# Fung-Lab/MatDeepLearn

Hardware: AMD Instinct MI355X
Metric: edges/sec training CGCNN on bulk_data (higher is better)
Workload: dtype bf16

## Files before the change

include/mdl_hip.h:

```cpp
#ifndef MDL_HIP_H
#define MDL_HIP_H

#include <stddef.h>
#include <stdint.h>

#ifdef __cplusplus
extern "C" {
#endif

#define MDL_VERSION 100

enum { MDL_F32 = 0, MDL_BF16 = 1 };
enum { MDL_SUM = 0, MDL_MEAN = 1, MDL_MAX = 2 };
enum {
    MDL_OK = 0,
    MDL_E_ARG = -1,
    MDL_E_UNSUPP = -2,
    MDL_E_LAUNCH = -3
};

#define MDL_DTYPE_MASK 0xff
#define MDL_DETERMINISTIC 0x100
#define MDL_K3_PER_WAVE 0x200
#define MDL_K3_EDGE_LANE 0x400
#define MDL_BN_SHIFT_ROW 0x800
#define MDL_SPLIT_BF16 0x1000
#define MDL_MLP_F32_IO 0x2000

typedef void* mdlStream_t;

int mdl_version(void);
const char* mdl_last_error_string(void);
int mdl_debug_last_k3(void);

int mdl_rbf_expand(const float* d, const float* offsets, float coeff, void* out, int64_t E, int G,
                   int64_t ld_out, int out_dtype, mdlStream_t stream);

int mdl_csr_rowptr(const int32_t* sorted_index, int64_t E, int64_t N, int32_t* rowptr, mdlStream_t stream);

int mdl_segment_reduce_fwd(const void* src, const int32_t* rowptr, const int32_t* perm, void* out,
                           int32_t* argmax, int64_t N, int64_t C, int reduce, int dtype, mdlStream_t stream);
int mdl_segment_reduce_bwd(const void* grad_out, const int32_t* rowptr, const int32_t* seg,
                           const int32_t* perm, const int32_t* argmax, void* grad_src, int64_t N,
                           int64_t E, int64_t C, int reduce, int dtype, mdlStream_t stream);
int mdl_segment_reduce_bwd_add(const void* grad_out, const int32_t* rowptr, const int32_t* seg, const int32_t* perm,
                               const void* addend, void* grad_src, int64_t N, int64_t E, int64_t C, int reduce, int dtype,
                               mdlStream_t stream);

size_t mdl_cgconv_wpack_bytes(int C, int G, int dtype);
int mdl_cgconv_pack_weights(const float* w_f, const float* b_f, const float* w_s, const float* b_s, int C,
                            int G, void* wpack, float* bpack, int dtype, mdlStream_t stream);
int mdl_cgconv_pack_weights_node(const float* w_f, const float* b_f, const float* w_s, const float* b_s, int C,
                                 int G, void* wpack, float* bpack, void* wn_t, int dtype, mdlStream_t stream);

int mdl_cgconv_pack_weights_multi(int L, const float* const* w_f, const float* const* b_f, const float* const* w_s,
                                  const float* const* b_s, int C, int G, void* const* wpack, float* const* bpack,
                                  void* const* wn_t, int dtype, mdlStream_t stream);

int mdl_cgconv_fwd(const void* x, const void* edge_attr, const int32_t* rowptr, const int32_t* src,
                   const int32_t* tgt, const int32_t* eperm, const void* wpack, const float* bpack,
                   void* out, int64_t N, int64_t E, int C, int G, int aggr, int dtype, mdlStream_t stream);

typedef struct MdlCgConv {
    uint32_t size;
    int32_t dtype;
    uint32_t flags;
    int32_t aggr;
    int64_t N, E;
    int32_t C, G;
    const void* x;
    const void* edge_attr;
    const int32_t* rowptr;
    const int32_t* src;
    const int32_t* tgt;
    const int32_t* eperm;
    const void* wpack;
    const float* bpack;
    void* out;
    float* bn_sums;
    const float* bn_shift;
    const int64_t* bn_rows;
    const void* grad_out;
    void* r_tgt;
    void* r_src;
    int32_t r_src_dtype;
    int32_t ld_dwe;
    float* dwe;
    float* db;
    void* workspace;
    size_t workspace_bytes;
    const int32_t* balance;
} MdlCgConv;
int mdl_cgconv_fwd_ex(const MdlCgConv* args, mdlStream_t stream);
int mdl_cgconv_bwd_ex(const MdlCgConv* args, mdlStream_t stream);

int mdl_cgconv_balance(const int32_t* rowptr, const int32_t* src, int64_t N, int32_t* cost, mdlStream_t stream);

size_t mdl_cgconv_workspace_bytes(int64_t N, int64_t E, int C, int G, int dtype);

typedef struct MdlCgNode {
    uint32_t size;
    int32_t dtype;
    uint32_t flags;
    int32_t zero_src;
    int64_t N;
    int32_t C;
    int32_t r_src_dtype;
    int32_t ld_dwn;
    int32_t reserved;
    const void* x;
    const void* grad_out;
    const void* r_tgt;
    void* r_src;
    const void* wn_t;
    void* dx;
    float* dwn;
} MdlCgNode;
int mdl_cgconv_bwd_node_ex(const MdlCgNode* args, mdlStream_t stream);

int mdl_cgconv_pack_node_weights(const float* w_f, const float* w_s, int C, int G, void* wn_t, int dtype, mdlStream_t stream);
int mdl_cgconv_assemble_grads(const float* dwn, const float* dwe, const float* db, int C, int G, float* dw_f, float* dw_s,
                              float* db_f, float* db_s, mdlStream_t stream);

int mdl_assemble_batch(const int64_t* ids, const int64_t* noff, const int64_t* eoff, const int64_t* node_ptr,
                       const int64_t* edge_ptr, const float* x_all, const int32_t* src_l, const int32_t* tgt_l,
                       const float* dist, const float* dist_norm, const int32_t* lrowptr, const float* y_all,
                       void* x, int64_t* batch, int32_t* rowptr, int32_t* src, int32_t* tgt, float* ew, float* dn,
                       float* y, int B, int F, int T, int target_index, int dtype, mdlStream_t stream);
int mdl_assemble_batch_padded(const int64_t* ids, const int64_t* noff, const int64_t* eoff, const int64_t* node_ptr,
                              const int64_t* edge_ptr, const float* x_all, const int32_t* src_l, const int32_t* tgt_l,
                              const float* dist, const float* dist_norm, const int32_t* lrowptr, const float* y_all,
                              void* x, int64_t* batch, int32_t* rowptr, int32_t* src, int32_t* tgt, float* ew, float* dn,
                              float* y, int B, int F, int T, int target_index, int dtype, int64_t n_cap, int64_t e_cap,
                              int32_t* pool_seg, int32_t* col_s, int32_t* eid_s, int32_t* src_s, mdlStream_t stream);

int mdl_ssp_bwd(const void* g, const void* y, void* dx, int64_t n, int dtype, mdlStream_t stream);

int mdl_linear_act_stats(const void* x, const void* w, const void* bias, const void* p1, const int32_t* idx1, const void* p2,
                         const int32_t* idx2, const void* p3, const int32_t* idx3, void* out, int64_t N, int K, int M, int act,
                         float* bn_sums, const int64_t* n_rows_dev, int dtype, mdlStream_t stream);
int mdl_linear_gather_act(const void* x, const void* w, const void* bias, const void* p1, const int32_t* idx1,
                          const void* p2, const int32_t* idx2, const void* p3, const int32_t* idx3, void* out,
                          int64_t N, int K, int M, int act, int dtype, mdlStream_t stream);

int mdl_nnconv_msg_fwd(const void* Y, const void* h, const int32_t* rowptr_s, const int32_t* eid_s, void* m, int64_t N,
                       int Co, int D3, int dtype, mdlStream_t stream);
int mdl_nnconv_msg_bwd(const void* Y, const void* h, const void* dm, const int32_t* rowptr_s, const int32_t* eid_s,
                       void* dh, void* dY, int64_t N, int Co, int D3, int dtype, mdlStream_t stream);

int mdl_pad_batch_tail(const int64_t* noff, const int64_t* eoff, int B, int64_t n_cap, int32_t* rowptr, int64_t* batch,
                       mdlStream_t stream);

int mdl_assemble_transposed(const int64_t* ids, const int64_t* noff, const int64_t* eoff, const int64_t* node_ptr,
                            const int64_t* edge_ptr, const int32_t* src_l, const int32_t* tgt_l, const int32_t* eperm_s,
                            const int32_t* lrowptr_s, int32_t* rowptr_s, int32_t* col_s, int32_t* eid_s, int32_t* src_s, int B,
                            int64_t n_cap, mdlStream_t stream);
int mdl_pad_edge_tail(const int64_t* noff, const int64_t* eoff, int B, int64_t n_cap, int64_t e_cap, int32_t* src, int32_t* tgt,
                      int32_t* col_s, int32_t* eid_s, int32_t* src_s, mdlStream_t stream);

int mdl_loss_fwd_bwd(const float* pred, const float* y, int64_t n, int kind, float* loss, float* grad, mdlStream_t stream);
int mdl_loss_fwd_bwd_rows(const float* pred, const float* y, int64_t n, int64_t n_total, int kind, float* loss, float* grad,
                          mdlStream_t stream);

#define MDL_BN_REPLICAS 16
int mdl_bn_sums_rows(void);
int mdl_bn_stats_n(const void* x, float* sums, int64_t N, int C, const int64_t* n_rows_dev, int dtype, mdlStream_t stream);
int mdl_bn_apply_n(const void* x, float* sums, const float* gamma, const float* beta, float* save, float* running_mean,
                   float* running_var, void* y, int64_t N, int C, float eps, float momentum, const int64_t* n_rows_dev,
                   int dtype, mdlStream_t stream);
int mdl_bn_bwd_stats_n(const void* dy, const void* x, const float* save, float* sums, int64_t N, int C,
                       const int64_t* n_rows_dev, int dtype, mdlStream_t stream);
int mdl_bn_bwd_apply_n(const void* dy, const void* x, const float* save, float* sums, const float* gamma, void* dx,
                       int64_t N, int C, const int64_t* n_rows_dev, int dtype, mdlStream_t stream);
int mdl_bn_bwd_apply_relu_n(const void* dy, const void* x, const float* save, float* sums, const float* gamma, void* dx,
                            int64_t N, int C, const int64_t* n_rows_dev, int dtype, mdlStream_t stream);
int mdl_linear_act(const void* x, const void* w, const void* bias, void* out, int64_t N, int K, int M, int act, int dtype,
                   mdlStream_t stream);
int mdl_linear_act_in(const void* x, const void* y, int xact, const void* w, const void* bias, void* out, int64_t N, int K,
                      int M, int act, int dtype, mdlStream_t stream);

int mdl_mlp_head_fwd(const void* x, const void* const* w, const void* const* b, void* const* h, int64_t N, int K0, int NL,
                     const int* M, int dtype, mdlStream_t stream);
int mdl_mlp_head_bwd(const void* x, const void* const* w, const void* const* h, const void* gy, void* dx, float* const* dw,
                     float* const* db, int64_t N, int K0, int NL, const int* M, int dtype, mdlStream_t stream);

int mdl_gru_gates_fwd(const void* gi, const void* gh, const float* h, float* h_out, void* out_lp, int64_t N, int C, int dtype,
                      mdlStream_t stream);
int mdl_gru_gates_bwd(const void* gi, const void* gh, const float* h, const float* g_h, const void* g_lp, void* dgi, void* dgh,
                      float* dh, int64_t N, int C, int dtype, mdlStream_t stream);

int mdl_linear_wide(const void* x, const void* w, void* out, int64_t N, int K, int64_t M, int dtype, mdlStream_t stream);

int mdl_gemm_tn(const void* a, int64_t lda, int M, const void* b, int64_t ldb, int K, float* c, int64_t N, int dtype,
                mdlStream_t stream);
int mdl_gemm_tn_colsum(const void* a, int64_t lda, int M, const void* b, int64_t ldb, int K, float* c, float* colsum,
                       int64_t N, int dtype, mdlStream_t stream);
int mdl_gemm_tn_act(const void* a, int64_t lda, int M, const void* y, int64_t ldy, int act, const void* b, int64_t ldb,
                    int K, float* c, float* colsum, int64_t N, int dtype, mdlStream_t stream);
int mdl_dense_bwd(const void* g, int64_t ldg, int M, const void* y, int64_t ldy, int act, const void* x, int64_t ldx, int K,
                  const void* w, void* dx, int64_t lddx, int xout, void* gm, float* dw, float* db, int64_t N, int dtype,
                  mdlStream_t stream);
size_t mdl_tn_scratch_bytes(void);
int mdl_dense_bwd_ex(const void* g, int64_t ldg, int M, const void* y, int64_t ldy, int act, const void* x, int64_t ldx, int K,
                     const void* w, void* dx, int64_t lddx, int xout, void* gm, float* dw, float* db, void* scratch, int64_t N,
                     int dtype, mdlStream_t stream);
int mdl_gemm_tn_ex(const void* a, int64_t lda, int M, const void* y, int64_t ldy, int act, const void* b, int64_t ldb, int K,
                   float* c, float* colsum, void* scratch, int64_t N, int dtype, mdlStream_t stream);

int mdl_gather_rows(const void* src, const int32_t* idx, void* out, int64_t E, int64_t C, int dtype,
                    mdlStream_t stream);
int mdl_gather_mul_reduce(const void* h, const void* w, const float* scale, const int32_t* rowptr,
                          const int32_t* col, const int32_t* eid, void* out, int64_t N, int64_t F, int reduce,
                          int dtype, mdlStream_t stream);
int mdl_gather_mul_reduce_dw(const void* g, const void* w, const float* scale, const int32_t* rowptr_s,
                             const int32_t* col_s, const int32_t* eid_s, void* dh, const void* h, void* dw,
                             int64_t N, int64_t F, int dtype, mdlStream_t stream);
int mdl_cfconv_supported(int F, int G, int dtype);
size_t mdl_cfconv_wpack_bytes(void);
int mdl_cfconv_pack_weights(const float* w1, const float* b1, const float* w2, const float* b2, int F, int G, void* wpack,
                            mdlStream_t stream);
int mdl_cfconv_fwd(const void* rbf, const float* cut, const void* h, const int32_t* rowptr, const int32_t* src,
                   const int32_t* tgt, const void* wpack, void* out, void* a1, void* w, int64_t N, int64_t E, int F, int G,
                   int dtype, mdlStream_t stream);
size_t mdl_cfconv_bwd_w_scratch_bytes(void);
int mdl_cfconv_bwd_w(const void* rbf, const float* cut, const void* h, const void* g, const int32_t* rowptr, const int32_t* src,
                     const int32_t* tgt, const void* wpack, float* dw1, float* db1, float* dw2, float* db2, void* scratch, int64_t N,
                     int64_t E, int F, int G, int dtype, mdlStream_t stream);
int mdl_edge_mul(const void* a, const int32_t* ia, const void* b, const int32_t* ib, const float* scale, void* out,
                 int64_t E, int64_t F, int dtype, mdlStream_t stream);
int mdl_edge_dot(const void* a, const int32_t* ia, const void* b, const int32_t* ib, const void* w, float* out, int64_t E,
                 int64_t F, int dtype, mdlStream_t stream);
int mdl_cfconv_bwd_edge_supported(int F, int G, int dtype);
int mdl_cfconv_bwd_edge(const void* rbf, const float* cut, const void* h, const void* g, const int32_t* rowptr, const int32_t* src,
                        const int32_t* tgt, const void* wpack, const float* w1, const float* b1, const float* w2, const float* b2,
                        int64_t N, int64_t E, int F, int G, int dtype, float* dcut, void* drbf, const float* d_norm,
                        const float* offsets, float coeff, float scale, float* dd, mdlStream_t stream);

int mdl_split_bf16(const float* src, void* hi, void* lo, int64_t n, mdlStream_t stream);

size_t mdl_graph_workspace_bytes(int64_t N, int64_t G, int max_neighbors);
int mdl_graph_build(const double* pos, const int64_t* node_ptr, const double* cell, const int32_t* pbc, int64_t N, int64_t G,
                    double radius, int max_neighbors, int64_t* edge_ptr, int32_t* src, int32_t* tgt, float* dist,
                    int32_t* out_deg, int64_t edge_capacity, void* workspace, size_t workspace_bytes, mdlStream_t stream);

int mdl_rbf_expand_bwd(const void* g_out, int64_t ld_g, int g_dtype, const float* d, const float* offsets, float coeff,
                       float* dd, int64_t E, int G, mdlStream_t stream);

int mdl_cgconv_bwd_edge(const void* x, const void* edge_attr, const int32_t* rowptr, const int32_t* src, const int32_t* tgt,
                        const void* wpack, const float* bpack, const void* grad_out, int64_t N, int64_t E, int C, int G,
                        int aggr, int dtype, void* de, const float* d_norm, const float* offsets, float coeff, float scale,
                        float* dd, mdlStream_t stream);

int mdl_linear_rbf_dist_grad_supported(int M, int G, int dtype);
int mdl_linear_rbf_dist_grad(const void* g, int64_t ld_g, const void* act_y, int64_t ld_y, const void* w, int dtype,
                             const float* d, const float* offsets, float coeff, float scale, float* dd, int accumulate,
                             int64_t E, int M, int G, mdlStream_t stream);

size_t mdl_edge_geometry_workspace_bytes(int64_t G);
int mdl_edge_geometry_fwd(const double* pos, const int64_t* node_ptr, const double* cell, const int32_t* pbc, int64_t N,
                          int64_t G, const int32_t* src, const int32_t* tgt, int64_t E, float* dist, float* u,
                          void* workspace, size_t workspace_bytes, mdlStream_t stream);
int mdl_edge_geometry_bwd(const float* dd, const float* u, const int32_t* rowptr_t, const int32_t* eid_t,
                          const int32_t* rowptr_s, const int32_t* eid_s, int64_t N, int64_t E, float* dpos,
                          mdlStream_t stream);

size_t mdl_edge_strain_grad_workspace_bytes(int64_t G, int64_t E, int32_t slices);
int mdl_edge_strain_grad(const float* dd, const float* dist, const float* u, const int32_t* rowptr_t, const int32_t* eid_t,
                         const int64_t* node_ptr, int64_t N, int64_t G, int64_t E, int32_t slices, float* out, void* workspace,
                         size_t workspace_bytes, mdlStream_t stream);

#ifdef __cplusplus
}
#endif
#endif
```

matdeeplearn_amd/_lib.py:

```python
import ctypes
import os

import torch

HERE = os.path.dirname(os.path.abspath(__file__))
LIB_PATH = os.path.join(HERE, "lib", "libmdl_hip.so")


def use_library(path):
    global LIB_PATH, _lib
    if _lib is not None and os.path.abspath(path) != os.path.abspath(LIB_PATH):
        raise MdlError("use_library(%s): %s is already loaded in this process" % (path, LIB_PATH))
    LIB_PATH = path

MDL_F32, MDL_BF16 = 0, 1
MDL_SUM, MDL_MEAN, MDL_MAX = 0, 1, 2
MDL_DTYPE_MASK, MDL_DETERMINISTIC, MDL_K3_PER_WAVE, MDL_K3_EDGE_LANE = 0xFF, 0x100, 0x200, 0x400
MDL_MLP_F32_IO = 0x2000
MDL_SPLIT_BF16 = 0x1000
MDL_BN_SHIFT_ROW = 0x800
MDL_BN_REPLICAS = 16
REDUCE = {"sum": MDL_SUM, "add": MDL_SUM, "mean": MDL_MEAN, "max": MDL_MAX}

_vp, _i64, _i32, _f32, _sz = ctypes.c_void_p, ctypes.c_int64, ctypes.c_int, ctypes.c_float, ctypes.c_size_t
_u32 = ctypes.c_uint32


class MdlCgConv(ctypes.Structure):
    _fields_ = [("size", _u32), ("dtype", _i32), ("flags", _u32), ("aggr", _i32), ("N", _i64), ("E", _i64), ("C", _i32), ("G", _i32),
                ("x", _vp), ("edge_attr", _vp), ("rowptr", _vp), ("src", _vp), ("tgt", _vp), ("eperm", _vp), ("wpack", _vp),
                ("bpack", _vp), ("out", _vp), ("bn_sums", _vp), ("bn_shift", _vp), ("bn_rows", _vp), ("grad_out", _vp),
                ("r_tgt", _vp), ("r_src", _vp), ("r_src_dtype", _i32), ("ld_dwe", _i32), ("dwe", _vp), ("db", _vp),
                ("workspace", _vp), ("workspace_bytes", _sz), ("balance", _vp)]


class MdlCgNode(ctypes.Structure):
    _fields_ = [("size", _u32), ("dtype", _i32), ("flags", _u32), ("zero_src", _i32), ("N", _i64), ("C", _i32), ("r_src_dtype", _i32),
                ("ld_dwn", _i32), ("reserved", _i32), ("x", _vp), ("grad_out", _vp), ("r_tgt", _vp), ("r_src", _vp), ("wn_t", _vp), ("dx", _vp), ("dwn", _vp)]


def _dp(t):
    return None if t is None else t.data_ptr()


def cg_args(**kw):
    a = MdlCgConv()
    a.size = ctypes.sizeof(MdlCgConv)
    for k, v in kw.items():
        setattr(a, k, _dp(v) if torch.is_tensor(v) else v)
    return a


def cg_node_args(**kw):
    a = MdlCgNode()
    a.size = ctypes.sizeof(MdlCgNode)
    for k, v in kw.items():
        setattr(a, k, _dp(v) if torch.is_tensor(v) else v)
    return a

PROTOTYPES = {
    "mdl_version": (_i32, []),
    "mdl_last_error_string": (ctypes.c_char_p, []),
    "mdl_debug_last_k3": (_i32, []),
    "mdl_rbf_expand": (_i32, [_vp, _vp, _f32, _vp, _i64, _i32, _i64, _i32, _vp]),
    "mdl_csr_rowptr": (_i32, [_vp, _i64, _i64, _vp, _vp]),
    "mdl_segment_reduce_fwd": (_i32, [_vp, _vp, _vp, _vp, _vp, _i64, _i64, _i32, _i32, _vp]),
    "mdl_segment_reduce_bwd": (_i32, [_vp, _vp, _vp, _vp, _vp, _vp, _i64, _i64, _i64, _i32, _i32, _vp]),
    "mdl_segment_reduce_bwd_add": (_i32, [_vp, _vp, _vp, _vp, _vp, _vp, _i64, _i64, _i64, _i32, _i32, _vp]),
    "mdl_cgconv_wpack_bytes": (_sz, [_i32, _i32, _i32]),
    "mdl_cgconv_pack_weights": (_i32, [_vp, _vp, _vp, _vp, _i32, _i32, _vp, _vp, _i32, _vp]),
    "mdl_cgconv_pack_weights_node": (_i32, [_vp, _vp, _vp, _vp, _i32, _i32, _vp, _vp, _vp, _i32, _vp]),
    "mdl_cgconv_pack_weights_multi": (_i32, [_i32, _vp, _vp, _vp, _vp, _i32, _i32, _vp, _vp, _vp, _i32, _vp]),
    "mdl_cgconv_fwd": (_i32, [_vp] * 9 + [_i64, _i64, _i32, _i32, _i32, _i32, _vp]),
    "mdl_cgconv_fwd_ex": (_i32, [ctypes.POINTER(MdlCgConv), _vp]),
    "mdl_cgconv_bwd_ex": (_i32, [ctypes.POINTER(MdlCgConv), _vp]),
    "mdl_cgconv_bwd_node_ex": (_i32, [ctypes.POINTER(MdlCgNode), _vp]),
    "mdl_cgconv_workspace_bytes": (ctypes.c_size_t, [_i64, _i64, _i32, _i32, _i32]),
    "mdl_cgconv_balance": (_i32, [_vp, _vp, _i64, _vp, _vp]),
    "mdl_cgconv_pack_node_weights": (_i32, [_vp, _vp, _i32, _i32, _vp, _i32, _vp]),
    "mdl_cgconv_assemble_grads": (_i32, [_vp, _vp, _vp, _i32, _i32, _vp, _vp, _vp, _vp, _vp]),
    "mdl_assemble_batch": (_i32, [_vp] * 20 + [_i32, _i32, _i32, _i32, _i32, _vp]),
    "mdl_assemble_batch_padded": (_i32, [_vp] * 20 + [_i32, _i32, _i32, _i32, _i32, _i64, _i64, _vp, _vp, _vp, _vp, _vp]),
    "mdl_nnconv_msg_fwd": (_i32, [_vp] * 5 + [_i64, _i32, _i32, _i32, _vp]),
    "mdl_nnconv_msg_bwd": (_i32, [_vp] * 7 + [_i64, _i32, _i32, _i32, _vp]),
    "mdl_pad_batch_tail": (_i32, [_vp, _vp, _i32, _i64, _vp, _vp, _vp]),
    "mdl_assemble_transposed": (_i32, [_vp] * 13 + [_i32, _i64, _vp]),
    "mdl_pad_edge_tail": (_i32, [_vp, _vp, _i32, _i64, _i64, _vp, _vp, _vp, _vp, _vp, _vp]),
    "mdl_loss_fwd_bwd": (_i32, [_vp, _vp, _i64, _i32, _vp, _vp, _vp]),
    "mdl_loss_fwd_bwd_rows": (_i32, [_vp, _vp, _i64, _i64, _i32, _vp, _vp, _vp]),
    "mdl_bn_sums_rows": (_i32, []),
    "mdl_bn_stats_n": (_i32, [_vp, _vp, _i64, _i32, _vp, _i32, _vp]),
    "mdl_bn_apply_n": (_i32, [_vp] * 8 + [_i64, _i32, _f32, _f32, _vp, _i32, _vp]),
    "mdl_bn_bwd_stats_n": (_i32, [_vp, _vp, _vp, _vp, _i64, _i32, _vp, _i32, _vp]),
    "mdl_bn_bwd_apply_n": (_i32, [_vp] * 6 + [_i64, _i32, _vp, _i32, _vp]),
    "mdl_bn_bwd_apply_relu_n": (_i32, [_vp] * 6 + [_i64, _i32, _vp, _i32, _vp]),
    "mdl_linear_act": (_i32, [_vp, _vp, _vp, _vp, _i64, _i32, _i32, _i32, _i32, _vp]),
    "mdl_dense_bwd": (_i32, [_vp, _i64, _i32, _vp, _i64, _i32, _vp, _i64, _i32, _vp, _vp, _i64, _i32, _vp, _vp, _vp, _i64, _i32, _vp]),
    "mdl_dense_bwd_ex": (_i32, [_vp, _i64, _i32, _vp, _i64, _i32, _vp, _i64, _i32, _vp, _vp, _i64, _i32, _vp, _vp, _vp, _vp, _i64, _i32, _vp]),
    "mdl_tn_scratch_bytes": (_sz, []),
    "mdl_linear_act_stats": (_i32, [_vp, _vp, _vp, _vp, _vp, _vp, _vp, _vp, _vp, _vp, _i64, _i32, _i32, _i32, _vp, _vp, _i32, _vp]),
    "mdl_linear_act_in": (_i32, [_vp, _vp, _i32, _vp, _vp, _vp, _i64, _i32, _i32, _i32, _i32, _vp]),
    "mdl_ssp_bwd": (_i32, [_vp, _vp, _vp, _i64, _i32, _vp]),
    "mdl_linear_gather_act": (_i32, [_vp] * 10 + [_i64, _i32, _i32, _i32, _i32, _vp]),
    "mdl_linear_wide": (_i32, [_vp, _vp, _vp, _i64, _i32, _i64, _i32, _vp]),
    "mdl_mlp_head_fwd": (_i32, [_vp, _vp, _vp, _vp, _i64, _i32, _i32, _vp, _i32, _vp]),
    "mdl_mlp_head_bwd": (_i32, [_vp, _vp, _vp, _vp, _vp, _vp, _vp, _i64, _i32, _i32, _vp, _i32, _vp]),
    "mdl_gru_gates_fwd": (_i32, [_vp, _vp, _vp, _vp, _vp, _i64, _i32, _i32, _vp]),
    "mdl_gru_gates_bwd": (_i32, [_vp, _vp, _vp, _vp, _vp, _vp, _vp, _vp, _i64, _i32, _i32, _vp]),
    "mdl_gemm_tn": (_i32, [_vp, _i64, _i32, _vp, _i64, _i32, _vp, _i64, _i32, _vp]),
    "mdl_split_bf16": (_i32, [_vp, _vp, _vp, _i64, _vp]),
    "mdl_gemm_tn_colsum": (_i32, [_vp, _i64, _i32, _vp, _i64, _i32, _vp, _vp, _i64, _i32, _vp]),
    "mdl_gemm_tn_act": (_i32, [_vp, _i64, _i32, _vp, _i64, _i32, _vp, _i64, _i32, _vp, _vp, _i64, _i32, _vp]),
    "mdl_gemm_tn_ex": (_i32, [_vp, _i64, _i32, _vp, _i64, _i32, _vp, _i64, _i32, _vp, _vp, _vp, _i64, _i32, _vp]),
    "mdl_gather_rows": (_i32, [_vp, _vp, _vp, _i64, _i64, _i32, _vp]),
    "mdl_gather_mul_reduce": (_i32, [_vp] * 7 + [_i64, _i64, _i32, _i32, _vp]),
    "mdl_gather_mul_reduce_dw": (_i32, [_vp] * 9 + [_i64, _i64, _i32, _vp]),
    "mdl_edge_mul": (_i32, [_vp] * 6 + [_i64, _i64, _i32, _vp]),
    "mdl_cfconv_supported": (_i32, [_i32, _i32, _i32]),
    "mdl_cfconv_wpack_bytes": (_sz, []),
    "mdl_cfconv_pack_weights": (_i32, [_vp] * 4 + [_i32, _i32, _vp, _vp]),
    "mdl_cfconv_fwd": (_i32, [_vp] * 10 + [_i64, _i64, _i32, _i32, _i32, _vp]),
    "mdl_cfconv_bwd_w_scratch_bytes": (_sz, []),
    "mdl_cfconv_bwd_w": (_i32, [_vp] * 13 + [_i64, _i64, _i32, _i32, _i32, _vp]),
    "mdl_cfconv_bwd_edge_supported": (_i32, [_i32, _i32, _i32]),
    "mdl_cfconv_bwd_edge": (_i32, [_vp] * 12 + [_i64, _i64, _i32, _i32, _i32, _vp, _vp, _vp, _vp, _f32, _f32, _vp, _vp]),
    "mdl_edge_dot": (_i32, [_vp] * 6 + [_i64, _i64, _i32, _vp]),
    "mdl_graph_workspace_bytes": (_sz, [_i64, _i64, _i32]),
    "mdl_graph_build": (_i32, [_vp] * 4 + [_i64, _i64, ctypes.c_double, _i32] + [_vp] * 5 + [_i64, _vp, _sz, _vp]),
    "mdl_rbf_expand_bwd": (_i32, [_vp, _i64, _i32, _vp, _vp, _f32, _vp, _i64, _i32, _vp]),
    "mdl_cgconv_bwd_edge": (_i32, [_vp] * 8 + [_i64, _i64, _i32, _i32, _i32, _i32, _vp, _vp, _vp, _f32, _f32, _vp, _vp]),
    "mdl_linear_rbf_dist_grad_supported": (_i32, [_i32, _i32, _i32]),
    "mdl_linear_rbf_dist_grad": (_i32, [_vp, _i64, _vp, _i64, _vp, _i32, _vp, _vp, _f32, _f32, _vp, _i32, _i64, _i32, _i32, _vp]),
    "mdl_edge_geometry_workspace_bytes": (_sz, [_i64]),
    "mdl_edge_geometry_fwd": (_i32, [_vp] * 4 + [_i64, _i64, _vp, _vp, _i64, _vp, _vp, _vp, _sz, _vp]),
    "mdl_edge_geometry_bwd": (_i32, [_vp] * 6 + [_i64, _i64, _vp, _vp]),
    "mdl_edge_strain_grad_workspace_bytes": (_sz, [_i64, _i64, _i32]),
    "mdl_edge_strain_grad": (_i32, [_vp] * 6 + [_i64, _i64, _i64, _i32, _vp, _vp, _sz, _vp]),
}

_lib = None


class MdlError(RuntimeError):
    pass


def lib():
    global _lib
    if _lib is None:
        if not os.path.exists(LIB_PATH):
            raise MdlError(
                "libmdl_hip.so not found at %s — build it with `python -m matdeeplearn_amd._build` "
                "(hipcc --offload-arch=gfx950).  matdeeplearn_amd has no CPU/eager fallback." % LIB_PATH)
        handle = ctypes.CDLL(LIB_PATH)
        for name, (res, args) in PROTOTYPES.items():
            fn = getattr(handle, name)
            fn.restype, fn.argtypes = res, args
        _lib = handle
    return _lib


def check(rc, what):
    if rc != 0:
        raise MdlError("%s failed (%d): %s" % (what, rc, lib().mdl_last_error_string().decode()))


def dtype_code(t):
    if t.dtype == torch.float32:
        return MDL_F32
    if t.dtype == torch.bfloat16:
        return MDL_BF16
    raise MdlError("unsupported dtype %s (float32 or bfloat16)" % t.dtype)


def require_hip(*tensors):
    cur = None
    for t in tensors:
        if t is None:
            continue
        if not t.is_cuda:
            raise MdlError("matdeeplearn_amd ops need tensors on a HIP device (got %s); there is no CPU path — "
                           "the CPU restatement lives in oracle/ and is test infrastructure only" % t.device)
        if cur is None:
            cur = torch.cuda.current_device()
        if t.device.index != cur:
            raise MdlError("tensor on %s but the current HIP device is cuda:%d — call torch.cuda.set_device(%d) in "
                           "this process before using matdeeplearn_amd" % (t.device, cur, t.device.index))


def ptr(t):
    return None if t is None else ctypes.c_void_p(t.data_ptr())


def stream():
    return ctypes.c_void_p(torch._C._cuda_getCurrentRawStream(torch.cuda.current_device()))
```

matdeeplearn_amd/csrc/bn.hip:

```cpp
#include "mdl_common.h"

namespace mdl {

constexpr int BN_R = MDL_BN_REPLICAS;

__device__ __forceinline__ void bn_totals(const float* __restrict__ sums, float* tot, int C, float* publish) {
    for (int c = threadIdx.x; c < 2 * C; c += blockDim.x) {
        float v[BN_R];
#pragma unroll
        for (int r = 0; r < BN_R; ++r) v[r] = sums[(size_t)r * 2 * C + c];
        float t = 0.0f;
#pragma unroll
        for (int r = 0; r < BN_R; ++r) t += v[r];
        tot[c] = t;
        if (publish && blockIdx.x == 0) publish[c] = t;
    }
    __syncthreads();
}

template <typename T, int MODE, int W>
__global__ __launch_bounds__(256) void bn_reduce_kernel(const T* __restrict__ a, const T* __restrict__ b,
                                                        const float* __restrict__ save, float* __restrict__ sums,
                                                        int64_t Ncap, int C, const int64_t* __restrict__ n_dev) {
    typedef VecW<T, W> V;
    const int64_t N = n_dev ? max((int64_t)1, min(*n_dev, Ncap)) : Ncap;
    __shared__ float red[2][256 * 8 / 8 * 8];
    const int CG = C / W;
    const int rows_per_block = (int)blockDim.x / CG;
    const int cg = threadIdx.x % CG, rl = threadIdx.x / CG;
    const bool active = rl < rows_per_block;
    float s0[W], s1[W], p0[W], p1[W];
#pragma unroll
    for (int j = 0; j < W; ++j) { s0[j] = 0.0f; s1[j] = 0.0f; }
    if (MODE == 0) {
        V::ld(a + cg * W, p0);
    } else {
#pragma unroll
        for (int j = 0; j < W; ++j) { p0[j] = save[cg * W + j]; p1[j] = save[C + cg * W + j]; }
    }
    if (active) {
        constexpr int U = 4;
        const int64_t stride = (int64_t)gridDim.x * rows_per_block;
        for (int64_t n0 = (int64_t)blockIdx.x * rows_per_block + rl; n0 < N; n0 += U * stride) {
            float va[U][W], vb[U][W];
#pragma unroll
            for (int u = 0; u < U; ++u) {
                const int64_t n = min(n0 + u * stride, N - 1);
                V::ld(a + n * C + cg * W, va[u]);
                if (MODE != 0) V::ld(b + n * C + cg * W, vb[u]);
            }
#pragma unroll
            for (int u = 0; u < U; ++u) {
                const float m = (n0 + u * stride < N) ? 1.0f : 0.0f;
                if (MODE == 0) {
#pragma unroll
                    for (int j = 0; j < W; ++j) { const float d = (va[u][j] - p0[j]) * m; s0[j] += d; s1[j] += d * d; }
                } else {
#pragma unroll
                    for (int j = 0; j < W; ++j) { const float v = va[u][j] * m; s0[j] += v; s1[j] += v * ((vb[u][j] - p0[j]) * p1[j]); }
                }
            }
        }
    }
#pragma unroll
    for (int j = 0; j < W; ++j) { red[0][threadIdx.x * W + j] = s0[j]; red[1][threadIdx.x * W + j] = s1[j]; }
    __syncthreads();
    if ((int)threadIdx.x < C) {
        const int c = threadIdx.x, g = c / W, j = c % W;
        float t0 = 0.0f, t1 = 0.0f;
        for (int r = 0; r < rows_per_block; ++r) { t0 += red[0][(r * CG + g) * W + j]; t1 += red[1][(r * CG + g) * W + j]; }
        float* dst = sums + (size_t)(blockIdx.x % BN_R) * 2 * C;
        unsafeAtomicAdd(dst + c, t0);
        unsafeAtomicAdd(dst + C + c, t1);
    }
}

template <typename T, int W>
__global__ __launch_bounds__(256) void bn_apply_kernel(const T* __restrict__ x, float* __restrict__ sums,
                                                       const float* __restrict__ gamma, const float* __restrict__ beta,
                                                       float* __restrict__ save, float* __restrict__ run_mean,
                                                       float* __restrict__ run_var, T* __restrict__ y, int64_t Ncap, int C,
                                                       float eps, float momentum, const int64_t* __restrict__ n_dev,
                                                       int shift_row) {
    typedef VecW<T, W> V;
    constexpr int U = 4;
    const int64_t N = n_dev ? max((int64_t)1, min(*n_dev, Ncap)) : Ncap;
    __shared__ float tot[512];
    const int CG = C / W;
    const int cg = threadIdx.x % CG;
    const int64_t total = N * CG;
    const int64_t stride = (int64_t)gridDim.x * blockDim.x;
    int64_t q0 = (int64_t)blockIdx.x * blockDim.x + threadIdx.x;
    float v[U][W];
#pragma unroll
    for (int u = 0; u < U; ++u) V::ld(x + (min(q0 + u * stride, total - 1) / CG) * C + cg * W, v[u]);
    float mean[W], scale[W], shiftv[W], sh[W];
    V::ld(x + cg * W, sh);
    if (shift_row) {
        const float* srow = sums + (size_t)(2 * BN_R + 2) * C;
#pragma unroll
        for (int j = 0; j < W; ++j) sh[j] = srow[cg * W + j];
    }
    bn_totals(sums, tot, C, sums + (size_t)BN_R * 2 * C);
    const float invn = 1.0f / (float)N;
#pragma unroll
    for (int j = 0; j < W; ++j) {
        const int c = cg * W + j;
        const float m1 = tot[c] * invn;
        const float var = fmaxf(tot[C + c] * invn - m1 * m1, 0.0f);
        const float istd = rsqrtf(var + eps);
        mean[j] = sh[j] + m1;
        const float g = gamma ? gamma[c] : 1.0f;
        scale[j] = istd * g;
        shiftv[j] = (beta ? beta[c] : 0.0f) - mean[j] * scale[j];
        if (blockIdx.x == 0 && (int)threadIdx.x < CG) {
            save[c] = mean[j];
            save[C + c] = istd;
            if (run_mean) {
                const float unb = N > 1 ? var * ((float)N / (float)(N - 1)) : var;
                run_mean[c] = (1.0f - momentum) * run_mean[c] + momentum * mean[j];
                run_var[c] = (1.0f - momentum) * run_var[c] + momentum * unb;
            }
        }
    }
    while (true) {
#pragma unroll
        for (int u = 0; u < U; ++u) {
            const int64_t q = q0 + u * stride;
#pragma unroll
            for (int j = 0; j < W; ++j) v[u][j] = v[u][j] * scale[j] + shiftv[j];
            if (q < total) V::st(y + (q / CG) * C + cg * W, v[u]);
        }
        q0 += U * stride;
        if (q0 >= total) break;
#pragma unroll
        for (int u = 0; u < U; ++u) V::ld(x + (min(q0 + u * stride, total - 1) / CG) * C + cg * W, v[u]);
    }
    if (N < Ncap) {
        float z[W];
#pragma unroll
        for (int j = 0; j < W; ++j) z[j] = 0.0f;
        for (int64_t q = total + (int64_t)blockIdx.x * blockDim.x + threadIdx.x; q < Ncap * CG; q += stride)
            V::st(y + (q / CG) * C + cg * W, z);
    }
}

template <typename T, int W, bool MASK = false>
__global__ __launch_bounds__(256) void bn_bwd_apply_kernel(const T* __restrict__ dy, const T* __restrict__ x,
                                                           const float* __restrict__ save, float* __restrict__ sums,
                                                           const float* __restrict__ gamma, T* __restrict__ dx, int64_t Ncap,
                                                           int C, const int64_t* __restrict__ n_dev) {
    typedef VecW<T, W> V;
    constexpr int U = 2;
    const int64_t N = n_dev ? max((int64_t)1, min(*n_dev, Ncap)) : Ncap;
    __shared__ float tot[512];
    const int CG = C / W;
    const int cg = threadIdx.x % CG;
    const int64_t total = N * CG;
    const int64_t stride = (int64_t)gridDim.x * blockDim.x;
    int64_t q0 = (int64_t)blockIdx.x * blockDim.x + threadIdx.x;
    float vd[U][W], vx[U][W];
#pragma unroll
    for (int u = 0; u < U; ++u) {
        const int64_t n = min(q0 + u * stride, total - 1) / CG;
        V::ld(dy + n * C + cg * W, vd[u]);
        V::ld(x + n * C + cg * W, vx[u]);
    }
    bn_totals(sums, tot, C, sums + (size_t)BN_R * 2 * C);
    const float invn = 1.0f / (float)N;
    float mean[W], istd[W], k0[W], k1[W], gs[W];
#pragma unroll
    for (int j = 0; j < W; ++j) {
        const int c = cg * W + j;
        mean[j] = save[c];
        istd[j] = save[C + c];
        gs[j] = (gamma ? gamma[c] : 1.0f) * istd[j];
        k0[j] = tot[c] * invn;
        k1[j] = tot[C + c] * invn;
    }
    while (true) {
#pragma unroll
        for (int u = 0; u < U; ++u) {
            const int64_t q = q0 + u * stride;
#pragma unroll
            for (int j = 0; j < W; ++j) {
                const float d = gs[j] * (vd[u][j] - k0[j] - (vx[u][j] - mean[j]) * istd[j] * k1[j]);
                vd[u][j] = (!MASK || vx[u][j] > 0.0f) ? d : 0.0f;
            }
            if (q < total) V::st(dx + (q / CG) * C + cg * W, vd[u]);
        }
        q0 += U * stride;
        if (q0 >= total) break;
#pragma unroll
        for (int u = 0; u < U; ++u) {
            const int64_t n = min(q0 + u * stride, total - 1) / CG;
            V::ld(dy + n * C + cg * W, vd[u]);
            V::ld(x + n * C + cg * W, vx[u]);
        }
    }
    if (N < Ncap) {
        float z[W];
#pragma unroll
        for (int j = 0; j < W; ++j) z[j] = 0.0f;
        for (int64_t q = total + (int64_t)blockIdx.x * blockDim.x + threadIdx.x; q < Ncap * CG; q += stride)
            V::st(dx + (q / CG) * C + cg * W, z);
    }
}


static int bn_width(int C, int dtype) { return (dtype == MDL_BF16 && C % 8 == 0) ? 8 : 4; }
static int bn_threads(int C, int W) { const int cg = C / W; return 256 / cg * cg; }

static int bn_check(const char* name, int64_t N, int C, int dtype, const void* p) {
    MDL_REQUIRE(dtype == MDL_F32 || dtype == MDL_BF16, MDL_E_UNSUPP, "%s: unsupported dtype %d", name, dtype);
    MDL_REQUIRE(N >= 1 && C >= 4 && C % 4 == 0 && C <= 256, MDL_E_UNSUPP,
                "%s: need N>=1 and C a multiple of 4, C<=256 (got N=%lld C=%d)", name, (long long)N, C);
    MDL_REQUIRE(p && reinterpret_cast<uintptr_t>(p) % (bn_width(C, dtype) * (dtype == MDL_BF16 ? 2 : 4)) == 0, MDL_E_ARG,
                "%s: null or misaligned tensor", name);
    return MDL_OK;
}

static unsigned bn_grid(int64_t N, int C, int W, bool det) {
    if (det) return 1;
    const int rows = 256 / (C / W);
    int64_t g = cdiv(N, (int64_t)rows * 8);
    if (g > 1024) g = 1024;
    return (unsigned)(g < 1 ? 1 : g);
}

}

extern "C" int mdl_bn_sums_rows(void) { return 2 * (MDL_BN_REPLICAS + 1); }

extern "C" int mdl_bn_stats_n(const void* x, float* sums, int64_t N, int C, const int64_t* n_dev, int dtype, mdlStream_t stream) {
    using namespace mdl;
    const bool det = (dtype & MDL_DETERMINISTIC) != 0;
    dtype &= MDL_DTYPE_MASK;
    int rc = bn_check("mdl_bn_stats", N, C, dtype, x);
    if (rc) return rc;
    hipStream_t st = (hipStream_t)stream;
    const int W = bn_width(C, dtype);
    if (dtype == MDL_BF16 && W == 8) hipLaunchKernelGGL((bn_reduce_kernel<bf16_t, 0, 8>), dim3(bn_grid(N, C, W, det)), dim3(bn_threads(C, 8)), 0, st, (const bf16_t*)x, (const bf16_t*)nullptr, (const float*)nullptr, sums, N, C, n_dev);
    else if (dtype == MDL_BF16) hipLaunchKernelGGL((bn_reduce_kernel<bf16_t, 0, 4>), dim3(bn_grid(N, C, W, det)), dim3(bn_threads(C, 4)), 0, st, (const bf16_t*)x, (const bf16_t*)nullptr, (const float*)nullptr, sums, N, C, n_dev);
    else hipLaunchKernelGGL((bn_reduce_kernel<float, 0, 4>), dim3(bn_grid(N, C, W, det)), dim3(bn_threads(C, 4)), 0, st, (const float*)x, (const float*)nullptr, (const float*)nullptr, sums, N, C, n_dev);
    return check_launch("mdl_bn_stats");
}

extern "C" int mdl_bn_apply_n(const void* x, float* sums, const float* gamma, const float* beta, float* save,
                              float* running_mean, float* running_var, void* y, int64_t N, int C, float eps, float momentum,
                              const int64_t* n_dev, int dtype, mdlStream_t stream) {
    using namespace mdl;
    const int shift_row = (dtype & MDL_BN_SHIFT_ROW) ? 1 : 0;
    dtype &= MDL_DTYPE_MASK;
    int rc = bn_check("mdl_bn_apply", N, C, dtype, x);
    if (rc) return rc;
    hipStream_t st = (hipStream_t)stream;
    int64_t g = cdiv(N * (C / bn_width(C, dtype)), 256 * 4);
    if (g > 768) g = 768;
    if (g < 1) g = 1;
    const int W = bn_width(C, dtype);
    if (dtype == MDL_BF16 && W == 8) hipLaunchKernelGGL((bn_apply_kernel<bf16_t, 8>), dim3((unsigned)g), dim3(bn_threads(C, 8)), 0, st, (const bf16_t*)x, sums, gamma, beta, save, running_mean, running_var, (bf16_t*)y, N, C, eps, momentum, n_dev, shift_row);
    else if (dtype == MDL_BF16) hipLaunchKernelGGL((bn_apply_kernel<bf16_t, 4>), dim3((unsigned)g), dim3(bn_threads(C, 4)), 0, st, (const bf16_t*)x, sums, gamma, beta, save, running_mean, running_var, (bf16_t*)y, N, C, eps, momentum, n_dev, shift_row);
    else hipLaunchKernelGGL((bn_apply_kernel<float, 4>), dim3((unsigned)g), dim3(bn_threads(C, 4)), 0, st, (const float*)x, sums, gamma, beta, save, running_mean, running_var, (float*)y, N, C, eps, momentum, n_dev, shift_row);
    return check_launch("mdl_bn_apply");
}

extern "C" int mdl_bn_bwd_stats_n(const void* dy, const void* x, const float* save, float* sums, int64_t N, int C,
                                  const int64_t* n_dev, int dtype, mdlStream_t stream) {
    using namespace mdl;
    const bool det = (dtype & MDL_DETERMINISTIC) != 0;
    dtype &= MDL_DTYPE_MASK;
    int rc = bn_check("mdl_bn_bwd_stats", N, C, dtype, x);
    if (rc) return rc;
    hipStream_t st = (hipStream_t)stream;
    const int W = bn_width(C, dtype);
    if (dtype == MDL_BF16 && W == 8) hipLaunchKernelGGL((bn_reduce_kernel<bf16_t, 1, 8>), dim3(bn_grid(N, C, W, det)), dim3(bn_threads(C, 8)), 0, st, (const bf16_t*)dy, (const bf16_t*)x, save, sums, N, C, n_dev);
    else if (dtype == MDL_BF16) hipLaunchKernelGGL((bn_reduce_kernel<bf16_t, 1, 4>), dim3(bn_grid(N, C, W, det)), dim3(bn_threads(C, 4)), 0, st, (const bf16_t*)dy, (const bf16_t*)x, save, sums, N, C, n_dev);
    else hipLaunchKernelGGL((bn_reduce_kernel<float, 1, 4>), dim3(bn_grid(N, C, W, det)), dim3(bn_threads(C, 4)), 0, st, (const float*)dy, (const float*)x, save, sums, N, C, n_dev);
    return check_launch("mdl_bn_bwd_stats");
}

static int bn_bwd_apply_launch(const char* name, bool mask, const void* dy, const void* x, const float* save, float* sums, const float* gamma,
                               void* dx, int64_t N, int C, const int64_t* n_dev, int dtype, mdlStream_t stream) {
    using namespace mdl;
    dtype &= MDL_DTYPE_MASK;
    int rc = bn_check(name, N, C, dtype, x);
    if (rc) return rc;
    hipStream_t st = (hipStream_t)stream;
    int64_t g = cdiv(N * (C / bn_width(C, dtype)), 256 * 4);
    if (g > 768) g = 768;
    if (g < 1) g = 1;
    const int W = bn_width(C, dtype);
    if (mask) {
        MDL_REQUIRE(dtype == MDL_BF16, MDL_E_UNSUPP, "%s: bf16 only", name);
        if (W == 8) hipLaunchKernelGGL((bn_bwd_apply_kernel<bf16_t, 8, true>), dim3((unsigned)g), dim3(bn_threads(C, 8)), 0, st, (const bf16_t*)dy, (const bf16_t*)x, save, sums, gamma, (bf16_t*)dx, N, C, n_dev);
        else hipLaunchKernelGGL((bn_bwd_apply_kernel<bf16_t, 4, true>), dim3((unsigned)g), dim3(bn_threads(C, 4)), 0, st, (const bf16_t*)dy, (const bf16_t*)x, save, sums, gamma, (bf16_t*)dx, N, C, n_dev);
        return check_launch(name);
    }
    if (dtype == MDL_BF16 && W == 8) hipLaunchKernelGGL((bn_bwd_apply_kernel<bf16_t, 8>), dim3((unsigned)g), dim3(bn_threads(C, 8)), 0, st, (const bf16_t*)dy, (const bf16_t*)x, save, sums, gamma, (bf16_t*)dx, N, C, n_dev);
    else if (dtype == MDL_BF16) hipLaunchKernelGGL((bn_bwd_apply_kernel<bf16_t, 4>), dim3((unsigned)g), dim3(bn_threads(C, 4)), 0, st, (const bf16_t*)dy, (const bf16_t*)x, save, sums, gamma, (bf16_t*)dx, N, C, n_dev);
    else hipLaunchKernelGGL((bn_bwd_apply_kernel<float, 4>), dim3((unsigned)g), dim3(bn_threads(C, 4)), 0, st, (const float*)dy, (const float*)x, save, sums, gamma, (float*)dx, N, C, n_dev);
    return check_launch(name);
}

extern "C" int mdl_bn_bwd_apply_n(const void* dy, const void* x, const float* save, float* sums, const float* gamma,
                                  void* dx, int64_t N, int C, const int64_t* n_dev, int dtype, mdlStream_t stream) {
    return bn_bwd_apply_launch("mdl_bn_bwd_apply", false, dy, x, save, sums, gamma, dx, N, C, n_dev, dtype, stream);
}
extern "C" int mdl_bn_bwd_apply_relu_n(const void* dy, const void* x, const float* save, float* sums, const float* gamma,
                                       void* dx, int64_t N, int C, const int64_t* n_dev, int dtype, mdlStream_t stream) {
    return bn_bwd_apply_launch("mdl_bn_bwd_apply_relu", true, dy, x, save, sums, gamma, dx, N, C, n_dev, dtype, stream);
}
```

matdeeplearn_amd/csrc/cgconv_node.hip:

```cpp
#include "mdl_common.h"

namespace mdl {

constexpr int K3C_NW = 8;

typedef __attribute__((ext_vector_type(4))) unsigned u32x4_t;

__device__ __forceinline__ bf16x8 pack8(const float* v) {
    u32x4_t r = {pk_bf16(v[0], v[1]), pk_bf16(v[2], v[3]), pk_bf16(v[4], v[5]), pk_bf16(v[6], v[7])};
    return __builtin_bit_cast(bf16x8, r);
}

template <int CP, bool RS16 = false, int NW = 4>
__global__ __launch_bounds__(64 * NW, 2) void cgconv_node_stream_kernel(const bf16_t* __restrict__ x, const bf16_t* __restrict__ gout,
                                                                    const bf16_t* __restrict__ r_tgt,
                                                                    const float* __restrict__ r_src,
                                                                    const bf16_t* __restrict__ wn_t, bf16_t* __restrict__ dx,
                                                                    float* __restrict__ dwn, int64_t N, int zero_src, int ld_out) {
    typedef __attribute__((ext_vector_type(4))) short s16x4;
    typedef __attribute__((address_space(3))) s16x4* lds4_t;
    constexpr int TN = 64;
    constexpr int K4 = 4 * CP;
    constexpr int LD = K4 + 8;
    constexpr int LX = CP + 8;
    constexpr int NT = CP / 32;
    constexpr int TCH = 2 * CP / 8;
    constexpr int SCH = 2 * CP / 4;
    constexpr int NTH = 64 * NW;
    constexpr int NTL = TN * TCH / NTH;
    constexpr int NSL = RS16 ? NTL : TN * SCH / NTH;
    constexpr int XCH = CP / 8;
    constexpr int NXL = TN * XCH / NTH;
    constexpr int MJ = (K4 / 32) * NT / NW;
    static_assert(NTL >= 1 && NSL >= 1 && NXL >= 1 && MJ >= 1, "too many waves for this width");
    extern __shared__ __attribute__((aligned(16))) char smem[];
    bf16_t* wl = reinterpret_cast<bf16_t*>(smem);
    bf16_t* rl = wl + CP * LD;
    bf16_t* xl = rl + TN * LD;
    const int tid = threadIdx.x, lane = tid & 63, i = lane & 31, h = lane >> 5, wv = __builtin_amdgcn_readfirstlane(tid >> 6);
    for (int q = tid; q < CP * (K4 / 8); q += NTH) {
        const int row = q / (K4 / 8), c8 = q - row * (K4 / 8);
        *reinterpret_cast<bf16x8*>(wl + row * LD + c8 * 8) = *reinterpret_cast<const bf16x8*>(wn_t + row * K4 + c8 * 8);
    }
    f32x16 dw[MJ];
#pragma unroll
    for (int j = 0; j < MJ; ++j)
#pragma unroll
        for (int r = 0; r < 16; ++r) dw[j][r] = 0.0f;

    const int64_t n_tiles = (N + TN - 1) / TN;
    u32x4_t treg[NTL];
    f32x4 sreg[NSL];
    u32x4_t xreg[NXL];
    static_assert(NTH % TCH == 0 && NTH % SCH == 0 && NTH % XCH == 0, "chunk mapping");
    constexpr int TROWS = NTH / TCH, SROWS = NTH / SCH, XROWS = NTH / XCH;
    const int trow0 = tid / TCH, tcc = tid % TCH, srow0 = tid / SCH, scc = tid % SCH, xrow0 = tid / XCH, xcc = tid % XCH;
    const int to = (trow0 * (2 * CP) + 8 * tcc) * 2, so = (srow0 * (2 * CP) + 4 * scc) * 4, xo = (xrow0 * CP + 8 * xcc) * 2;
    auto rsrc = [](const void* base, int64_t bytes) {
        return __builtin_amdgcn_make_buffer_rsrc(const_cast<void*>(base), 0, (int)(bytes < 0x7fffffffLL ? bytes : 0x7fffffffLL), 0x00020000);
    };
    auto opaque = [](int v) { asm volatile("" : "+s"(v)); return v; };
    auto load_tile = [&](int64_t tile) {
        const int64_t nb = tile * TN, rem = N - nb;
        const __amdgpu_buffer_rsrc_t tr = rsrc(r_tgt + nb * (2 * CP), rem * (2 * CP * 2));
        const __amdgpu_buffer_rsrc_t sr = RS16 ? rsrc(reinterpret_cast<const bf16_t*>(r_src) + nb * (2 * CP), rem * (2 * CP * 2))
                                               : rsrc(r_src + nb * (2 * CP), rem * (2 * CP * 4));
        const __amdgpu_buffer_rsrc_t xr = rsrc(x + nb * CP, rem * (CP * 2));
#pragma unroll
        for (int l = 0; l < NTL; ++l) treg[l] = __builtin_amdgcn_raw_buffer_load_b128(tr, to + opaque(l * (TROWS * 2 * CP * 2)), 0, 0);
#pragma unroll
        for (int l = 0; l < NSL; ++l)
            sreg[l] = __builtin_bit_cast(f32x4, __builtin_amdgcn_raw_buffer_load_b128(
                sr, RS16 ? to + opaque(l * (TROWS * 2 * CP * 2)) : so + opaque(l * (SROWS * 2 * CP * 4)), 0, 0));
#pragma unroll
        for (int l = 0; l < NXL; ++l) xreg[l] = __builtin_amdgcn_raw_buffer_load_b128(xr, xo + opaque(l * (XROWS * CP * 2)), 0, 0);
    };
    int64_t tile = blockIdx.x;
    if (tile < n_tiles) load_tile(tile);
    for (; tile < n_tiles; tile += gridDim.x) {
        const int64_t nb = tile * TN;
        __syncthreads();
#pragma unroll
        for (int l = 0; l < NTL; ++l) *reinterpret_cast<u32x4_t*>(rl + (trow0 + l * TROWS) * LD + 8 * tcc) = treg[l];
#pragma unroll
        for (int l = 0; l < NSL; ++l) {
            if constexpr (RS16) {
                *reinterpret_cast<u32x4_t*>(rl + (trow0 + l * TROWS) * LD + 2 * CP + 8 * tcc) = __builtin_bit_cast(u32x4_t, sreg[l]);
            } else {
                typedef __attribute__((ext_vector_type(2))) unsigned u32x2_t;
                const u32x2_t v = {pk_bf16(sreg[l][0], sreg[l][1]), pk_bf16(sreg[l][2], sreg[l][3])};
                *reinterpret_cast<u32x2_t*>(rl + (srow0 + l * SROWS) * LD + 2 * CP + 4 * scc) = v;
            }
        }
        if (zero_src) {
            const int64_t rem = N - nb;
            const __amdgpu_buffer_rsrc_t sz = RS16 ? rsrc(reinterpret_cast<const bf16_t*>(r_src) + nb * (2 * CP), rem * (2 * CP * 2))
                                                   : rsrc(r_src + nb * (2 * CP), rem * (2 * CP * 4));
#pragma unroll
            for (int l = 0; l < NSL; ++l)
                __builtin_amdgcn_raw_buffer_store_b128(u32x4_t{0u, 0u, 0u, 0u}, sz,
                                                       RS16 ? to + opaque(l * (TROWS * 2 * CP * 2)) : so + opaque(l * (SROWS * 2 * CP * 4)), 0, 0);
        }
#pragma unroll
        for (int l = 0; l < NXL; ++l) {
            *reinterpret_cast<u32x4_t*>(xl + (xrow0 + l * XROWS) * LX + 8 * xcc) = xreg[l];
        }
        __syncthreads();
        const bool dxw = wv < 2 * NT;
        const int mt0 = wv / NT, nt0 = wv - mt0 * NT;
        const int64_t remg = N - nb - mt0 * 32;
        const int go = (4 * h * CP + nt0 * 32 + i) * 2;
        const bool more = tile + gridDim.x < n_tiles;
        if (!dxw) {
            if (more) load_tile(tile + gridDim.x);
        } else {
            short gv[16];
            const __amdgpu_buffer_rsrc_t gr = rsrc(gout + (nb + mt0 * 32) * CP, (remg > 0 ? remg : 0) * (CP * 2));
#pragma unroll
            for (int r = 0; r < 16; ++r) gv[r] = __builtin_amdgcn_raw_buffer_load_b16(gr, go + ((r & 3) + 8 * (r >> 2)) * CP * 2, 0, 0);
            if (more) load_tile(tile + gridDim.x);
            f32x16 acc;
#pragma unroll
            for (int r = 0; r < 16; ++r) acc[r] = 0.0f;
#pragma unroll
            for (int kk = 0; kk < K4 / 16; ++kk) {
                const bf16x8 a = *reinterpret_cast<const bf16x8*>(rl + (mt0 * 32 + i) * LD + 16 * kk + 8 * h);
                const bf16x8 b = *reinterpret_cast<const bf16x8*>(wl + (nt0 * 32 + i) * LD + 16 * kk + 8 * h);
                acc = __builtin_amdgcn_mfma_f32_32x32x16_bf16(a, b, acc, 0, 0, 0);
            }
            const __amdgpu_buffer_rsrc_t dr = rsrc(dx + (nb + mt0 * 32) * CP, (remg > 0 ? remg : 0) * (CP * 2));
#pragma unroll
            for (int r = 0; r < 16; ++r)
                __builtin_amdgcn_raw_buffer_store_b16((short)f2bf(bf2f((bf16_t)gv[r]) + acc[r]), dr, go + ((r & 3) + 8 * (r >> 2)) * CP * 2, 0, 0);
        }
#pragma unroll
        for (int j = 0; j < MJ; ++j) {
            const int blk = wv * MJ + j, mt = blk / NT, nt = blk - mt * NT;
            const int t = i & 15;
#pragma unroll
            for (int ks = 0; ks < TN / 16; ++ks) {
                const bf16_t* pa = rl + (16 * ks + 8 * h + (t >> 2)) * LD + mt * 32 + (i & 16) + 4 * (t & 3);
                const bf16_t* pb = xl + (16 * ks + 8 * h + (t >> 2)) * LX + nt * 32 + (i & 16) + 4 * (t & 3);
                const s16x4 a0 = __builtin_amdgcn_ds_read_tr16_b64_v4i16((lds4_t)pa), a1 = __builtin_amdgcn_ds_read_tr16_b64_v4i16((lds4_t)(pa + 4 * LD));
                const s16x4 b0 = __builtin_amdgcn_ds_read_tr16_b64_v4i16((lds4_t)pb), b1 = __builtin_amdgcn_ds_read_tr16_b64_v4i16((lds4_t)(pb + 4 * LX));
                const bf16x8 af = {a0[0], a0[1], a0[2], a0[3], a1[0], a1[1], a1[2], a1[3]};
                const bf16x8 bfr = {b0[0], b0[1], b0[2], b0[3], b1[0], b1[1], b1[2], b1[3]};
                dw[j] = __builtin_amdgcn_mfma_f32_32x32x16_bf16(af, bfr, dw[j], 0, 0, 0);
            }
        }
    }
#pragma unroll
    for (int j = 0; j < MJ; ++j) {
        const int blk = wv * MJ + j, mt = blk / NT, nt = blk - mt * NT;
#pragma unroll
        for (int r = 0; r < 16; ++r) {
            const int R = mt * 32 + d_row(r, h), K = nt * 32 + i;
            const int64_t at = ld_out > 0 ? (int64_t)(((R / CP) & 1) * CP + R % CP) * ld_out + ((R / CP) >> 1) * CP + K : (int64_t)R * CP + K;
            unsafeAtomicAdd(dwn + at, dw[j][r]);
        }
    }
}

template <int CP, int NW>
__global__ __launch_bounds__(64 * NW, 1) void cgconv_node_x3_kernel(const float* __restrict__ x, const float* __restrict__ gout,
                                                                    const float* __restrict__ r_tgt, float* __restrict__ r_src,
                                                                    const float* __restrict__ wn_t, float* __restrict__ dx,
                                                                    float* __restrict__ dwn, int64_t N, int zero_src, int ld_out) {
    typedef __attribute__((ext_vector_type(4))) short s16x4;
    typedef __attribute__((address_space(3))) s16x4* lds4_t;
    typedef __attribute__((ext_vector_type(2))) unsigned u32x2_t;
    constexpr int TN = 64, K4 = 4 * CP, LD = K4 + 8, LX = CP + 8, NT = CP / 32, NTH = 64 * NW;
    constexpr int RCH = 2 * CP / 4;
    constexpr int XCH = CP / 4;
    constexpr int NRL = TN * RCH / NTH;
    constexpr int NXL = TN * XCH / NTH;
    constexpr int MJ = (K4 / 32) * NT / NW;
    static_assert(NRL >= 1 && NXL >= 1 && MJ >= 1 && NTH % RCH == 0 && NTH % XCH == 0 && 2 * NT <= NW, "shape / wave count");
    extern __shared__ __attribute__((aligned(16))) char smem[];
    bf16_t* wl_h = reinterpret_cast<bf16_t*>(smem);
    bf16_t* wl_l = wl_h + CP * LD;
    bf16_t* rl_h = wl_l + CP * LD;
    bf16_t* rl_l = rl_h + TN * LD;
    bf16_t* xl_h = rl_l + TN * LD;
    bf16_t* xl_l = xl_h + TN * LX;
    const int tid = threadIdx.x, lane = tid & 63, i = lane & 31, h = lane >> 5, wv = __builtin_amdgcn_readfirstlane(tid >> 6);
    auto split4 = [](const f32x4& v, u32x2_t& hi, u32x2_t& lo) {
        const unsigned ha = pk_bf16(v[0], v[1]), hb = pk_bf16(v[2], v[3]);
        hi = u32x2_t{ha, hb};
        lo = u32x2_t{pk_bf16(v[0] - __builtin_bit_cast(float, ha << 16), v[1] - __builtin_bit_cast(float, ha & 0xffff0000u)),
                     pk_bf16(v[2] - __builtin_bit_cast(float, hb << 16), v[3] - __builtin_bit_cast(float, hb & 0xffff0000u))};
    };
    for (int q = tid; q < CP * (K4 / 4); q += NTH) {
        const int row = q / (K4 / 4), c4 = q - row * (K4 / 4);
        u32x2_t hi, lo;
        split4(*reinterpret_cast<const f32x4*>(wn_t + row * K4 + c4 * 4), hi, lo);
        *reinterpret_cast<u32x2_t*>(wl_h + row * LD + c4 * 4) = hi;
        *reinterpret_cast<u32x2_t*>(wl_l + row * LD + c4 * 4) = lo;
    }
    f32x16 dw[MJ];
#pragma unroll
    for (int j = 0; j < MJ; ++j)
#pragma unroll
        for (int r = 0; r < 16; ++r) dw[j][r] = 0.0f;

    const int64_t n_tiles = (N + TN - 1) / TN;
    f32x4 treg[NRL], sreg[NRL], xreg[NXL];
    constexpr int RROWS = NTH / RCH, XROWS = NTH / XCH;
    const int rrow0 = tid / RCH, rcc = tid % RCH, xrow0 = tid / XCH, xcc = tid % XCH;
    const int ro = (rrow0 * (2 * CP) + 4 * rcc) * 4, xo = (xrow0 * CP + 4 * xcc) * 4;
    auto rsrc = [](const void* base, int64_t bytes) {
        return __builtin_amdgcn_make_buffer_rsrc(const_cast<void*>(base), 0, (int)(bytes < 0 ? 0 : (bytes < 0x7fffffffLL ? bytes : 0x7fffffffLL)), 0x00020000);
    };
    auto opaque = [](int v) { asm volatile("" : "+s"(v)); return v; };
    auto load_tile = [&](int64_t tile) {
        const int64_t nb = tile * TN, rem = N - nb;
        const __amdgpu_buffer_rsrc_t tr = rsrc(r_tgt + nb * (2 * CP), rem * (2 * CP * 4));
        const __amdgpu_buffer_rsrc_t sr = rsrc(r_src + nb * (2 * CP), rem * (2 * CP * 4));
        const __amdgpu_buffer_rsrc_t xr = rsrc(x + nb * CP, rem * (CP * 4));
#pragma unroll
        for (int l = 0; l < NRL; ++l) treg[l] = __builtin_bit_cast(f32x4, __builtin_amdgcn_raw_buffer_load_b128(tr, ro + opaque(l * (RROWS * 2 * CP * 4)), 0, 0));
#pragma unroll
        for (int l = 0; l < NRL; ++l) sreg[l] = __builtin_bit_cast(f32x4, __builtin_amdgcn_raw_buffer_load_b128(sr, ro + opaque(l * (RROWS * 2 * CP * 4)), 0, 0));
#pragma unroll
        for (int l = 0; l < NXL; ++l) xreg[l] = __builtin_bit_cast(f32x4, __builtin_amdgcn_raw_buffer_load_b128(xr, xo + opaque(l * (XROWS * CP * 4)), 0, 0));
    };
    int64_t tile = blockIdx.x;
    if (tile < n_tiles) load_tile(tile);
    for (; tile < n_tiles; tile += gridDim.x) {
        const int64_t nb = tile * TN;
        __syncthreads();
#pragma unroll
        for (int l = 0; l < NRL; ++l) {
            u32x2_t hi, lo;
            split4(treg[l], hi, lo);
            *reinterpret_cast<u32x2_t*>(rl_h + (rrow0 + l * RROWS) * LD + 4 * rcc) = hi;
            *reinterpret_cast<u32x2_t*>(rl_l + (rrow0 + l * RROWS) * LD + 4 * rcc) = lo;
            split4(sreg[l], hi, lo);
            *reinterpret_cast<u32x2_t*>(rl_h + (rrow0 + l * RROWS) * LD + 2 * CP + 4 * rcc) = hi;
            *reinterpret_cast<u32x2_t*>(rl_l + (rrow0 + l * RROWS) * LD + 2 * CP + 4 * rcc) = lo;
        }
        if (zero_src) {
            const __amdgpu_buffer_rsrc_t sz = rsrc(r_src + nb * (2 * CP), (N - nb) * (2 * CP * 4));
#pragma unroll
            for (int l = 0; l < NRL; ++l)
                __builtin_amdgcn_raw_buffer_store_b128(u32x4_t{0u, 0u, 0u, 0u}, sz, ro + opaque(l * (RROWS * 2 * CP * 4)), 0, 0);
        }
#pragma unroll
        for (int l = 0; l < NXL; ++l) {
            u32x2_t hi, lo;
            split4(xreg[l], hi, lo);
            *reinterpret_cast<u32x2_t*>(xl_h + (xrow0 + l * XROWS) * LX + 4 * xcc) = hi;
            *reinterpret_cast<u32x2_t*>(xl_l + (xrow0 + l * XROWS) * LX + 4 * xcc) = lo;
        }
        __syncthreads();
        const bool dxw = wv < 2 * NT;
        const int mt0 = wv / NT, nt0 = wv - mt0 * NT;
        const int64_t remg = N - nb - mt0 * 32;
        const int go = (4 * h * CP + nt0 * 32 + i) * 4;
        const bool more = tile + gridDim.x < n_tiles;
        if (!dxw) {
            if (more) load_tile(tile + gridDim.x);
        } else {
            float gv[16];
            const __amdgpu_buffer_rsrc_t gr = rsrc(gout + (nb + mt0 * 32) * CP, (remg > 0 ? remg : 0) * (CP * 4));
#pragma unroll
            for (int r = 0; r < 16; ++r)
                gv[r] = __builtin_bit_cast(float, __builtin_amdgcn_raw_buffer_load_b32(gr, go + ((r & 3) + 8 * (r >> 2)) * CP * 4, 0, 0));
            if (more) load_tile(tile + gridDim.x);
            f32x16 acc;
#pragma unroll
            for (int r = 0; r < 16; ++r) acc[r] = 0.0f;
#pragma unroll
            for (int kk = 0; kk < K4 / 16; ++kk) {
                const int ao = (mt0 * 32 + i) * LD + 16 * kk + 8 * h, bo = (nt0 * 32 + i) * LD + 16 * kk + 8 * h;
                const bf16x8 ah = *reinterpret_cast<const bf16x8*>(rl_h + ao), al = *reinterpret_cast<const bf16x8*>(rl_l + ao);
                const bf16x8 bh = *reinterpret_cast<const bf16x8*>(wl_h + bo), bl = *reinterpret_cast<const bf16x8*>(wl_l + bo);
                acc = __builtin_amdgcn_mfma_f32_32x32x16_bf16(al, bh, acc, 0, 0, 0);
                acc = __builtin_amdgcn_mfma_f32_32x32x16_bf16(ah, bl, acc, 0, 0, 0);
                acc = __builtin_amdgcn_mfma_f32_32x32x16_bf16(ah, bh, acc, 0, 0, 0);
            }
            const __amdgpu_buffer_rsrc_t dr = rsrc(dx + (nb + mt0 * 32) * CP, (remg > 0 ? remg : 0) * (CP * 4));
#pragma unroll
            for (int r = 0; r < 16; ++r)
                __builtin_amdgcn_raw_buffer_store_b32(__builtin_bit_cast(unsigned, gv[r] + acc[r]), dr, go + ((r & 3) + 8 * (r >> 2)) * CP * 4, 0, 0);
        }
#pragma unroll
        for (int j = 0; j < MJ; ++j) {
            const int blk = wv * MJ + j, mt = blk / NT, nt = blk - mt * NT;
            const int t = i & 15;
#pragma unroll
            for (int ks = 0; ks < TN / 16; ++ks) {
                const int pa = (16 * ks + 8 * h + (t >> 2)) * LD + mt * 32 + (i & 16) + 4 * (t & 3);
                const int pb = (16 * ks + 8 * h + (t >> 2)) * LX + nt * 32 + (i & 16) + 4 * (t & 3);
                auto frag = [&](const bf16_t* base, int off, int ld) {
                    const s16x4 v0 = __builtin_amdgcn_ds_read_tr16_b64_v4i16((lds4_t)(base + off));
                    const s16x4 v1 = __builtin_amdgcn_ds_read_tr16_b64_v4i16((lds4_t)(base + off + 4 * ld));
                    return bf16x8{v0[0], v0[1], v0[2], v0[3], v1[0], v1[1], v1[2], v1[3]};
                };
                const bf16x8 ah = frag(rl_h, pa, LD), al = frag(rl_l, pa, LD), bh = frag(xl_h, pb, LX), bl = frag(xl_l, pb, LX);
                dw[j] = __builtin_amdgcn_mfma_f32_32x32x16_bf16(al, bh, dw[j], 0, 0, 0);
                dw[j] = __builtin_amdgcn_mfma_f32_32x32x16_bf16(ah, bl, dw[j], 0, 0, 0);
                dw[j] = __builtin_amdgcn_mfma_f32_32x32x16_bf16(ah, bh, dw[j], 0, 0, 0);
            }
        }
    }
#pragma unroll
    for (int j = 0; j < MJ; ++j) {
        const int blk = wv * MJ + j, mt = blk / NT, nt = blk - mt * NT;
#pragma unroll
        for (int r = 0; r < 16; ++r) {
            const int R = mt * 32 + d_row(r, h), K = nt * 32 + i;
            const int64_t at = ld_out > 0 ? (int64_t)(((R / CP) & 1) * CP + R % CP) * ld_out + ((R / CP) >> 1) * CP + K : (int64_t)R * CP + K;
            unsafeAtomicAdd(dwn + at, dw[j][r]);
        }
    }
}

}

namespace mdl {
template <typename TO>
__global__ __launch_bounds__(256) void cgconv_pack_node_kernel(const float* __restrict__ wf, const float* __restrict__ ws, int C,
                                                               int Cp, int ldw, TO* __restrict__ wn_t) {
    const int total = C * 4 * Cp;
    for (int q = blockIdx.x * blockDim.x + threadIdx.x; q < total; q += gridDim.x * blockDim.x) {
        const int k = q / (4 * Cp), r = q - k * (4 * Cp);
        const int blk = r / Cp, c = r - blk * Cp;
        float v = 0.0f;
        if (c < C) v = ((blk & 1) ? ws : wf)[c * ldw + (blk >> 1) * C + k];
        if constexpr (std::is_same<TO, float>::value) wn_t[q] = v; else wn_t[q] = f2bf(v);
    }
}
__global__ __launch_bounds__(256) void cgconv_grads_kernel(const float* __restrict__ dwn, const float* __restrict__ dwe,
                                                           const float* __restrict__ db, int C, int Cp, int G, int GP,
                                                           float* __restrict__ dwf, float* __restrict__ dws,
                                                           float* __restrict__ dbf, float* __restrict__ dbs) {
    const int ldw = 2 * C + G, total = 2 * C * ldw;
    for (int q = blockIdx.x * blockDim.x + threadIdx.x; q < total; q += gridDim.x * blockDim.x) {
        const int part = q / (C * ldw), rem = q - part * (C * ldw);
        const int c = rem / ldw, k = rem - c * ldw;
        float v;
        if (k < C) v = dwn[(part * Cp + c) * C + k];
        else if (k < 2 * C) v = dwn[((2 + part) * Cp + c) * C + (k - C)];
        else v = dwe[(part * Cp + c) * GP + (k - 2 * C)];
        (part ? dws : dwf)[rem] = v;
    }
    for (int q = blockIdx.x * blockDim.x + threadIdx.x; q < 2 * C; q += gridDim.x * blockDim.x) {
        const int part = q / C, c = q - part * C;
        float* dst = part ? dbs : dbf;
        if (dst) dst[c] = db[part * Cp + c];
    }
}
}

extern "C" int mdl_cgconv_pack_node_weights(const float* w_f, const float* w_s, int C, int G, void* wn_t, int dtype,
                                            mdlStream_t stream) {
    using namespace mdl;
    MDL_REQUIRE(dtype == MDL_BF16 || dtype == MDL_F32, MDL_E_UNSUPP, "mdl_cgconv_pack_node_weights: dtype must be MDL_BF16 or MDL_F32");
    MDL_REQUIRE(w_f && w_s && wn_t && C >= 1 && G >= 0, MDL_E_ARG, "mdl_cgconv_pack_node_weights: bad arguments");
    const int Cp = (C + 31) / 32 * 32;
    if (dtype == MDL_F32)
        hipLaunchKernelGGL(cgconv_pack_node_kernel<float>, dim3((unsigned)cdiv((int64_t)C * 4 * Cp, 256)), dim3(256), 0, (hipStream_t)stream,
                           w_f, w_s, C, Cp, 2 * C + G, (float*)wn_t);
    else
    hipLaunchKernelGGL(cgconv_pack_node_kernel<bf16_t>, dim3((unsigned)cdiv((int64_t)C * 4 * Cp, 256)), dim3(256), 0, (hipStream_t)stream, w_f,
                       w_s, C, Cp, 2 * C + G, (bf16_t*)wn_t);
    return check_launch("mdl_cgconv_pack_node_weights");
}

extern "C" int mdl_cgconv_assemble_grads(const float* dwn, const float* dwe, const float* db, int C, int G, float* dw_f,
                                         float* dw_s, float* db_f, float* db_s, mdlStream_t stream) {
    using namespace mdl;
    MDL_REQUIRE(dwn && dwe && db && dw_f && dw_s && C >= 1 && G >= 0, MDL_E_ARG, "mdl_cgconv_assemble_grads: bad arguments");
    const int Cp = (C + 31) / 32 * 32, GP = (G + 63) / 64 * 64;
    hipLaunchKernelGGL(cgconv_grads_kernel, dim3((unsigned)cdiv((int64_t)2 * C * (2 * C + G), 256)), dim3(256), 0, (hipStream_t)stream,
                       dwn, dwe, db, C, Cp, G, GP, dw_f, dw_s, db_f, db_s);
    return check_launch("mdl_cgconv_assemble_grads");
}

static int bwd_node_launch(const void* x, const void* grad_out, const void* r_tgt, float* r_src, const void* wn_t, void* dx,
                           float* dwn, int64_t N, int C, int dtype, int zero_src, bool rs16, int ld_out, mdlStream_t stream);

extern "C" int mdl_cgconv_bwd_node_ex(const MdlCgNode* a, mdlStream_t stream) {
    MDL_REQUIRE(a && a->size == sizeof(MdlCgNode), MDL_E_ARG, "mdl_cgconv_bwd_node_ex: argument struct of another layout (size %u, expected %u)",
                a ? a->size : 0u, (unsigned)sizeof(MdlCgNode));
    MDL_REQUIRE((a->flags & ~(uint32_t)(MDL_DETERMINISTIC | MDL_SPLIT_BF16)) == 0, MDL_E_ARG, "mdl_cgconv_bwd_node_ex: unknown flag bits %#x", a->flags);
    MDL_REQUIRE(a->r_src_dtype == MDL_F32 || a->r_src_dtype == MDL_BF16, MDL_E_ARG, "mdl_cgconv_bwd_node_ex: r_src_dtype must be MDL_F32 or MDL_BF16");
    if (a->flags & MDL_SPLIT_BF16) {
        using namespace mdl;
        MDL_REQUIRE(a->dtype == MDL_F32 && a->r_src_dtype == MDL_F32 && a->C == 64 && !(a->flags & MDL_DETERMINISTIC), MDL_E_UNSUPP,
                    "mdl_cgconv_bwd_node_ex: MDL_SPLIT_BF16 needs MDL_F32 storage, fp32 by-source sums, C = 64 (C=%d dtype=%d)", a->C, a->dtype);
        MDL_REQUIRE(a->N >= 0 && (a->N == 0 || (a->x && a->grad_out && a->r_tgt && a->r_src && a->wn_t && a->dx && a->dwn)), MDL_E_ARG,
                    "mdl_cgconv_bwd_node_ex: bad arguments");
        MDL_REQUIRE(reinterpret_cast<uintptr_t>(a->wn_t) % 16 == 0 && reinterpret_cast<uintptr_t>(a->r_tgt) % 16 == 0 &&
                        reinterpret_cast<uintptr_t>(a->r_src) % 16 == 0 && reinterpret_cast<uintptr_t>(a->x) % 16 == 0 &&
                        reinterpret_cast<uintptr_t>(a->grad_out) % 4 == 0 && reinterpret_cast<uintptr_t>(a->dx) % 4 == 0, MDL_E_ARG,
                    "mdl_cgconv_bwd_node_ex: 16-byte alignment required");
        MDL_REQUIRE(a->ld_dwn == 0 || a->ld_dwn >= 2 * a->C, MDL_E_ARG, "mdl_cgconv_bwd_node_ex: ld_dwn (%d) below 2 C", a->ld_dwn);
        if (a->N == 0) return MDL_OK;
        constexpr int NWX = 8;
        const int lds = (2 * 64 * (256 + 8) + 2 * 64 * (256 + 8) + 2 * 64 * (64 + 8)) * 2;
        int64_t sgrid = cdiv(a->N, 64);
        if (sgrid > 256) sgrid = 256;
        auto kf = cgconv_node_x3_kernel<64, NWX>;
        hipError_t e = set_max_dynamic_lds(reinterpret_cast<const void*>(kf), lds);
        if (e != hipSuccess) { set_error("mdl_cgconv_bwd_node_ex: LDS attribute (%d B): %s", lds, hipGetErrorString(e)); return MDL_E_LAUNCH; }
        hipLaunchKernelGGL(kf, dim3((unsigned)sgrid), dim3(64 * NWX), lds, (hipStream_t)stream, (const float*)a->x, (const float*)a->grad_out,
                           (const float*)a->r_tgt, static_cast<float*>(a->r_src), (const float*)a->wn_t, (float*)a->dx, a->dwn, a->N, a->zero_src, a->ld_dwn);
        return check_launch("mdl_cgconv_bwd_node_ex");
    }
    return bwd_node_launch(a->x, a->grad_out, a->r_tgt, static_cast<float*>(a->r_src), a->wn_t, a->dx, a->dwn, a->N, a->C,
                           a->dtype | (int)a->flags, a->zero_src, a->r_src_dtype == MDL_BF16, a->ld_dwn, stream);
}

static int bwd_node_launch(const void* x, const void* grad_out, const void* r_tgt, float* r_src, const void* wn_t, void* dx,
                           float* dwn, int64_t N, int C, int dtype, int zero_src, bool rs16, int ld_out, mdlStream_t stream) {
    using namespace mdl;
    const bool det = (dtype & MDL_DETERMINISTIC) != 0;
    dtype &= MDL_DTYPE_MASK;
    MDL_REQUIRE(dtype == MDL_BF16, MDL_E_UNSUPP, "mdl_cgconv_bwd_node: bf16 only (fp32 parity mode uses library GEMMs)");
    MDL_REQUIRE(C == 32 || C == 64, MDL_E_UNSUPP, "mdl_cgconv_bwd_node: C must be 32 or 64 (got %d)", C);
    MDL_REQUIRE(N >= 0 && (N == 0 || (x && grad_out && r_tgt && r_src && wn_t && dx && dwn)), MDL_E_ARG,
                "mdl_cgconv_bwd_node: bad arguments");
    MDL_REQUIRE(reinterpret_cast<uintptr_t>(wn_t) % 16 == 0 && reinterpret_cast<uintptr_t>(r_tgt) % 16 == 0 &&
                    reinterpret_cast<uintptr_t>(r_src) % 16 == 0, MDL_E_ARG, "mdl_cgconv_bwd_node: 16-byte alignment required");
    MDL_REQUIRE(ld_out == 0 || ld_out >= 2 * C, MDL_E_ARG, "mdl_cgconv_bwd_node_ex: ld_dwn (%d) below 2 C", ld_out);
    if (N == 0) return MDL_OK;
    hipStream_t st = (hipStream_t)stream;
    int64_t sgrid = cdiv(N, 64);
    if (det) sgrid = 1;
    if (sgrid > 256) sgrid = 256;
    if (C == 64) {
        const int lds = (64 * (256 + 8) + 64 * (256 + 8) + 64 * (64 + 8)) * 2;
        auto kf = rs16 ? cgconv_node_stream_kernel<64, true, K3C_NW> : cgconv_node_stream_kernel<64, false, K3C_NW>;
        set_max_dynamic_lds(reinterpret_cast<const void*>(kf), lds);
        hipLaunchKernelGGL(kf, dim3((unsigned)sgrid), dim3(64 * K3C_NW), lds, st, (const bf16_t*)x, (const bf16_t*)grad_out,
                           (const bf16_t*)r_tgt, r_src, (const bf16_t*)wn_t, (bf16_t*)dx, dwn, N, zero_src, ld_out);
    } else {
        const int lds = (32 * (128 + 8) + 64 * (128 + 8) + 64 * (32 + 8)) * 2;
        auto kf = rs16 ? cgconv_node_stream_kernel<32, true> : cgconv_node_stream_kernel<32, false>;
        hipLaunchKernelGGL(kf, dim3((unsigned)sgrid), dim3(256), lds, st, (const bf16_t*)x, (const bf16_t*)grad_out,
                           (const bf16_t*)r_tgt, r_src, (const bf16_t*)wn_t, (bf16_t*)dx, dwn, N, zero_src, ld_out);
    }
    return check_launch("mdl_cgconv_bwd_node");
}
```

matdeeplearn_amd/models/_base.py:

```python
import torch
import torch.nn.functional as F
from torch import nn

from .. import ops
from ..nn import BatchNorm1d, Set2Set, lowp_copies as _lowp


def dense(lin, h, split=False):
    if h.dtype == lin.weight.dtype:
        if split and ops.linear_split_ok(h, lin.weight):
            return ops._LinearSplitTN.apply(h, lin.weight, lin.bias)
        return lin(h)
    return ops.linear(h, lin.weight, lin.bias, _lowp(lin))


def dense_act(lin, h, act, split=False):
    if h.dtype == lin.weight.dtype:
        return getattr(F, act)(dense(lin, h, split))
    return ops.linear_act(h, lin.weight, lin.bias, act, _lowp(lin))


class GraphModel(nn.Module):

    def _begin(self, data, dim1, pre_fc_count, gc_count, pool, pool_order, batch_norm, batch_track_stats, act,
               dropout_rate, compute_dtype, lists=("conv_list", "bn_list")):
        assert gc_count > 0, "Need at least 1 GC layer"
        self.batch_track_stats = batch_track_stats != "False"
        self.batch_norm, self.pool, self.act = batch_norm, pool, act
        self.pool_order, self.dropout_rate = pool_order, dropout_rate
        self.compute_dtype = {"fp32": torch.float32, "bf16": torch.bfloat16, "bf16x3": torch.float32}[compute_dtype]
        self.split_products = compute_dtype == "bf16x3"
        self.gc_dim = data.num_features if pre_fc_count == 0 else dim1
        y0 = data[0].y
        self.output_dim = 1 if y0.ndim == 0 else len(y0[0])
        self.pre_lin_list = nn.ModuleList(
            [nn.Linear(data.num_features if i == 0 else dim1, dim1) for i in range(pre_fc_count)])
        for name in lists:
            setattr(self, name, nn.ModuleList())

    def _add_bn(self, dim):
        if self.batch_norm == "True":
            self.bn_list.append(BatchNorm1d(dim, track_running_stats=self.batch_track_stats))

    def _finish(self, dim2, post_fc_count, post_in, early_mult=1, set2set_names=("set2set",)):
        s2s_early = self.pool == "set2set" and self.pool_order == "early"
        if self.pool_order == "early":
            first_in = post_in * ((2 * early_mult - 1) if (s2s_early and early_mult > 1) else (2 if s2s_early else early_mult))
        else:
            first_in = post_in
        self.post_lin_list = nn.ModuleList(
            [nn.Linear(first_in if i == 0 else dim2, dim2) for i in range(post_fc_count)])
        self.lin_out = nn.Linear(dim2 if post_fc_count > 0 else first_in, self.output_dim)
        if s2s_early:
            for name in set2set_names:
                setattr(self, name, Set2Set(post_in, processing_steps=3))
        elif self.pool == "set2set" and self.pool_order == "late":
            setattr(self, set2set_names[0], Set2Set(self.output_dim, processing_steps=3, num_layers=1))
            self.lin_out_2 = nn.Linear(self.output_dim * 2, self.output_dim)
        if self.split_products:
            from ..nn import use_split_linears
            use_split_linears(self)

    def _inputs(self, data):
        cd = self.compute_dtype
        n = data.x.shape[0]
        csr = getattr(data, "csr", None)
        if csr is None:
            csr = ops.csr_for(data.edge_index, n)
        return data.x.to(cd), data.edge_attr.to(cd), csr

    def _cast_dense(self, dtype):
        lins = getattr(self, "_dense_layers", None)
        if lins is None:
            lins = [m for m in self.modules() if isinstance(m, nn.Linear)]
            object.__setattr__(self, "_dense_layers", lins)
        params = [p for lin in lins for p in (lin.weight, lin.bias) if p is not None]
        if not params or not params[0].is_cuda or params[0].dtype == dtype:
            return
        cache = getattr(self, "_lowp_cache", None)
        if cache is None or len(cache) != len(params) or cache[0].dtype != dtype or cache[0].device != params[0].device:
            cache = [torch.empty_like(p, dtype=dtype) for p in params]
            self._lowp_cache = cache
        with torch.no_grad():
            torch._foreach_copy_(cache, [p.detach() for p in params])
        k = 0
        for lin in lins:
            w = cache[k]; k += 1
            b = None
            if lin.bias is not None:
                b = cache[k]; k += 1
            lin._mdl_lowp = (w, b, lin.weight._version, None if lin.bias is None else lin.bias._version)

    def _open_grad_arena(self, device):
        n = getattr(self, "_arena_floats", None)
        if n is None:
            R = ops.bn_sums_rows()
            n = sum(p.numel() + 128 for m in self.modules() if isinstance(m, nn.Linear) for p in (m.weight, m.bias) if p is not None)
            n += sum(R * m.num_features + 128 for m in self.modules() if isinstance(m, (BatchNorm1d, nn.BatchNorm1d)))
            object.__setattr__(self, "_arena_floats", n)
        ops.new_grad_arena(device, n)

    def _pre(self, out):
        if torch.is_grad_enabled() and out.is_cuda:
            self._open_grad_arena(out.device)
        if out.dtype == torch.bfloat16 and torch.is_grad_enabled():
            self._cast_dense(out.dtype)
        for lin in self.pre_lin_list:
            out = dense_act(lin, out, self.act, split=self.split_products)
        return out

    def _bn(self, i, out):
        return self.bn_list[i](out) if self.batch_norm == "True" else out

    def _drop(self, out):
        return F.dropout(out, p=self.dropout_rate, training=self.training)

    def _post(self, out, final=False):
        lins = list(self.post_lin_list) + [self.lin_out]
        if out.dtype != self.lin_out.weight.dtype and ops.mlp_head_ok(out, lins, self.act):
            return ops.mlp_head(out, lins, [_lowp(lin) for lin in lins], f32_out=final)
        for lin in self.post_lin_list:
            out = dense_act(lin, out, self.act, split=self.split_products)
        return dense(self.lin_out, out)

    def _pool(self, out, data):
        num_graphs = getattr(data, "num_graphs", None)
        if self.pool == "set2set":
            return self.set2set(out, data.batch, num_graphs)
        return ops.POOLS[self.pool](out, data.batch, num_graphs, seg_index=getattr(data, "pool_index", None))

    def _head(self, out, data):
        if self.pool_order == "early":
            out = self._post(self._pool(out, data).to(out.dtype), final=True)
        else:
            out = self._post(out)
            if self.pool == "set2set":
                out = dense(self.lin_out_2, self._pool(out, data).to(out.dtype))
            else:
                out = self._pool(out, data)
        out = out.float()
        return out.view(-1) if out.shape[1] == 1 else out
```

matdeeplearn_amd/models/cgcnn.py:

```python
import torch
from torch import nn

from .. import ops
from ..nn import CGConv
from ._base import GraphModel


class CGCNN(GraphModel):
    needs_by_source = False

    def __init__(self, data, dim1=64, dim2=64, pre_fc_count=1, gc_count=3, post_fc_count=1,
                 pool="global_mean_pool", pool_order="early", batch_norm="True", batch_track_stats="True",
                 act="relu", dropout_rate=0.0, compute_dtype="fp32", **kwargs):
        super().__init__()
        self._begin(data, dim1, pre_fc_count, gc_count, pool, pool_order, batch_norm, batch_track_stats, act,
                    dropout_rate, compute_dtype)
        for _ in range(gc_count):
            self.conv_list.append(CGConv(self.gc_dim, data.num_edge_features, aggr="mean", batch_norm=False))
            self._add_bn(self.gc_dim)
        self._finish(dim2, post_fc_count, self.gc_dim)

    def forward(self, data):
        x, edge_attr, csr = self._inputs(data)
        out = self._pre(x)
        bn_on = self.batch_norm == "True"
        packs = ops.cgconv_prepack(list(self.conv_list), out.dtype, out.device, want_node=torch.is_grad_enabled()) if out.is_cuda else None
        dist = getattr(data, "dist", None)
        for i, conv in enumerate(self.conv_list):
            prev = self.bn_list[i - 1].bias if (bn_on and i > 0) else None
            out = self._drop(conv(out, None, edge_attr, csr=csr, bn=self.bn_list[i] if bn_on else None, bn_shift=prev,
                                  packed=None if packs is None else packs[i], split=self.split_products, dist=dist))
        return self._head(out, data)
```

matdeeplearn_amd/nn.py:

```python
from torch import nn

from . import ops


class CGConv(nn.Module):

    def __init__(self, channels, dim=0, aggr="add", batch_norm=False, bias=True, **kwargs):
        super().__init__()
        if isinstance(channels, (tuple, list)):
            if channels[0] != channels[1]:
                raise ops.MdlError("CGConv: bipartite channel pairs are not on the reference path")
            channels = channels[0]
        if batch_norm:
            raise ops.MdlError("CGConv(batch_norm=True) is not used by the reference (cgcnn.py:81)")
        self.channels, self.dim, self.aggr = channels, dim, aggr
        self.lin_f = nn.Linear(2 * channels + dim, channels, bias=bias)
        self.lin_s = nn.Linear(2 * channels + dim, channels, bias=bias)
        self.reset_parameters()

    def reset_parameters(self):
        self.lin_f.reset_parameters()
        self.lin_s.reset_parameters()

    def forward(self, x, edge_index, edge_attr=None, csr=None, bn=None, bn_shift=None, packed=None, split=False, dist=None):
# ... 195 lines not shown
        n = x.shape[0]
        if edge_weight is None:
            edge_weight = torch.ones(csr.E, device=x.device)
        ew = edge_weight.float()
        deg = ops.scatter(ew.unsqueeze(1), csr.col, 0, n, "sum").squeeze(1)
        dis = deg.pow(-0.5)
        dis = torch.where(torch.isinf(dis), torch.zeros_like(dis), dis)
        norm = ops.gather(dis.unsqueeze(1), csr.row).squeeze(1) * ew * ops.gather(dis.unsqueeze(1), csr.col).squeeze(1)
        out = ops.gather_mul_reduce(_lin(self.lin, x), csr, w=None, scale=norm, reduce="sum")
        return out + self.bias.to(out.dtype) if self.bias is not None else out


class NNConv(nn.Module):
    def __init__(self, in_channels, out_channels, nn_module, aggr="add", root_weight=True, bias=True, chunk=32768):
        super().__init__()
        self.in_channels, self.out_channels, self.aggr, self.chunk = in_channels, out_channels, aggr, chunk
        self.nn = nn_module
        self.lin = nn.Linear(in_channels, out_channels, bias=False) if root_weight else None
        self.bias = nn.Parameter(torch.zeros(out_channels)) if bias else None
        self.reset_parameters()

    def reset_parameters(self):
        for m in self.nn.modules():
            if m is not self.nn and hasattr(m, "reset_parameters"):
                m.reset_parameters()
        if self.lin is not None:
            self.lin.reset_parameters()
        if self.bias is not None:
            self.bias.data.zero_()

    def _messages(self, xj, edge_attr):
        w = self.nn(edge_attr).view(-1, self.in_channels, self.out_channels)
        return torch.bmm(xj.unsqueeze(1), w).squeeze(1)

    def _last_linear(self):
        last = self.nn[-1] if isinstance(self.nn, nn.Sequential) and len(self.nn) > 0 else None
        if isinstance(last, nn.Linear) and last.out_features == self.in_channels * self.out_channels:
            return last
        return None

    def forward(self, x, edge_index, edge_attr, csr=None, dist=None):
        from torch.utils.checkpoint import checkpoint
        if csr is None:
            csr = ops.csr_for(edge_index, x.shape[0])
        last = self._last_linear()
        ci, co = self.in_channels, self.out_channels
        if last is not None and (co * (last.in_features + 1) + last.in_features + co) * 4 <= 160 * 1024:
            hdn = _seq(list(self.nn)[:-1], edge_attr, dist=dist)
            d3 = last.in_features
            w2 = last.weight.view(ci, co * d3).to(x.dtype)
            Y = ops.matmul_wide(x, w2)
            m = ops.nnconv_msg(Y, hdn.to(x.dtype), csr, co)
            linear_aggr = self.aggr in ("mean", "add", "sum")
            if last.bias is not None and not linear_aggr:
                m = m + ops.gather(x @ last.bias.view(ci, co).to(x.dtype), csr.row)
            out = ops.scatter(m, csr.col, 0, x.shape[0], self.aggr)
            if last.bias is not None and linear_aggr:
                out = out + ops.gather_mul_reduce(x @ last.bias.view(ci, co).to(x.dtype), csr, reduce=self.aggr)
            if self.lin is not None:
                out = out + _lin(self.lin, x)
            if self.bias is not None:
                out = out + self.bias.to(out.dtype)
            return out
        if dist is not None and torch.is_grad_enabled() and dist[0].requires_grad:
            edge_attr = ops.expansion_of(dist, edge_attr.dtype)
        xj = ops.gather(x, csr.row)
        parts = []
        for s in range(0, csr.E, self.chunk):
            a, b = xj[s:s + self.chunk], edge_attr[s:s + self.chunk]
            parts.append(checkpoint(self._messages, a, b, use_reentrant=False) if torch.is_grad_enabled()
                         else self._messages(a, b))
        m = torch.cat(parts) if parts else xj.new_zeros((0, self.out_channels))
        out = ops.scatter(m, csr.col, 0, x.shape[0], self.aggr)
        if self.lin is not None:
            out = out + self.lin(x)
        if self.bias is not None:
            out = out + self.bias.to(out.dtype)
        return out


class MetaLayer(nn.Module):
    def __init__(self, edge_model=None, node_model=None, global_model=None):
        super().__init__()
        self.edge_model, self.node_model, self.global_model = edge_model, node_model, global_model

    def forward(self, x, edge_index, edge_attr=None, u=None, batch=None):
        row, col = edge_index[0], edge_index[1]
        if self.edge_model is not None:
            edge_attr = self.edge_model(ops.gather(x, row), ops.gather(x, col), edge_attr, u,
                                        batch if batch is None else batch.index_select(0, row))
        if self.node_model is not None:
            x = self.node_model(x, edge_index, edge_attr, u, batch)
        if self.global_model is not None:
            u = self.global_model(x, edge_index, edge_attr, u, batch)
        return x, edge_attr, u


class Set2Set(nn.Module):
    def __init__(self, in_channels, processing_steps, num_layers=1):
        super().__init__()
        self.in_channels, self.out_channels = in_channels, 2 * in_channels
        self.processing_steps, self.num_layers = processing_steps, num_layers
        self.lstm = nn.LSTM(self.out_channels, in_channels, num_layers)
        self.lstm.reset_parameters()

    def forward(self, x, batch, size=None):
        b = int(batch.max()) + 1 if size is None else size
        xf = x.float()
        h = (xf.new_zeros((self.num_layers, b, self.in_channels)), xf.new_zeros((self.num_layers, b, self.in_channels)))
        q_star = xf.new_zeros(b, self.out_channels)
        for _ in range(self.processing_steps):
            q, h = self.lstm(q_star.unsqueeze(0), h)
            q = q.view(b, self.in_channels)
            e = (xf * ops.gather(q, batch)).sum(dim=-1, keepdim=True)
            emax = ops.gather(ops.scatter(e, batch, 0, b, "max", assume_sorted=True).detach(), batch)
            a = torch.exp(e - emax)
            a = a / (ops.gather(ops.scatter(a, batch, 0, b, "sum", assume_sorted=True), batch) + 1e-16)
            r = ops.scatter(a * xf, batch, 0, b, "sum", assume_sorted=True)
            q_star = torch.cat([q, r], dim=-1)
        return q_star


class BatchNorm1d(nn.BatchNorm1d):

    def _sync_counter(self):
        pending = getattr(self, "_nbt_pending", 0)
        if pending and self.num_batches_tracked is not None:
            self.num_batches_tracked.add_(pending)
        self._nbt_pending = 0

    def forward(self, x):
        use_batch_stats = self.training or not self.track_running_stats
        if use_batch_stats and x.dim() == 2 and ops.bn_supported(x) and self.momentum is not None:
            rm = rv = None
            if self.training and self.track_running_stats:
                rm, rv = self.running_mean, self.running_var
                self._nbt_pending = getattr(self, "_nbt_pending", 0) + 1
            return ops.batch_norm_train(x, self.weight, self.bias, rm, rv, self.eps, self.momentum)
        self._sync_counter()
        return super().forward(x)

    def after_cgconv(self, conv, x, edge_index, edge_attr, csr, shift=None, packed=None):
        use_batch_stats = self.training or not self.track_running_stats
        if not (use_batch_stats and self.momentum is not None and self.num_features == x.shape[1] and ops.bn_supported(x)
                and ops.cgconv_bn_stats_ok(x, edge_attr, csr)):
            return None
        rm = rv = None
        if self.training and self.track_running_stats:
            rm, rv = self.running_mean, self.running_var
            self._nbt_pending = getattr(self, "_nbt_pending", 0) + 1
        return ops.cgconv_bn(x, edge_index, edge_attr, conv.lin_f.weight, conv.lin_f.bias, conv.lin_s.weight, conv.lin_s.bias,
                             conv.aggr, csr, self.weight, self.bias, rm, rv, self.eps, self.momentum, shift, packed)

    def after_linear_relu(self, h, weight, bias, lowp=None, gathered=None):
        use_batch_stats = self.training or not self.track_running_stats
        if not (use_batch_stats and self.momentum is not None and ops.linear_relu_bn_ok(h, weight, bias is not None, gathered)):
            return None
        rm = rv = None
        if self.training and self.track_running_stats:
            rm, rv = self.running_mean, self.running_var
            self._nbt_pending = getattr(self, "_nbt_pending", 0) + 1
        return ops.linear_relu_bn(h, weight, bias, lowp, self.weight, self.bias, rm, rv, self.eps, self.momentum, gathered)

    def _save_to_state_dict(self, destination, prefix, keep_vars):
        self._sync_counter()
        super()._save_to_state_dict(destination, prefix, keep_vars)

    def _load_from_state_dict(self, *args, **kwargs):
        self._nbt_pending = 0
        super()._load_from_state_dict(*args, **kwargs)
```

matdeeplearn_amd/ops.py:

```python
import collections
import os

import torch

from . import _lib
from ._lib import MdlError, check, dtype_code, lib, ptr, require_hip, stream

_ACT_CODE = {"relu": 1, "ssp": 2}
_LN2 = 0.6931471805599453


def _f32c(t):
    return None if t is None else t.detach().float().contiguous()


def _stream_key(device):
    return (device.index, torch.cuda.current_stream(device).cuda_stream)


class EdgeCSR:

    __slots__ = ("rowptr", "src", "tgt", "eperm", "N", "E", "_row", "_col", "_t", "_attr", "_tb", "_bal", "partial", "__weakref__")

    def __init__(self, rowptr, src, tgt, eperm, N, E, row=None, col=None):
# ... 362 lines not shown
    if ev is None or key not in ev:
        return fn()
    a, b = torch.cuda.Event(enable_timing=True), torch.cuda.Event(enable_timing=True)
    a.record()
    rc = fn()
    b.record()
    ev[key].append((a, b))
    return rc


class ZeroArena:

    def __init__(self, device, nbytes=4 << 20):
        self.buf = torch.empty(nbytes // 4, dtype=torch.float32, device=device)
        self.off = 0

    def reset(self):
        self.buf.zero_()
        self.off = 0

    def take(self, shape):
        n = 1
        for d in shape:
            n *= int(d)
        n_al = (n + 63) & ~63
        if self.off + n_al > self.buf.numel():
            return None
        t = self.buf[self.off:self.off + n].view(*shape)
        self.off += n_al
        return t


_ARENA = None

_GRAD_ARENA = None


def new_grad_arena(device, nfloats):
    global _GRAD_ARENA
    _GRAD_ARENA = [torch.zeros(int(nfloats), dtype=torch.float32, device=device), 0]


def _zeros_grad(n, device):
    a = _GRAD_ARENA
    n_al = (int(n) + 63) & ~63
    if a is not None and a[0].device == device and a[1] + n_al <= a[0].numel():
        t = a[0][a[1]:a[1] + int(n)]
        a[1] += n_al
        return t
    return torch.zeros(int(n), dtype=torch.float32, device=device)


class zero_arena:
    def __init__(self, device, nbytes=4 << 20):
        self.key = (torch.device(device), nbytes)

    _cache = {}

    def __enter__(self):
        global _ARENA
        a = zero_arena._cache.get(self.key)
        if a is None:
            a = zero_arena._cache[self.key] = ZeroArena(*self.key)
        a.reset()
        self.prev, _ARENA = _ARENA, a
        return a

    def __exit__(self, *exc):
        global _ARENA
        _ARENA = self.prev
        return False


def _zeros_step(shape, device):
    a = _ARENA
    if a is not None and a.buf.device == device:
        t = a.take(shape)
        if t is not None:
            return t
    return torch.zeros(shape, dtype=torch.float32, device=device)


_WS = {}


def _workspace(device, nbytes):
    key = _stream_key(device)
    t = _WS.get(key)
    if t is None or t.numel() < nbytes:
        t = _WS[key] = torch.empty(max(int(nbytes), 256), dtype=torch.uint8, device=device)
    return t


_TN_SCRATCH = True
_TNS = {}


_TN_SCRATCH_MIN_ROWS = 4096
_DENSE_MIN_ROWS = 64


def _tn_scratch(device, rows=None):
    if not _TN_SCRATCH or (rows is not None and rows < _TN_SCRATCH_MIN_ROWS):
        return None
    key = _stream_key(device)
    t = _TNS.get(key)
    if t is None:
        t = _TNS[key] = torch.empty(lib().mdl_tn_scratch_bytes(), dtype=torch.uint8, device=device)
    return t


def _gemm_tn(a, lda, M, y, ldy, act, b, ldb, K, c, colsum, N, flags, device):
    return lib().mdl_gemm_tn_ex(ptr(a), lda, M, ptr(y), ldy, act, ptr(b), ldb, K, ptr(c), ptr(colsum), ptr(_tn_scratch(device, N)), N, flags,
                                stream())


_DET = False


def set_deterministic(on=True):
    global _DET
    prev, _DET = _DET, bool(on)
    return prev


class deterministic:
    def __init__(self, on=True):
        self.on = on

    def __enter__(self):
        self.prev = set_deterministic(self.on)
        return self

    def __exit__(self, *exc):
        set_deterministic(self.prev)
        return False


OPTIONS = {
    "deterministic": ("_DET", "bit-reproducible launch shapes of every atomically accumulating kernel (slow; HIP-vs-HIP tests)"),
    "gmr_dw": ("_GMR_DW", "CFConv backward: dh and dw from one walk over the by-source CSR"),
    "balance": ("_BALANCE", "cost-balanced node ranges for the edge-per-lane CGConv backward (E >= 4e5)"),
    "pad128": ("_PAD128", "C in (96, 128): static 128-channel CGConv kernels on zero-padded rows"),
    "rsrc16": ("_RSRC16", "by-source sums of the CGConv backward in bf16 (packed atomics)"),
    "cg_bn_stats": ("_CG_BN_STATS", "BatchNorm statistics in the CGConv forward's epilogue (measured time-neutral: off)"),
    "direct_grads": ("_DIRECT_GRADS", "K3 / K3c add into the final dW layout (measured slower at small batches: off)"),
    "cfconv_fused": ("_CFCONV_FUSED", "K4: the fused CFConv forward"),
    "cfconv_recompute": ("_CFCONV_RECOMPUTE", "K4b: CFConv backward with the filter recomputed (no per-edge activations)"),
    "tn_colsum": ("_TN_COLSUM", "bias gradients out of the TN GEMM"),
    "dense_bwd": ("_DENSE_BWD", "dX + dW + db of a tall dense layer in one pass"),
    "dense_bwd_wide": ("_DENSE_BWD_WIDE", "... also when both widths exceed 128"),
    "mlp_head": ("_MLP_HEAD", "post-FC head as one launch per direction"),
    "linear_wide": ("_LINEAR_WIDE", "NNConv's Y = x W2r on the streaming kernel"),
    "tn_scratch": ("_TN_SCRATCH", "weight-gradient blocks of the TN products as plain stores + a reduce launch (off: atomics from every workgroup)"),
}


def configure(**kw):
    prev = {}
    g = globals()
    for k, v in kw.items():
        if k not in OPTIONS:
            raise MdlError("ops.configure: unknown option %r (known: %s)" % (k, ", ".join(sorted(OPTIONS))))
        attr = OPTIONS[k][0]
        prev[k] = g[attr]
        g[attr] = bool(v)
    return prev


def options():
    return {k: globals()[a] for k, (a, _) in OPTIONS.items()}


def _dflag():
    return _lib.MDL_DETERMINISTIC if _DET else 0


K3_VARIANT = None


def _k3flag():
    return {None: 0, "per_wave": _lib.MDL_K3_PER_WAVE, "edge_lane": _lib.MDL_K3_EDGE_LANE}[K3_VARIANT]


def last_k3():
    return int(lib().mdl_debug_last_k3())


_GMR_DW = True
_BALANCE = True
_PAD128 = True
_RSRC16 = True


_RSRC = {}


_RSRC_CAP = {}


def _take_rsrc(nfloats, device):
    if torch.cuda.is_current_stream_capturing():
        owned = _RSRC_CAP.setdefault(device.index, [])
        for ent in owned:
            if ent[0].numel() >= nfloats and not ent[1]:
                return ent
        cand = [k for k, v in _RSRC.items() if k[0] == device.index and not v[1] and v[0].numel() >= nfloats]
        if not cand:
            return None
        ent = _RSRC.pop(max(cand, key=lambda k: _RSRC[k][0].numel()))
        owned.append(ent)
        return ent
    key = _stream_key(device)
    ent = _RSRC.get(key)
    if ent is None or ent[0].numel() < nfloats or ent[1]:
        ent = _RSRC[key] = [torch.zeros(int(nfloats), dtype=torch.float32, device=device), False]
    return ent


class _CGConvFn(torch.autograd.Function):
    @staticmethod
    def forward(ctx, x, edge_attr, w_f, b_f, w_s, b_s, csr, aggr, bn=None, packed=None, split=False, d_norm=None, rbf=None):
        require_hip(x, edge_attr, w_f, w_s)
        if edge_attr.dtype != x.dtype:
            raise MdlError("cgconv: x (%s) and edge_attr (%s) must share a dtype" % (x.dtype, edge_attr.dtype))
        x, edge_attr = x.contiguous(), edge_attr.contiguous()
        N, C = x.shape
        E, G = edge_attr.shape
        if csr.N != N or csr.E != E:
            raise MdlError("cgconv: CSR (%d nodes, %d edges) does not match x/edge_attr (%d, %d)" % (csr.N, csr.E, N, E))
        dt = dtype_code(x)
        L = lib()
        sp = _lib.MDL_SPLIT_BF16 if (split and dt == _lib.MDL_F32 and G == 50 and E > 0 and not _DET
                                     and ((C == 64 and x.data_ptr() % 16 == 0) or (_PAD128 and 96 < C <= 128))) else 0
        ctx.split = sp
        wf32, ws32, bf32, bs32 = _f32c(w_f), _f32c(w_s), _f32c(b_f), _f32c(b_s)
        nbytes = L.mdl_cgconv_wpack_bytes(C, G, dt | sp)
        if nbytes == 0:
            raise MdlError("cgconv: unsupported C=%d G=%d" % (C, G))
        Ck = C
        if _PAD128 and (dt == _lib.MDL_BF16 or sp) and G == 50 and 96 < C < 128 and (csr.eperm is None or sp) and E > 0:
            Ck = 128
            x = torch.nn.functional.pad(x, (0, Ck - C))
        use_packed = packed is not None and packed[3] == (C, G, dt)
        wn_t = None
        if use_packed:
            wpack, bpack, wn_t = packed[:3]
        elif dt == _lib.MDL_BF16 and (C in (32, 64) or Ck == 128) and any(ctx.needs_input_grad):
            wpack = torch.empty(nbytes, dtype=torch.uint8, device=x.device)
            bpack = torch.empty(2 * _rup(C, 32), dtype=torch.float32, device=x.device)
            wn_t = torch.empty((C, 4 * _rup(C, 32)), dtype=torch.bfloat16, device=x.device)
            check(L.mdl_cgconv_pack_weights_node(ptr(wf32), ptr(bf32), ptr(ws32), ptr(bs32), C, G, ptr(wpack), ptr(bpack),
                                                 ptr(wn_t), dt, stream()), "mdl_cgconv_pack_weights_node")
        else:
            wpack, bpack = _plain_pack(wf32, bf32, ws32, bs32, C, G, dt | sp, x.device, nbytes)
        ctx.wn_t = wn_t
        out = torch.empty_like(x)
        edge_attr = csr.sorted_attr(edge_attr)
        bn_sums, bn_shift = bn if bn is not None else (None, None)
        args = _lib.cg_args(dtype=dt, flags=sp, aggr=aggr, N=N, E=E, C=Ck, G=G, x=x, edge_attr=edge_attr, rowptr=csr.rowptr, src=csr.src,
                            tgt=csr.tgt, wpack=wpack, bpack=bpack, out=out, bn_sums=bn_sums, bn_shift=bn_shift,
                            bn_rows=_true_rows_for(N) if bn_sums is not None else None)
        check(_launch_timed("fwd", lambda: L.mdl_cgconv_fwd_ex(args, stream())), "mdl_cgconv_fwd_ex")
        dist_saved = () if d_norm is None else (d_norm.detach().contiguous(), rbf[0].contiguous())
        ctx.save_for_backward(x, edge_attr, wf32, ws32, wpack, bpack, *dist_saved)
        ctx.rbf_coeff = None if d_norm is None else float(rbf[1])
        ctx.bias32 = (bf32, bs32)
        ctx.csr, ctx.aggr, ctx.has_bias = csr, aggr, (b_f is not None, b_s is not None)
        ctx.wdtypes = (w_f.dtype, w_s.dtype)
        ctx.C = C
        return out if Ck == C else out[:, :C].contiguous()

    @staticmethod
    @torch.autograd.function.once_differentiable
    def backward(ctx, g):
        need_de = ctx.needs_input_grad[1]
        need_dd = len(ctx.needs_input_grad) > 11 and ctx.needs_input_grad[11] and ctx.rbf_coeff is not None
        de, dd = _cgconv_edge_grads(ctx, g, need_de, need_dd) if (need_de or need_dd) else (None, None)
        grads = _CGConvFn._backward_main(ctx, g)
        return grads[:1] + (de,) + grads[2:] + (dd, None)

    @staticmethod
    def _backward_main(ctx, g):
        x, edge_attr, wf32, ws32, wpack, bpack = ctx.saved_tensors[:6]
        csr = ctx.csr
        N, Ck = x.shape
        C = ctx.C
        E, G = edge_attr.shape
        Cp, GP = _rup(C, 32), _rup(G, 64)
        g = g.contiguous()
        dt = dtype_code(x)
        xk, gk = x, g
        if Ck != C:
            gk = torch.nn.functional.pad(g, (0, Ck - C))
            x = x[:, :C]
        r_tgt = torch.empty((N, 2 * Cp), dtype=x.dtype, device=x.device)
        sp = ctx.split
        node_x3 = bool(sp) and dt == _lib.MDL_F32 and C == 64
        node_hip = (dt == _lib.MDL_BF16 and C == Cp and C in (32, 64)) or node_x3
        rs16 = (_RSRC16 and dt == _lib.MDL_BF16 and (node_hip or Ck == 128) and G == 50 and E > 0
                and x.data_ptr() % 16 == 0 and edge_attr.data_ptr() % 4 == 0)
        nrs = N * 2 * Cp // 2 if rs16 else N * 2 * Cp
        keep = _take_rsrc(nrs, x.device) if node_hip else None
        if keep is not None:
            r_src, keep[1] = keep[0][:nrs], True
            r_src = r_src.view(torch.bfloat16).view(N, 2 * Cp) if rs16 else r_src.view(N, 2 * Cp)
        else:
            r_src = torch.zeros((N, 2 * Cp), dtype=torch.bfloat16 if rs16 else torch.float32, device=x.device)
        ldw = 2 * C + G
        direct = node_hip and _DIRECT_GRADS
        if direct:
            gbuf = _zeros_grad(2 * C * ldw + 2 * C, x.device)
            dW = gbuf[:2 * C * ldw].view(2 * C, ldw)
            db = gbuf[2 * C * ldw:]
            dwe, dwn, ld_dwe = dW[:, 2 * C:], dW, ldw
        else:
            small = _zeros_step((2 * Cp * GP + 2 * Cp + 4 * Cp * C,), x.device)
            dwe = small[:2 * Cp * GP].view(2 * Cp, GP)
            db = small[2 * Cp * GP:2 * Cp * GP + 2 * Cp]
            dwn = small[2 * Cp * GP + 2 * Cp:].view(4 * Cp, C)
            ld_dwe = 0
        ws = _workspace(x.device, lib().mdl_cgconv_workspace_bytes(N, E, C, G, dt))
        fl = _dflag()
        bal = csr.balance() if (rs16 and _BALANCE and E >= 400000 and not fl) else None
        eargs = _lib.cg_args(dtype=dt, flags=fl | (_k3flag() if rs16 else 0) | sp, aggr=ctx.aggr, N=N, E=E, C=Ck, G=G, x=xk, edge_attr=edge_attr,
                             rowptr=csr.rowptr, src=csr.src, tgt=csr.tgt, wpack=wpack, bpack=bpack, grad_out=gk, r_tgt=r_tgt, r_src=r_src,
                             r_src_dtype=_lib.MDL_BF16 if rs16 else _lib.MDL_F32, dwe=dwe, ld_dwe=ld_dwe, db=db, workspace=ws,
                             workspace_bytes=ws.numel(), balance=bal)
        check(_launch_timed("bwd", lambda: lib().mdl_cgconv_bwd_ex(eargs, stream())), "mdl_cgconv_bwd_ex")
        if node_hip:
            wn_t = _node_weights(ctx, C, Cp, torch.float32 if node_x3 else torch.bfloat16, x.device, wf32, ws32)
            dx = torch.empty_like(x)
            nargs = _lib.cg_node_args(dtype=dt, flags=fl | (sp if node_x3 else 0), zero_src=1 if keep is not None else 0, N=N, C=C,
                                      r_src_dtype=_lib.MDL_BF16 if rs16 else _lib.MDL_F32, ld_dwn=ldw if direct else 0, x=x, grad_out=g,
                                      r_tgt=r_tgt, r_src=r_src, wn_t=wn_t, dx=dx, dwn=dwn)
            check(_launch_timed("bwd_node", lambda: lib().mdl_cgconv_bwd_node_ex(nargs, stream())), "mdl_cgconv_bwd_node_ex")
            if keep is not None:
                keep[1] = False
            if direct:
                dW_f, dW_s = dW[:C], dW[C:]
                db_f = db[:C].to(ctx.wdtypes[0]) if ctx.has_bias[0] else None
                db_s = db[C:].to(ctx.wdtypes[1]) if ctx.has_bias[1] else None
            else:
                dW_f, db_f, dW_s, db_s = _assemble_grads(ctx, dwn, dwe, db, C, G, x.device, timed=True)
        elif dt == _lib.MDL_BF16 and Cp == 128 and C % 2 == 0 and N > 0:
            rs_b = r_src.to(torch.bfloat16)
            wn_t = _node_weights(ctx, C, Cp, torch.bfloat16, x.device, wf32, ws32)
            dx = torch.addmm(g, r_tgt, wn_t[:, :2 * Cp].t())
            dx.addmm_(rs_b, wn_t[:, 2 * Cp:].t())
            xc = x.contiguous()
            for blk, r in enumerate((r_tgt[:, :Cp], r_tgt[:, Cp:], rs_b[:, :Cp], rs_b[:, Cp:])):
                check(_gemm_tn(r, r.stride(0), Cp, None, 0, 0, xc, xc.stride(0), C, dwn[blk * Cp:(blk + 1) * Cp], None, N, dt | fl,
                               x.device), "mdl_gemm_tn")
            dW_f, db_f, dW_s, db_s = _assemble_grads(ctx, dwn, dwe, db, C, G, x.device, timed=False)
        else:
            Wn = torch.cat([wf32[:, :C], ws32[:, :C], wf32[:, C:2 * C], ws32[:, C:2 * C]], dim=0)
            rt = r_tgt.view(N, 2, Cp)[:, :, :C]
            rs = r_src.view(N, 2, Cp)[:, :, :C]
            cd = torch.float32 if dt == _lib.MDL_F32 else torch.bfloat16
            R = torch.cat([rt[:, 0], rt[:, 1], rs[:, 0], rs[:, 1]], dim=1).to(cd)
            dx = torch.addmm(g, R, Wn.to(cd))
            dWn = torch.mm(R.t(), x).float()
            dW_f = torch.cat([dWn[0:C], dWn[2 * C:3 * C], dwe[:C, :G]], dim=1)
            dW_s = torch.cat([dWn[C:2 * C], dWn[3 * C:4 * C], dwe[Cp:Cp + C, :G]], dim=1)
            db_f = db[:C].clone() if ctx.has_bias[0] else None
            db_s = db[Cp:Cp + C].clone() if ctx.has_bias[1] else None
        return dx, None, dW_f.to(ctx.wdtypes[0]), db_f, dW_s.to(ctx.wdtypes[1]), db_s, None, None, None, None, None


def _node_weights(ctx, C, Cp, dtype, device, wf32, ws32):
    wn_t, ctx.wn_t = ctx.wn_t, None
    if wn_t is None:
        wn_t = torch.empty((C, 4 * Cp), dtype=dtype, device=device)
        check(lib().mdl_cgconv_pack_node_weights(ptr(wf32), ptr(ws32), C, wf32.shape[1] - 2 * C, ptr(wn_t), dtype_code(wn_t), stream()),
              "mdl_cgconv_pack_node_weights")
    return wn_t


def _assemble_grads(ctx, dwn, dwe, db, C, G, device, timed):
    dW_f = torch.empty((C, 2 * C + G), dtype=torch.float32, device=device)
    dW_s = torch.empty_like(dW_f)
    db_f = torch.empty(C, dtype=torch.float32, device=device) if ctx.has_bias[0] else None
    db_s = torch.empty(C, dtype=torch.float32, device=device) if ctx.has_bias[1] else None
    launch = lambda: lib().mdl_cgconv_assemble_grads(ptr(dwn), ptr(dwe), ptr(db), C, G, ptr(dW_f), ptr(dW_s), ptr(db_f), ptr(db_s), stream())
    check(_launch_timed("bwd_grads", launch) if timed else launch(), "mdl_cgconv_assemble_grads")
    return dW_f, db_f, dW_s, db_s


def cgconv_prepack(convs, x_dtype, device, want_node=True):
    import ctypes
    if len(convs) < 2 or len(convs) > 16 or device.type != "cuda":
        return None
    C, G = convs[0].channels, convs[0].dim
    dt = _lib.MDL_BF16 if x_dtype == torch.bfloat16 else _lib.MDL_F32
    if any(c.channels != C or c.dim != G or c.lin_f.weight.dtype != torch.float32 or not c.lin_f.weight.is_contiguous()
           or not c.lin_s.weight.is_contiguous() or (c.lin_f.bias is None) != (convs[0].lin_f.bias is None) for c in convs):
        return None
    if not (dt == _lib.MDL_BF16 and (C in (32, 64) or (_PAD128 and G == 50 and 96 < C < 128))):
        return None
    L = lib()
    nbytes = L.mdl_cgconv_wpack_bytes(C, G, dt)
    if nbytes == 0:
        return None
    n = len(convs)
    wbuf = torch.empty((n, nbytes), dtype=torch.uint8, device=device)
    bbuf = torch.empty((n, 2 * _rup(C, 32)), dtype=torch.float32, device=device)
    nbuf = torch.empty((n, C, 4 * _rup(C, 32)), dtype=torch.bfloat16, device=device) if want_node else None
    tab = lambda ts: (ctypes.c_void_p * n)(*[None if t is None else t.data_ptr() for t in ts])
    has_b = convs[0].lin_f.bias is not None
    check(L.mdl_cgconv_pack_weights_multi(
        n, tab([c.lin_f.weight.detach() for c in convs]), tab([c.lin_f.bias.detach() for c in convs]) if has_b else None,
        tab([c.lin_s.weight.detach() for c in convs]), tab([c.lin_s.bias.detach() for c in convs]) if has_b else None, C, G,
        tab(list(wbuf)), tab(list(bbuf)), tab(list(nbuf)) if want_node else None, dt, stream()), "mdl_cgconv_pack_weights_multi")
    return [(wbuf[k], bbuf[k], nbuf[k] if want_node else None, (C, G, dt)) for k in range(n)]


def cgconv(x, edge_index, edge_attr, w_f, b_f, w_s, b_s, aggr="mean", csr=None, bn_stats=None, packed=None, split=False, dist=None):
    if aggr not in ("mean", "add", "sum"):
        raise MdlError("cgconv: aggr must be mean or add")
    if csr is None:
        csr = csr_for(edge_index, x.shape[0])
    if dist is None:
        return _CGConvFn.apply(x, edge_attr, w_f, b_f, w_s, b_s, csr, _lib.REDUCE[aggr], bn_stats, packed, split)
    d_norm, offsets, coeff = _check_dist("cgconv", dist, edge_attr, "edge_attr")
    return _CGConvFn.apply(x, edge_attr, w_f, b_f, w_s, b_s, csr, _lib.REDUCE[aggr], bn_stats, packed, split, d_norm,
                           (offsets.float(), float(coeff)))


def _check_dist(name, dist, edge_attr, what):
    d_norm, offsets, coeff = dist
    require_hip(d_norm, offsets)
    if d_norm.dtype != torch.float32 or d_norm.numel() != edge_attr.shape[0] or offsets.numel() != edge_attr.shape[1]:
        raise MdlError("%s: dist = (d_norm [E] float32, offsets [G], coeff) must match %s %s" % (name, what, tuple(edge_attr.shape)))
    return d_norm, offsets, coeff


def _dist_grad_inputs(name, x, edge_index, d_norm, csr, start, stop, resolution, width, edge_attr, out):
    if csr is None:
        csr = csr_for(edge_index, x.shape[0])
    if d_norm.dtype != torch.float32 or d_norm.numel() != csr.E or csr.N != x.shape[0]:
        raise MdlError("%s: d_norm must be [E] float32 over the CSR's %d edges" % (name, csr.E))
    if out is not None and csr.eperm is not None:
        raise MdlError("%s: out= needs an edge list in CSR (target-sorted) order" % name)
    offsets = rbf_offsets(start, stop, resolution, x.device)
    d_sorted = _sort_edges(d_norm, csr).contiguous()
    if edge_attr is None:
        ea = rbf_expand(d_sorted.detach(), start, stop, resolution, width, out_dtype=x.dtype, offsets=offsets)
    else:
        ea = csr.sorted_attr(edge_attr.detach().contiguous())
    return csr, offsets, d_sorted, ea


def _bwd_edge_launch(x, ea_sorted, csr, wpack, bpack, g, aggr, C, G, de=None, d_sorted=None, offsets=None, coeff=0.0, scale=1.0, dd=None):
    check(_launch_timed("bwd_edge", lambda: lib().mdl_cgconv_bwd_edge(
        ptr(x), ptr(ea_sorted), ptr(csr.rowptr), ptr(csr.src), ptr(csr.tgt), ptr(wpack), ptr(bpack), ptr(g), x.shape[0], ea_sorted.shape[0],
        C, G, aggr, dtype_code(x), ptr(de), ptr(d_sorted), ptr(offsets), float(coeff), float(scale), ptr(dd), stream())),
        "mdl_cgconv_bwd_edge")


def _plain_pack(wf32, bf32, ws32, bs32, C, G, dt, device, nbytes=None):
    wpack = torch.empty(lib().mdl_cgconv_wpack_bytes(C, G, dt) if nbytes is None else nbytes, dtype=torch.uint8, device=device)
    bpack = torch.empty(2 * _rup(C, 32), dtype=torch.float32, device=device)
    check(lib().mdl_cgconv_pack_weights(ptr(wf32), ptr(bf32), ptr(ws32), ptr(bs32), C, G, ptr(wpack), ptr(bpack), dt, stream()),
          "mdl_cgconv_pack_weights")
    return wpack, bpack


def _unsort_edges(t, csr):
    if csr.eperm is None:
        return t
    out = torch.empty_like(t)
    out[csr.eperm.long()] = t
    return out


def _cgconv_edge_grads(ctx, g, need_de, need_dd):
    saved = ctx.saved_tensors
    x, edge_attr, wf32, ws32, wpack, bpack = saved[:6]
    csr = ctx.csr
    C = ctx.C
    E, G = edge_attr.shape
    dt = dtype_code(x)
    if x.shape[1] != C:
        x = x[:, :C].contiguous()
    g = g.contiguous()
    if ctx.split:
        wpack, bpack = _plain_pack(wf32, ctx.bias32[0], ws32, ctx.bias32[1], C, G, dt, x.device)
    de = dd = None
    if need_de:
        de = (torch.zeros if csr.partial else torch.empty)((E, G), dtype=edge_attr.dtype, device=x.device)
        _bwd_edge_launch(x, edge_attr, csr, wpack, bpack, g, ctx.aggr, C, G, de=de)
        de = _unsort_edges(de, csr)
    if need_dd:
        d_norm, offsets = saved[6], saved[7]
        d_sorted = _sort_edges(d_norm, csr)
        dd = torch.zeros(E, dtype=torch.float32, device=x.device)
        _bwd_edge_launch(x, edge_attr, csr, wpack, bpack, g, ctx.aggr, C, G, d_sorted=d_sorted, offsets=offsets, coeff=ctx.rbf_coeff, dd=dd)
        dd = _unsort_edges(dd, csr)
    return de, dd


def cgconv_dist_grad(x, edge_index, d_norm, w_f, b_f, w_s, b_s, grad_out, aggr="mean", csr=None, start=0.0, stop=1.0, resolution=50,
                     width=0.2, scale=1.0, edge_attr=None, out=None):
    if aggr not in ("mean", "add", "sum"):
        raise MdlError("cgconv_dist_grad: aggr must be mean or add")
    require_hip(x, d_norm, w_f, w_s, grad_out)
    with torch.no_grad():
        C, G, dt = x.shape[1], int(resolution), dtype_code(x)
        if lib().mdl_cgconv_wpack_bytes(C, G, dt) == 0:
            raise MdlError("cgconv_dist_grad: unsupported C=%d G=%d" % (C, G))
        csr, offsets, d_sorted, ea = _dist_grad_inputs("cgconv_dist_grad", x, edge_index, d_norm, csr, start, stop, G, width, edge_attr, out)
        wpack, bpack = _plain_pack(_f32c(w_f), _f32c(b_f), _f32c(w_s), _f32c(b_s), C, G, dt, x.device)
        dd = out if out is not None else torch.zeros(csr.E, dtype=torch.float32, device=x.device)
        _bwd_edge_launch(x.detach().contiguous(), ea, csr, wpack, bpack, grad_out.detach().to(x.dtype).contiguous(), _lib.REDUCE[aggr], C, G,
                         d_sorted=d_sorted, offsets=offsets, coeff=rbf_coeff(start, stop, width), scale=scale, dd=dd)
        return dd if out is not None else _unsort_edges(dd, csr)


_CG_BN_STATS = False
_DIRECT_GRADS = False


def cgconv_bn_stats_ok(x, edge_attr, csr):
    return (_CG_BN_STATS and not _DET and x.is_cuda and x.dtype == torch.bfloat16 and edge_attr.dtype == torch.bfloat16 and x.dim() == 2
            and x.shape[1] in (32, 64) and edge_attr.shape[1] == 50 and csr.eperm is None and csr.E > 0 and x.shape[0] >= 2
            and x.is_contiguous() and x.data_ptr() % 16 == 0 and edge_attr.data_ptr() % 4 == 0)


def cgconv_bn(x, edge_index, edge_attr, w_f, b_f, w_s, b_s, aggr, csr, bn_weight, bn_bias, running_mean, running_var, eps, momentum,
              shift=None, packed=None):
    C = x.shape[1]
    R = lib().mdl_bn_sums_rows()
    buf = _zeros_step((R + 3, C), x.device)
    y = cgconv(x, edge_index, edge_attr, w_f, b_f, w_s, b_s, aggr, csr=csr, bn_stats=(buf, _f32c(shift)), packed=packed)
    return _BatchNormTrain.apply(y, bn_weight, bn_bias, running_mean, running_var, eps, momentum, buf)


class _Gather(torch.autograd.Function):
    @staticmethod
    def forward(ctx, src, index):
        require_hip(src, index)
        src = src.contiguous()
        idx = index.to(torch.int32).contiguous()
        C = src.numel() // max(src.shape[0], 1)
        out = torch.empty((idx.numel(),) + tuple(src.shape[1:]), dtype=src.dtype, device=src.device)
        check(lib().mdl_gather_rows(ptr(src), ptr(idx), ptr(out), idx.numel(), C, dtype_code(src), stream()),
              "mdl_gather_rows")
        ctx.index, ctx.n = index, src.shape[0]
        return out

    @staticmethod
    def backward(ctx, g):
        return scatter(g, ctx.index, 0, ctx.n, "sum"), None


def gather(src, index):
    return _Gather.apply(src, index)


class _GatherMulReduce(torch.autograd.Function):
    @staticmethod
    def forward(ctx, h, w, scale, csr, reduce, pre=None):
        require_hip(h)
        h = h.contiguous()
        N, F = csr.N, h.shape[1]
        if w is not None:
            w = w.contiguous()
            if w.dtype != h.dtype:
                raise MdlError("gather_mul_reduce: h and w must share a dtype")
        if scale is not None:
            scale = scale.float().contiguous()
        if pre is not None:
            out = pre.view_as(pre)
        else:
            out = torch.empty((N, F), dtype=h.dtype, device=h.device)
            check(_launch_timed("gmr_fwd", lambda: lib().mdl_gather_mul_reduce(
                ptr(h), ptr(w), ptr(scale), ptr(csr.rowptr), ptr(csr.src), ptr(csr.eperm), ptr(out), N, F, reduce, dtype_code(h),
                stream())), "mdl_gather_mul_reduce")
        ctx.csr, ctx.reduce = csr, reduce
        ctx.save_for_backward(h, w, scale)
        return out

    @staticmethod
    def backward(ctx, g):
        h, w, scale = ctx.saved_tensors
        csr = ctx.csr
        g = g.contiguous()
        if ctx.reduce == _lib.MDL_MEAN:
            deg = (csr.rowptr[1:] - csr.rowptr[:-1]).clamp(min=1).to(g.dtype)
            g = g / deg.unsqueeze(1)
        dh = dw = None
        if scale is not None and ctx.needs_input_grad[2]:
            dscale = torch.empty(csr.E, dtype=torch.float32, device=h.device)
            check(lib().mdl_edge_dot(ptr(g), ptr(csr.col), ptr(h), ptr(csr.row), ptr(w), ptr(dscale), csr.E, h.shape[1],
                                     dtype_code(h), stream()), "mdl_edge_dot")
            dh, dw = _gmr_dh_dw(ctx, g, h, w, scale, csr)
            return dh, dw, dscale, None, None, None
        if (w is not None and ctx.needs_input_grad[0] and ctx.needs_input_grad[1] and _GMR_DW and h.dtype == torch.bfloat16
                and h.shape[1] % 2 == 0 and h.shape[1] <= 512 and scale is not None):
            rowptr_s, col_s, eid_s, _ = csr.transposed()
            dh = torch.empty_like(h)
            dw = (torch.zeros_like if _true_rows_for(w.shape[0]) is not None else torch.empty_like)(w)
            check(lib().mdl_gather_mul_reduce_dw(ptr(g), ptr(w), ptr(scale), ptr(rowptr_s), ptr(col_s), ptr(eid_s), ptr(dh), ptr(h),
                                                 ptr(dw), csr.N, h.shape[1], dtype_code(h), stream()), "mdl_gather_mul_reduce_dw")
            return dh, dw, None, None, None, None
        dh, dw = _gmr_dh_dw(ctx, g, h, w, scale, csr)
        return dh, dw, None, None, None, None


def _gmr_dh_dw(ctx, g, h, w, scale, csr):
    dh = dw = None
    if ctx.needs_input_grad[0]:
        rowptr_s, col_s, eid_s, _ = csr.transposed()
        dh = torch.empty_like(h)
        check(lib().mdl_gather_mul_reduce(ptr(g), ptr(w), ptr(scale), ptr(rowptr_s), ptr(col_s), ptr(eid_s),
                                          ptr(dh), csr.N, h.shape[1], _lib.MDL_SUM, dtype_code(h), stream()),
              "mdl_gather_mul_reduce(T)")
    if w is not None and ctx.needs_input_grad[1]:
        dw = torch.empty_like(w)
        check(lib().mdl_edge_mul(ptr(h), ptr(csr.row), ptr(g), ptr(csr.col), ptr(scale), ptr(dw), csr.E,
                                 h.shape[1], dtype_code(h), stream()), "mdl_edge_mul")
    return dh, dw


def gather_mul_reduce(h, csr, w=None, scale=None, reduce="sum", pre=None):
    return _GatherMulReduce.apply(h, w, scale, csr, _lib.REDUCE[reduce], pre)


_CFCONV_FUSED = True
_CFCONV_RECOMPUTE = True
_CFCONV_RECOMPUTE_MIN_F = 96


def cfconv_fused_ok(rbf, h, csr, lin_a, lin_b):
    if not (_CFCONV_FUSED and rbf.is_cuda and rbf.dtype == torch.bfloat16 and h.dtype == torch.bfloat16 and rbf.dim() == 2
            and h.dim() == 2 and rbf.is_contiguous() and csr.eperm is None and rbf.shape[0] == csr.E):
        return False
    F, G = h.shape[1], rbf.shape[1]
    if tuple(lin_a.weight.shape) != (F, G) or tuple(lin_b.weight.shape) != (F, F):
        return False
    for t in (lin_a.weight, lin_b.weight, lin_a.bias, lin_b.bias):
        if t is not None and (t.dtype != torch.float32 or not t.is_contiguous() or not t.is_cuda):
            return False
    if not lib().mdl_cfconv_supported(F, G, dtype_code(h)):
        return False
    if torch.is_grad_enabled() and (lin_a.weight.requires_grad or lin_b.weight.requires_grad or h.requires_grad):
        return (linear_act_fused_ok(rbf, lin_a.weight, "ssp") and _hip_shape_ok(F, F) and rbf.shape[0] >= _DENSE_MIN_ROWS
                and lin_a.weight.requires_grad and lin_b.weight.requires_grad)
    return True


def cfconv_fused(rbf, cut, h, csr, lin_a, lin_b, want_acts):
    require_hip(rbf, h)
    F, G = h.shape[1], rbf.shape[1]
    E, N = csr.E, csr.N
    dev = h.device
    wpack = _cfconv_pack(lin_a.weight, lin_a.bias, lin_b.weight, lin_b.bias, F, G, dev)
    out = torch.empty((N, F), dtype=h.dtype, device=dev)
    a1 = torch.empty((E, F), dtype=h.dtype, device=dev) if want_acts else None
    w = torch.empty((E, F), dtype=h.dtype, device=dev) if want_acts else None
    h = h.contiguous()
    _cfconv_fwd_launch("cfconv_fwd", rbf, cut.float().contiguous(), h, csr.rowptr, csr.src, csr.tgt, wpack, N, E, out, a1, w)
    return out, a1, w


def _cfconv_pack(w1, b1, w2, b2, F, G, device):
    wpack = torch.empty(lib().mdl_cfconv_wpack_bytes(), dtype=torch.uint8, device=device)
    check(lib().mdl_cfconv_pack_weights(ptr(w1), ptr(b1), ptr(w2), ptr(b2), F, G, ptr(wpack), stream()), "mdl_cfconv_pack_weights")
    return wpack


def _cfconv_fwd_launch(key, rbf, cut, x, rowptr, src, tgt, wpack, N, E, out, a1=None, w=None):
    F, G = x.shape[1], rbf.shape[1]
    check(_launch_timed(key, lambda: lib().mdl_cfconv_fwd(
        ptr(rbf), ptr(cut), ptr(x), ptr(rowptr), ptr(src), ptr(tgt), ptr(wpack), ptr(out), ptr(a1), ptr(w), N, E, F, G,
        dtype_code(out), stream())), "mdl_cfconv_fwd" if key == "cfconv_fwd" else "mdl_cfconv_fwd(T)")


def _cfconv_param_grads(rbf, cut, h, g, csr, wpack, has_b):
    F, G = h.shape[1], rbf.shape[1]
    buf = torch.zeros(F * G + F * F + 2 * F, dtype=torch.float32, device=h.device)
    dw1, dw2 = buf[:F * G].view(F, G), buf[F * G:F * G + F * F].view(F, F)
    db1 = buf[F * G + F * F:F * G + F * F + F] if has_b[0] else None
    db2 = buf[F * G + F * F + F:] if has_b[1] else None
    scratch = torch.empty(lib().mdl_cfconv_bwd_w_scratch_bytes(), dtype=torch.uint8, device=h.device)
    check(_launch_timed("cfconv_bwd_w", lambda: lib().mdl_cfconv_bwd_w(
        ptr(rbf), ptr(cut), ptr(h), ptr(g), ptr(csr.rowptr), ptr(csr.src), ptr(csr.tgt), ptr(wpack), ptr(dw1), ptr(db1),
        ptr(dw2), ptr(db2), ptr(scratch), csr.N, csr.E, F, G, dtype_code(h) | _dflag(), stream())), "mdl_cfconv_bwd_w")
# ... 723 lines not shown
    return torch.nn.functional.linear(x, weight.to(x.dtype), None if bias is None else bias.to(x.dtype))


class _GRUGates(torch.autograd.Function):

    @staticmethod
    def forward(ctx, gi, gh, h):
        N, C3 = gi.shape
        C = C3 // 3
        gi, gh, h = gi.contiguous(), gh.contiguous(), h.contiguous()
        h_new = torch.empty((N, C), dtype=torch.float32, device=gi.device)
        lp = gi.dtype != torch.float32
        out = torch.empty((N, C), dtype=gi.dtype, device=gi.device) if lp else None
        check(lib().mdl_gru_gates_fwd(ptr(gi), ptr(gh), ptr(h), ptr(h_new), ptr(out), N, C, dtype_code(gi), stream()), "mdl_gru_gates_fwd")
        ctx.save_for_backward(gi, gh, h)
        ctx.lp = lp
        if lp:
            return h_new, out
        dummy = h_new.new_empty(0)
        ctx.mark_non_differentiable(dummy)
        return h_new, dummy

    @staticmethod
    def backward(ctx, g_h, g_out):
        gi, gh, h = ctx.saved_tensors
        N, C3 = gi.shape
        C = C3 // 3
        if not ctx.lp:
            g_out = None
        g_h = None if g_h is None else g_h.contiguous().float()
        g_out = None if g_out is None else g_out.contiguous().to(gi.dtype)
        if g_h is None and g_out is None:
            return None, None, None
        dgi, dgh = torch.empty_like(gi), torch.empty_like(gh)
        dh = torch.empty_like(h)
        check(lib().mdl_gru_gates_bwd(ptr(gi), ptr(gh), ptr(h), ptr(g_h), ptr(g_out), ptr(dgi), ptr(dgh), ptr(dh), N, C,
                                      dtype_code(gi), stream()), "mdl_gru_gates_bwd")
        return dgi, dgh, dh


def gru_gates_ok(gi, gh, h):
    return (gi.is_cuda and gi.dim() == 2 and gi.shape == gh.shape and gi.dtype == gh.dtype and gi.dtype in (torch.float32, torch.bfloat16)
            and gi.shape[1] % 3 == 0 and h.dtype == torch.float32 and h.shape == (gi.shape[0], gi.shape[1] // 3) and gi.shape[0] > 0)


def gru_gates(gi, gh, h):
    h_new, out = _GRUGates.apply(gi, gh, h)
    return (h_new, out) if gi.dtype != torch.float32 else (h_new, h_new)


_UNIT = {}


def unit_grad(device):
    device = torch.device(device)
    key = (device.type, device.index if device.index is not None else torch.cuda.current_device())
    t = _UNIT.get(key)
    if t is None:
        t = _UNIT[key] = torch.ones((), dtype=torch.float32, device=device)
    return t


def backward(loss):
    if loss.is_cuda and loss.dtype == torch.float32 and loss.dim() == 0:
        loss.backward(gradient=unit_grad(loss.device))
    else:
        loss.backward()


def _is_unit(g):
    t = _UNIT.get((g.device.type, g.device.index))
    return t is not None and g.data_ptr() == t.data_ptr() and g.dim() == 0


class _FusedLoss(torch.autograd.Function):
    @staticmethod
    def forward(ctx, pred, target, kind, rows, buf):
        p = pred.contiguous()
        y = target.contiguous()
        out = torch.empty(1 + p.numel(), dtype=torch.float32, device=p.device) if buf is None else buf[:1 + p.numel()]
        if rows is None:
            check(lib().mdl_loss_fwd_bwd(ptr(p), ptr(y), p.numel(), kind, ptr(out), ptr(out[1:]), stream()), "mdl_loss_fwd_bwd")
        else:
            check(lib().mdl_loss_fwd_bwd_rows(ptr(p), ptr(y), int(rows), p.numel(), kind, ptr(out), ptr(out[1:]), stream()),
                  "mdl_loss_fwd_bwd_rows")
        ctx.save_for_backward(out)
        ctx.shape = tuple(pred.shape)
        return out[0]

    @staticmethod
    def backward(ctx, g):
        (out,) = ctx.saved_tensors
        grad = out[1:] if _is_unit(g) else out[1:] * g
        return grad.view(ctx.shape), None, None, None, None


def loss(name, pred, target, rows=None, buf=None):
    if buf is not None and not (buf.is_cuda and buf.dtype == torch.float32 and buf.is_contiguous() and buf.dim() == 1
                                and buf.numel() >= 1 + pred.numel() and buf.device == pred.device):
        buf = None
    kind = {"l1_loss": 0, "mse_loss": 1}.get(name)
    if rows is not None:
        rows = int(rows)
        if (kind is not None and pred.is_cuda and pred.dtype == torch.float32 and target.dtype == torch.float32 and pred.dim() == 1
                and target.dim() == 1 and target.numel() == rows and 1 <= rows <= pred.numel() and not target.requires_grad):
            return _FusedLoss.apply(pred, target, kind, rows, buf)
        pred = pred[:rows]
    if (kind is not None and pred.is_cuda and pred.dtype == torch.float32 and target.dtype == torch.float32
            and pred.shape == target.shape and pred.numel() >= 1 and not target.requires_grad):
        return _FusedLoss.apply(pred, target, kind, None, buf)
    return getattr(torch.nn.functional, name)(pred, target)


def bn_supported(x):
    if not (x.is_cuda and x.dim() == 2 and x.is_contiguous() and x.dtype in (torch.float32, torch.bfloat16)):
        return False
    c = x.shape[1]
    w = 8 if (x.dtype == torch.bfloat16 and c % 8 == 0) else 4
    return x.shape[0] >= 2 and c % 4 == 0 and 4 <= c <= 256 and x.data_ptr() % (w * x.element_size()) == 0


_TRUE_ROWS = None


def _true_rows_for(nrows):
    tr = _TRUE_ROWS
    if tr is None:
        return None
    if isinstance(tr, dict):
        return tr.get(int(nrows))
    return tr


class true_rows:

    def __init__(self, n_dev):
        self.n_dev = n_dev

    def __enter__(self):
        global _TRUE_ROWS
        self.prev, _TRUE_ROWS = _TRUE_ROWS, self.n_dev
        return self

    def __exit__(self, *exc):
        global _TRUE_ROWS
        _TRUE_ROWS = self.prev
        return False


def bn_sums_rows():
    return int(lib().mdl_bn_sums_rows())


class _BatchNormTrain(torch.autograd.Function):
    @staticmethod
    def forward(ctx, x, weight, bias, running_mean, running_var, eps, momentum, pre=None):
        N, C = x.shape
        dt = dtype_code(x)
        R = lib().mdl_bn_sums_rows()
        buf = _zeros_step((R + 2, C), x.device) if pre is None else pre
        sums, save = buf[:R], buf[-2:]
        gw, gb = _f32c(weight), _f32c(bias)
        y = torch.empty_like(x)
        nd = _true_rows_for(N)
        if pre is None:
            check(lib().mdl_bn_stats_n(ptr(x), ptr(sums), N, C, ptr(nd), dt | _dflag(), stream()), "mdl_bn_stats")
        check(lib().mdl_bn_apply_n(ptr(x), ptr(sums), ptr(gw), ptr(gb), ptr(save), ptr(running_mean), ptr(running_var),
                                   ptr(y), N, C, float(eps), float(momentum), ptr(nd),
                                   dt | (_lib.MDL_BN_SHIFT_ROW if pre is not None else 0), stream()), "mdl_bn_apply")
        ctx.n_dev = nd
        ctx.save_for_backward(x, save, gw)
        ctx.has = (weight is not None, bias is not None)
        ctx.wdt = None if weight is None else weight.dtype
        return y

    @staticmethod
    def backward(ctx, dy):
        x, save, gw = ctx.saved_tensors
        N, C = x.shape
        dy = dy.contiguous()
        dt = dtype_code(x)
        R = lib().mdl_bn_sums_rows()
        sums = _zeros_grad(R * C, x.device).view(R, C)
        dx = torch.empty_like(x)
        nd = ctx.n_dev
        check(lib().mdl_bn_bwd_stats_n(ptr(dy), ptr(x), ptr(save), ptr(sums), N, C, ptr(nd), dt | _dflag(), stream()), "mdl_bn_bwd_stats")
        check(lib().mdl_bn_bwd_apply_n(ptr(dy), ptr(x), ptr(save), ptr(sums), ptr(gw), ptr(dx), N, C, ptr(nd), dt, stream()),
              "mdl_bn_bwd_apply")
        dgamma = sums[R - 1].to(ctx.wdt) if ctx.has[0] else None
        dbeta = sums[R - 2].to(ctx.wdt) if ctx.has[1] else None
        return dx, dgamma, dbeta, None, None, None, None, None


class _LinearReluBN(torch.autograd.Function):

    @staticmethod
    def forward(ctx, x, weight, bias, w_lp, b_lp, bn_w, bn_b, rm, rv, eps, momentum, idx, *tables):
        w = weight.to(x.dtype) if w_lp is None else w_lp
        b = None if bias is None else (bias.to(x.dtype) if b_lp is None else b_lp)
        N, K = x.shape
        M = weight.shape[0]
        dt = dtype_code(x)
        y = torch.empty((N, M), dtype=x.dtype, device=x.device)
        tabs = [None if t is None else t.contiguous() for t in tables]
        tb = tabs + [None] * (3 - len(tabs))
        ids = list(idx) + [None] * (3 - len(idx))
        R = lib().mdl_bn_sums_rows()
        buf = _zeros_step((R + 3, M), x.device)
        sums, save = buf[:R], buf[R + 1:]
        nd = _true_rows_for(N)
        in_epilogue = not _DET and len(tabs) in (0, 2) and K <= 160
        if in_epilogue:
            launch = lambda: lib().mdl_linear_act_stats(
                ptr(x), ptr(w), ptr(b), ptr(tb[0]), ptr(ids[0]), ptr(tb[1]), ptr(ids[1]), ptr(tb[2]), ptr(ids[2]), ptr(y),
                N, K, M, 1, ptr(sums), ptr(nd), dt, stream())
            check(_launch_timed("edge_linear", launch) if tabs else launch(), "mdl_linear_act_stats")
        elif tabs:
            check(_launch_timed("edge_linear", lambda: lib().mdl_linear_gather_act(
                ptr(x), ptr(w), ptr(b), ptr(tb[0]), ptr(ids[0]), ptr(tb[1]), ptr(ids[1]), ptr(tb[2]), ptr(ids[2]), ptr(y),
                N, K, M, 1, dt, stream())), "mdl_linear_gather_act")
        else:
            check(lib().mdl_linear_act(ptr(x), ptr(w), ptr(b), ptr(y), N, K, M, 1, dt, stream()), "mdl_linear_act")
        gw, gb = _f32c(bn_w), _f32c(bn_b)
        z = torch.empty_like(y)
        if not in_epilogue:
            check(lib().mdl_bn_stats_n(ptr(y), ptr(sums), N, M, ptr(nd), dt | _dflag(), stream()), "mdl_bn_stats")
        check(lib().mdl_bn_apply_n(ptr(y), ptr(sums), ptr(gw), ptr(gb), ptr(save), ptr(rm), ptr(rv), ptr(z), N, M, float(eps),
                                   float(momentum), ptr(nd), dt | (_lib.MDL_BN_SHIFT_ROW if in_epilogue else 0), stream()),
              "mdl_bn_apply")
        ctx.save_for_backward(x, w, y, save, gw)
        ctx.n_dev, ctx.idx, ctx.rows, ctx.ntab = nd, list(idx), [None if t is None else t.shape[0] for t in tabs], len(tabs)
        ctx.wdtype, ctx.has_bias, ctx.shape = weight.dtype, bias is not None, tuple(weight.shape)
        ctx.bn_has = (bn_w is not None, bn_b is not None)
        ctx.bn_wdt = None if bn_w is None else bn_w.dtype
        return z

    @staticmethod
    def backward(ctx, gz):
        x, w, y, save, gw = ctx.saved_tensors
        M, K = ctx.shape
        N = x.shape[0]
        gz = gz.contiguous()
        dt = dtype_code(x)
        R = lib().mdl_bn_sums_rows()
        sums = _zeros_grad(R * M, x.device).view(R, M)
        gp = torch.empty_like(y)
        check(lib().mdl_bn_bwd_stats_n(ptr(gz), ptr(y), ptr(save), ptr(sums), N, M, ptr(ctx.n_dev), dt | _dflag(), stream()),
              "mdl_bn_bwd_stats")
        check(lib().mdl_bn_bwd_apply_relu_n(ptr(gz), ptr(y), ptr(save), ptr(sums), ptr(gw), ptr(gp), N, M, ptr(ctx.n_dev), dt,
                                            stream()), "mdl_bn_bwd_apply_relu")
        dgamma = sums[R - 1].to(ctx.bn_wdt) if ctx.bn_has[0] else None
        dbeta = sums[R - 2].to(ctx.bn_wdt) if ctx.bn_has[1] else None
        buf = _zeros_grad(M * K + M, x.device)
        dw, dbv = buf[:M * K].view(M, K), buf[M * K:]
        dx = torch.empty((N, K), dtype=x.dtype, device=x.device)
        check(lib().mdl_dense_bwd_ex(ptr(gp), M, M, None, 0, 0, ptr(x), x.stride(0), K, ptr(w), ptr(dx), K, 0, None, ptr(dw),
                                     ptr(dbv) if ctx.has_bias else None, ptr(_tn_scratch(x.device, N)), N, dt | _dflag(), stream()),
              "mdl_dense_bwd")
        dts = []
        for t in range(ctx.ntab):
            need = ctx.needs_input_grad[12 + t] and ctx.rows[t] is not None
            dts.append(scatter(gp, ctx.idx[t], 0, ctx.rows[t], "sum") if need else None)
        return (dx if ctx.needs_input_grad[0] else None, dw.to(ctx.wdtype), dbv.to(ctx.wdtype) if ctx.has_bias else None,
                None, None, dgamma, dbeta, None, None, None, None, None) + tuple(dts)


def linear_relu_bn_ok(x, weight, has_bias, gathered=None):
    M, K = weight.shape
    kb = K + (1 if has_bias else 0)
    return (_DENSE_BWD and x.dtype == torch.bfloat16 and x.is_cuda and x.dim() == 2 and x.is_contiguous() and x.shape[0] >= _DENSE_MIN_ROWS
            and x.requires_grad and torch.is_grad_enabled() and weight.requires_grad
            and 34 <= M <= (128 if gathered else 160) and 34 <= K and kb <= 160 and M % 2 == 0 and K % 2 == 0
            and not (M > 128 and kb > 128) and M % 4 == 0 and x.data_ptr() % 16 == 0 and (gathered is None or len(gathered) <= 3))


def linear_relu_bn(x, weight, bias, lowp, bn_weight, bn_bias, running_mean, running_var, eps, momentum, gathered=None):
    w_lp, b_lp = (lowp if lowp is not None and lowp[0].dtype == x.dtype else (None, None))
    gathered = gathered or []
    idx = [ix if ix.dtype == torch.int32 else ix.to(torch.int32) for _, ix in gathered]
    return _LinearReluBN.apply(x, weight, bias, w_lp, b_lp, bn_weight, bn_bias, running_mean, running_var, eps, momentum, idx,
                               *[t.to(x.dtype) for t, _ in gathered])


def batch_norm_train(x, weight, bias, running_mean, running_var, eps=1e-5, momentum=0.1):
    return _BatchNormTrain.apply(x, weight, bias, running_mean, running_var, eps, momentum)


GRAPH_MAX_NEIGHBORS = 64


def _graph_args(pos, node_ptr, cell, pbc):
    require_hip(pos, node_ptr, cell, pbc)
    if pos.dtype != torch.float64 or pos.dim() != 2 or pos.shape[1] != 3:
        raise MdlError("build_graphs: pos must be [N, 3] float64 (got %s %s)" % (tuple(pos.shape), pos.dtype))
    if node_ptr.dtype != torch.int64 or node_ptr.dim() != 1 or node_ptr.numel() < 2:
        raise MdlError("build_graphs: node_ptr must be [G + 1] int64 with G >= 1")
    G = node_ptr.numel() - 1
    if cell.dtype != torch.float64 or tuple(cell.shape) != (G, 3, 3):
        raise MdlError("build_graphs: cell must be [G, 3, 3] float64 (got %s %s)" % (tuple(cell.shape), cell.dtype))
    if pbc.dim() == 2 and tuple(pbc.shape) == (G, 3):
        pbc = (pbc.to(torch.int32) * torch.tensor([1, 2, 4], dtype=torch.int32, device=pbc.device)).sum(1, dtype=torch.int32)
    if pbc.dtype != torch.int32 or tuple(pbc.shape) != (G,):
        raise MdlError("build_graphs: pbc must be a [G] int32 bitmask or [G, 3] booleans")
    return pos.contiguous(), node_ptr.contiguous(), cell.contiguous(), pbc.contiguous(), G


def _build_graphs_launch(pos, node_ptr, cell, pbc, G, radius, max_neighbors):
    N, k, dev = pos.shape[0], int(max_neighbors), pos.device
    nbytes = lib().mdl_graph_workspace_bytes(N, G, k)
    ws = torch.empty(max(nbytes, 1), dtype=torch.uint8, device=dev)
    cap = N * (k + 1) if 1 <= k <= GRAPH_MAX_NEIGHBORS else 1
    edge_ptr = torch.empty(G + 1, dtype=torch.int64, device=dev)
    src = torch.empty(cap, dtype=torch.int32, device=dev)
    tgt = torch.empty(cap, dtype=torch.int32, device=dev)
    dist = torch.empty(cap, dtype=torch.float32, device=dev)
    out_deg = torch.empty(N, dtype=torch.int32, device=dev)
    check(lib().mdl_graph_build(ptr(pos), ptr(node_ptr), ptr(cell), ptr(pbc), N, G, float(radius), k, ptr(edge_ptr), ptr(src),
                                ptr(tgt), ptr(dist), ptr(out_deg), cap, ptr(ws), nbytes, stream()), "mdl_graph_build")
    return edge_ptr, src, tgt, dist, out_deg


def build_graphs(pos, node_ptr, cell, pbc, radius=8.0, max_neighbors=12):
    pos, node_ptr, cell, pbc, G = _graph_args(pos, node_ptr, cell, pbc)
    N = pos.shape[0]
    if N < 1:
        raise MdlError("build_graphs: no atoms")
    bad = (node_ptr[0] != 0) | (node_ptr[-1] != N) | (node_ptr[1:] < node_ptr[:-1]).any()
    if bool(bad):
        raise MdlError("build_graphs: node_ptr must start at 0, be non-decreasing and end at N = %d" % N)
    edge_ptr, src, tgt, dist, out_deg = _build_graphs_launch(pos, node_ptr, cell, pbc, G, radius, max_neighbors)
    E = int(edge_ptr[-1])
    return edge_ptr, src[:E], tgt[:E], dist[:E], out_deg


class _EdgeVectors(torch.autograd.Function):
    @staticmethod
    def forward(ctx, pos, node_ptr, cell, pbc, src, tgt, csr):
        N, G, E = pos.shape[0], node_ptr.numel() - 1, src.numel()
        dist = torch.empty(E, dtype=torch.float32, device=pos.device)
        u = torch.empty((E, 3), dtype=torch.float32, device=pos.device)
        nbytes = lib().mdl_edge_geometry_workspace_bytes(G)
        ws = torch.empty(max(nbytes, 8), dtype=torch.uint8, device=pos.device)
        check(lib().mdl_edge_geometry_fwd(ptr(pos), ptr(node_ptr), ptr(cell), ptr(pbc), N, G, ptr(src), ptr(tgt), E, ptr(dist), ptr(u),
                                          ptr(ws), nbytes, stream()), "mdl_edge_geometry_fwd")
        ctx.save_for_backward(u, src, tgt)
        ctx.csr, ctx.N, ctx.pos_dtype = csr, N, pos.dtype
        ctx.mark_non_differentiable(u)
        return dist, u

    @staticmethod
    @torch.autograd.function.once_differentiable
    def backward(ctx, g_dist, _g_u):
        u, src, tgt = ctx.saved_tensors
        csr = ctx.csr
        if csr is None:
            csr = build_csr(torch.stack([src, tgt]), ctx.N)
        rowptr_s, _, eid_s, _ = csr.transposed()
        dpos = torch.empty((ctx.N, 3), dtype=torch.float32, device=u.device)
        check(lib().mdl_edge_geometry_bwd(ptr(g_dist.float().contiguous()), ptr(u), ptr(csr.rowptr), ptr(csr.eperm), ptr(rowptr_s), ptr(eid_s),
                                          ctx.N, u.shape[0], ptr(dpos), stream()), "mdl_edge_geometry_bwd")
        return dpos.to(ctx.pos_dtype), None, None, None, None, None, None


def edge_vectors(pos, node_ptr, cell, pbc, src, tgt, edge_ptr=None, csr=None, return_unit=False):
    pos, node_ptr, cell, pbc, G = _graph_args(pos, node_ptr, cell, pbc)
    require_hip(src, tgt)
    if src.dtype != torch.int32 or tgt.dtype != torch.int32 or src.shape != tgt.shape or src.dim() != 1:
        raise MdlError("edge_vectors: src / tgt must be [E] int32")
    if pos.shape[0] < 1:
        raise MdlError("edge_vectors: no atoms")
    if edge_ptr is not None:
        shift = torch.repeat_interleave(node_ptr[:-1], edge_ptr[1:] - edge_ptr[:-1], output_size=src.numel()).to(torch.int32)
        src, tgt = src + shift, tgt + shift
    if csr is not None and (csr.N != pos.shape[0] or csr.E != src.numel()):
        raise MdlError("edge_vectors: csr does not match the edge list")
    dist, u = _EdgeVectors.apply(pos, node_ptr, cell, pbc, src.contiguous(), tgt.contiguous(), csr)
    return (dist, u) if return_unit else dist


def edge_strain_grad(g_dist, dist, u, node_ptr, csr=None, src=None, tgt=None, _slices=None):
    require_hip(g_dist, dist, u, node_ptr)
    E = dist.numel()
    if dist.dtype != torch.float32 or dist.dim() != 1 or u.dtype != torch.float32 or tuple(u.shape) != (E, 3):
        raise MdlError("edge_strain_grad: dist must be [E] float32 and u [E, 3] float32 (got %s %s, %s %s)"
                       % (tuple(dist.shape), dist.dtype, tuple(u.shape), u.dtype))
    if not g_dist.is_floating_point() or tuple(g_dist.shape) != (E,):
        raise MdlError("edge_strain_grad: g_dist must be [E] floating point with E = %d (got %s %s)" % (E, tuple(g_dist.shape), g_dist.dtype))
    if node_ptr.dtype != torch.int64 or node_ptr.dim() != 1 or node_ptr.numel() < 2:
        raise MdlError("edge_strain_grad: node_ptr must be [G + 1] int64 with G >= 1")
    if any(t.device != dist.device for t in (g_dist, u, node_ptr)):
        raise MdlError("edge_strain_grad: g_dist, dist, u and node_ptr must be on one device")
    if csr is None:
        if src is None or tgt is None:
            raise MdlError("edge_strain_grad: needs the EdgeCSR of the edge list, or src / tgt to build it")
        require_hip(src, tgt)
        if src.dtype != torch.int32 or tgt.dtype != torch.int32 or tuple(src.shape) != (E,) or tuple(tgt.shape) != (E,):
            raise MdlError("edge_strain_grad: src / tgt must be [E] int32")
        csr = build_csr(torch.stack([src, tgt]), int(node_ptr[-1]))
    if csr.E != E or csr.rowptr.device != dist.device:
        raise MdlError("edge_strain_grad: csr does not match the edge list")
    S = 0 if _slices is None else int(_slices)
    if _slices is not None and not 1 <= S <= 65536:
        raise MdlError("edge_strain_grad: _slices must be in [1, 65536] (got %d)" % S)
    G = node_ptr.numel() - 1
    out = torch.empty((G, 3, 3), dtype=torch.float32, device=dist.device)
    nbytes = lib().mdl_edge_strain_grad_workspace_bytes(G, E, S)
    ws = torch.empty(max(nbytes, 8), dtype=torch.uint8, device=dist.device)
    check(lib().mdl_edge_strain_grad(ptr(g_dist.detach().float().contiguous()), ptr(dist.detach().contiguous()), ptr(u.contiguous()),
                                     ptr(csr.rowptr), ptr(csr.eperm), ptr(node_ptr.contiguous()), csr.N, G, E, S, ptr(out), ptr(ws),
                                     nbytes, stream()), "mdl_edge_strain_grad")
    return out
```

Measured before the change: 802.8 million.

## Fuse BN backward stats into cgconv node backward and fuse BN with mean-pool readout

The cgconv node-backward kernel gains a BN variant. It re-applies the preceding batch norm to the saved pre-BN activations, then accumulates the per-channel BN backward sums (sum of dy and dy*xhat) from the dx it just produced and pushes them into replica buffers with atomics. The BN backward then skips its own stats pass when the record matches its incoming gradient. A separate fused batchnorm plus mean-pool readout path with its own forward and backward kernels is also added, which avoids materialising the normalised node tensor before pooling. The cost is extra LDS, registers and atomics in the node kernel, plus version-based bookkeeping to check that the precomputed sums are still valid.

Measured after the change: 811.2 million (median of 6 runs). +1.0%, better.

```diff
diff --git a/include/mdl_hip.h b/include/mdl_hip.h
--- a/include/mdl_hip.h
+++ b/include/mdl_hip.h
@@ -115,6 +115,12 @@
     const void* wn_t;
     void* dx;
     float* dwn;
+    const void* bn_y;
+    const float* bn_save;
+    const float* bn_gamma;
+    const float* bn_beta;
+    float* bn_sums;
+    const int64_t* bn_nrows;
 } MdlCgNode;
 int mdl_cgconv_bwd_node_ex(const MdlCgNode* args, mdlStream_t stream);
 
@@ -174,6 +180,12 @@
                        int64_t N, int C, const int64_t* n_rows_dev, int dtype, mdlStream_t stream);
 int mdl_bn_bwd_apply_relu_n(const void* dy, const void* x, const float* save, float* sums, const float* gamma, void* dx,
                             int64_t N, int C, const int64_t* n_rows_dev, int dtype, mdlStream_t stream);
+int mdl_bn_meanpool_fwd(const void* y, float* sums, const float* gamma, const float* beta, float* save, float* running_mean,
+                        float* running_var, const int32_t* rowptr, void* pooled, float* mean_xhat, int64_t N, int C, int64_t G,
+                        float eps, float momentum, const int64_t* n_rows_dev, int dtype, mdlStream_t stream);
+int mdl_bn_meanpool_bwd(const void* grad_pooled, const void* y, const float* save, float* sums, const float* gamma,
+                        const int32_t* rowptr, const int32_t* seg, const float* mean_xhat, void* dx, int64_t N, int C, int64_t G,
+                        const int64_t* n_rows_dev, int dtype, mdlStream_t stream);
 int mdl_linear_act(const void* x, const void* w, const void* bias, void* out, int64_t N, int K, int M, int act, int dtype,
                    mdlStream_t stream);
 int mdl_linear_act_in(const void* x, const void* y, int xact, const void* w, const void* bias, void* out, int64_t N, int K,
diff --git a/matdeeplearn_amd/_lib.py b/matdeeplearn_amd/_lib.py
--- a/matdeeplearn_amd/_lib.py
+++ b/matdeeplearn_amd/_lib.py
@@ -36,7 +36,8 @@
 
 class MdlCgNode(ctypes.Structure):
     _fields_ = [("size", _u32), ("dtype", _i32), ("flags", _u32), ("zero_src", _i32), ("N", _i64), ("C", _i32), ("r_src_dtype", _i32),
-                ("ld_dwn", _i32), ("reserved", _i32), ("x", _vp), ("grad_out", _vp), ("r_tgt", _vp), ("r_src", _vp), ("wn_t", _vp), ("dx", _vp), ("dwn", _vp)]
+                ("ld_dwn", _i32), ("reserved", _i32), ("x", _vp), ("grad_out", _vp), ("r_tgt", _vp), ("r_src", _vp), ("wn_t", _vp), ("dx", _vp), ("dwn", _vp),
+                ("bn_y", _vp), ("bn_save", _vp), ("bn_gamma", _vp), ("bn_beta", _vp), ("bn_sums", _vp), ("bn_nrows", _vp)]
 
 
 def _dp(t):
@@ -94,6 +95,8 @@
     "mdl_bn_bwd_stats_n": (_i32, [_vp, _vp, _vp, _vp, _i64, _i32, _vp, _i32, _vp]),
     "mdl_bn_bwd_apply_n": (_i32, [_vp] * 6 + [_i64, _i32, _vp, _i32, _vp]),
     "mdl_bn_bwd_apply_relu_n": (_i32, [_vp] * 6 + [_i64, _i32, _vp, _i32, _vp]),
+    "mdl_bn_meanpool_fwd": (_i32, [_vp] * 10 + [_i64, _i32, _i64, _f32, _f32, _vp, _i32, _vp]),
+    "mdl_bn_meanpool_bwd": (_i32, [_vp] * 9 + [_i64, _i32, _i64, _vp, _i32, _vp]),
     "mdl_linear_act": (_i32, [_vp, _vp, _vp, _vp, _i64, _i32, _i32, _i32, _i32, _vp]),
     "mdl_dense_bwd": (_i32, [_vp, _i64, _i32, _vp, _i64, _i32, _vp, _i64, _i32, _vp, _vp, _i64, _i32, _vp, _vp, _vp, _i64, _i32, _vp]),
     "mdl_dense_bwd_ex": (_i32, [_vp, _i64, _i32, _vp, _i64, _i32, _vp, _i64, _i32, _vp, _vp, _i64, _i32, _vp, _vp, _vp, _vp, _i64, _i32, _vp]),
diff --git a/matdeeplearn_amd/csrc/bn.hip b/matdeeplearn_amd/csrc/bn.hip
--- a/matdeeplearn_amd/csrc/bn.hip
+++ b/matdeeplearn_amd/csrc/bn.hip
@@ -1,22 +1,7 @@
 #include "mdl_common.h"
+#include "bn_apply.h"
 
 namespace mdl {
-
-constexpr int BN_R = MDL_BN_REPLICAS;
-
-__device__ __forceinline__ void bn_totals(const float* __restrict__ sums, float* tot, int C, float* publish) {
-    for (int c = threadIdx.x; c < 2 * C; c += blockDim.x) {
-        float v[BN_R];
-#pragma unroll
-        for (int r = 0; r < BN_R; ++r) v[r] = sums[(size_t)r * 2 * C + c];
-        float t = 0.0f;
-#pragma unroll
-        for (int r = 0; r < BN_R; ++r) t += v[r];
-        tot[c] = t;
-        if (publish && blockIdx.x == 0) publish[c] = t;
-    }
-    __syncthreads();
-}
 
 template <typename T, int MODE, int W>
 __global__ __launch_bounds__(256) void bn_reduce_kernel(const T* __restrict__ a, const T* __restrict__ b,
@@ -57,7 +42,7 @@
                     for (int j = 0; j < W; ++j) { const float d = (va[u][j] - p0[j]) * m; s0[j] += d; s1[j] += d * d; }
                 } else {
 #pragma unroll
-                    for (int j = 0; j < W; ++j) { const float v = va[u][j] * m; s0[j] += v; s1[j] += v * ((vb[u][j] - p0[j]) * p1[j]); }
+                    for (int j = 0; j < W; ++j) { const float v = va[u][j] * m; s0[j] += v; s1[j] += v * bn_xhat(vb[u][j], p0[j], p1[j]); }
                 }
             }
         }
@@ -102,33 +87,15 @@
         for (int j = 0; j < W; ++j) sh[j] = srow[cg * W + j];
     }
     bn_totals(sums, tot, C, sums + (size_t)BN_R * 2 * C);
-    const float invn = 1.0f / (float)N;
-#pragma unroll
-    for (int j = 0; j < W; ++j) {
-        const int c = cg * W + j;
-        const float m1 = tot[c] * invn;
-        const float var = fmaxf(tot[C + c] * invn - m1 * m1, 0.0f);
-        const float istd = rsqrtf(var + eps);
-        mean[j] = sh[j] + m1;
-        const float g = gamma ? gamma[c] : 1.0f;
-        scale[j] = istd * g;
-        shiftv[j] = (beta ? beta[c] : 0.0f) - mean[j] * scale[j];
-        if (blockIdx.x == 0 && (int)threadIdx.x < CG) {
-            save[c] = mean[j];
-            save[C + c] = istd;
-            if (run_mean) {
-                const float unb = N > 1 ? var * ((float)N / (float)(N - 1)) : var;
-                run_mean[c] = (1.0f - momentum) * run_mean[c] + momentum * mean[j];
-                run_var[c] = (1.0f - momentum) * run_var[c] + momentum * unb;
-            }
-        }
-    }
+    float istd[W];
+    bn_forward_stats<W>(tot, sh, C, cg, N, eps, momentum, gamma, beta, save, run_mean, run_var,
+                        blockIdx.x == 0 && (int)threadIdx.x < CG, mean, istd, scale, shiftv);
     while (true) {
 #pragma unroll
         for (int u = 0; u < U; ++u) {
             const int64_t q = q0 + u * stride;
 #pragma unroll
-            for (int j = 0; j < W; ++j) v[u][j] = v[u][j] * scale[j] + shiftv[j];
+            for (int j = 0; j < W; ++j) v[u][j] = bn_apply_elem(v[u][j], scale[j], shiftv[j]);
             if (q < total) V::st(y + (q / CG) * C + cg * W, v[u]);
         }
         q0 += U * stride;
@@ -184,7 +151,7 @@
             const int64_t q = q0 + u * stride;
 #pragma unroll
             for (int j = 0; j < W; ++j) {
-                const float d = gs[j] * (vd[u][j] - k0[j] - (vx[u][j] - mean[j]) * istd[j] * k1[j]);
+                const float d = gs[j] * (vd[u][j] - k0[j] - bn_xhat(vx[u][j], mean[j], istd[j]) * k1[j]);
                 vd[u][j] = (!MASK || vx[u][j] > 0.0f) ? d : 0.0f;
             }
             if (q < total) V::st(dx + (q / CG) * C + cg * W, vd[u]);
diff --git a/matdeeplearn_amd/csrc/bn_apply.h b/matdeeplearn_amd/csrc/bn_apply.h
--- /dev/null
+++ b/matdeeplearn_amd/csrc/bn_apply.h
@@ -0,0 +1,68 @@
+#pragma once
+#include "mdl_common.h"
+
+namespace mdl {
+
+__device__ __forceinline__ void bn_affine(float mean, float invstd, float gamma, float beta, float& scale, float& shift) {
+    scale = invstd * gamma;
+    shift = fmaf(-mean, scale, beta);
+}
+__device__ __forceinline__ float bn_apply_elem(float x, float scale, float shift) { return fmaf(x, scale, shift); }
+__device__ __forceinline__ float bn_xhat(float x, float mean, float invstd) { return (x - mean) * invstd; }
+
+constexpr int BN_R = MDL_BN_REPLICAS;
+
+__device__ __forceinline__ void bn_totals(const float* __restrict__ sums, float* tot, int C, float* publish) {
+    for (int c = threadIdx.x; c < 2 * C; c += blockDim.x) {
+        float v[BN_R];
+#pragma unroll
+        for (int r = 0; r < BN_R; ++r) v[r] = sums[(size_t)r * 2 * C + c];
+        float t = 0.0f;
+#pragma unroll
+        for (int r = 0; r < BN_R; ++r) t += v[r];
+        tot[c] = t;
+        if (publish && blockIdx.x == 0) publish[c] = t;
+    }
+    __syncthreads();
+}
+
+template <int W>
+__device__ __forceinline__ void bn_forward_stats(const float* tot, const float* sh, int C, int cg, int64_t N, float eps, float momentum,
+                                                 const float* __restrict__ gamma, const float* __restrict__ beta,
+                                                 float* __restrict__ save, float* __restrict__ run_mean, float* __restrict__ run_var,
+                                                 bool writer, float* mean, float* istdv, float* scale, float* shiftv) {
+    const float invn = 1.0f / (float)N;
+#pragma unroll
+    for (int j = 0; j < W; ++j) {
+        const int c = cg * W + j;
+        const float m1 = tot[c] * invn;
+        const float var = fmaxf(tot[C + c] * invn - m1 * m1, 0.0f);
+        const float istd = rsqrtf(var + eps);
+        mean[j] = sh[j] + m1;
+        istdv[j] = istd;
+        const float g = gamma ? gamma[c] : 1.0f;
+        bn_affine(mean[j], istd, g, beta ? beta[c] : 0.0f, scale[j], shiftv[j]);
+        if (writer) {
+            save[c] = mean[j];
+            save[C + c] = istd;
+            if (run_mean) {
+                const float unb = N > 1 ? var * ((float)N / (float)(N - 1)) : var;
+                run_mean[c] = (1.0f - momentum) * run_mean[c] + momentum * mean[j];
+                run_var[c] = (1.0f - momentum) * run_var[c] + momentum * unb;
+            }
+        }
+    }
+}
+
+typedef __attribute__((ext_vector_type(4))) unsigned bn_u32x4;
+__device__ __forceinline__ bn_u32x4 bn_apply_chunk8(bn_u32x4 raw, const float* scale, const float* shift) {
+    bn_u32x4 out;
+#pragma unroll
+    for (int k = 0; k < 4; ++k) {
+        const float lo = __uint_as_float(raw[k] << 16), hi = __uint_as_float(raw[k] & 0xffff0000u);
+        out[k] = pk_bf16(bn_apply_elem(lo, scale[2 * k], shift[2 * k]), bn_apply_elem(hi, scale[2 * k + 1], shift[2 * k + 1]));
+    }
+    return out;
+}
+
+}
diff --git a/matdeeplearn_amd/csrc/cgconv_node.hip b/matdeeplearn_amd/csrc/cgconv_node.hip
--- a/matdeeplearn_amd/csrc/cgconv_node.hip
+++ b/matdeeplearn_amd/csrc/cgconv_node.hip
@@ -1,6 +1,16 @@
 #include "mdl_common.h"
+#include "bn_apply.h"
 
 namespace mdl {
+
+struct NodeBn {
+    const bf16_t* y;
+    const float* save;
+    const float* gamma;
+    const float* beta;
+    float* sums;
+    const int64_t* nrows;
+};
 
 constexpr int K3C_NW = 8;
 
@@ -11,12 +21,13 @@
     return __builtin_bit_cast(bf16x8, r);
 }
 
-template <int CP, bool RS16 = false, int NW = 4>
+template <int CP, bool RS16 = false, int NW = 4, bool BN = false>
 __global__ __launch_bounds__(64 * NW, 2) void cgconv_node_stream_kernel(const bf16_t* __restrict__ x, const bf16_t* __restrict__ gout,
                                                                     const bf16_t* __restrict__ r_tgt,
                                                                     const float* __restrict__ r_src,
                                                                     const bf16_t* __restrict__ wn_t, bf16_t* __restrict__ dx,
-                                                                    float* __restrict__ dwn, int64_t N, int zero_src, int ld_out) {
+                                                                    float* __restrict__ dwn, int64_t N, int zero_src, int ld_out,
+                                                                    const NodeBn bn) {
     typedef __attribute__((ext_vector_type(4))) short s16x4;
     typedef __attribute__((address_space(3))) s16x4* lds4_t;
     constexpr int TN = 64;
@@ -37,10 +48,25 @@
     bf16_t* wl = reinterpret_cast<bf16_t*>(smem);
     bf16_t* rl = wl + CP * LD;
     bf16_t* xl = rl + TN * LD;
+    bf16_t* yl = xl + TN * LX;
+    float* bnp = reinterpret_cast<float*>(yl + TN * LX);
+    float* bred = bnp + 4 * CP;
     const int tid = threadIdx.x, lane = tid & 63, i = lane & 31, h = lane >> 5, wv = __builtin_amdgcn_readfirstlane(tid >> 6);
     for (int q = tid; q < CP * (K4 / 8); q += NTH) {
         const int row = q / (K4 / 8), c8 = q - row * (K4 / 8);
         *reinterpret_cast<bf16x8*>(wl + row * LD + c8 * 8) = *reinterpret_cast<const bf16x8*>(wn_t + row * K4 + c8 * 8);
+    }
+    int64_t nrows = N;
+    float bs0 = 0.0f, bs1 = 0.0f;
+    if constexpr (BN) {
+        static_assert(NTH >= CP, "one thread per channel");
+        if (bn.nrows) nrows = max((int64_t)1, min(*bn.nrows, N));
+        if (tid < CP) {
+            const float mean = bn.save[tid], istd = bn.save[CP + tid];
+            float sc, sh;
+            bn_affine(mean, istd, bn.gamma ? bn.gamma[tid] : 1.0f, bn.beta ? bn.beta[tid] : 0.0f, sc, sh);
+            bnp[tid] = sc; bnp[CP + tid] = sh; bnp[2 * CP + tid] = mean; bnp[3 * CP + tid] = istd;
+        }
     }
     f32x16 dw[MJ];
 #pragma unroll
@@ -65,7 +91,7 @@
         const __amdgpu_buffer_rsrc_t tr = rsrc(r_tgt + nb * (2 * CP), rem * (2 * CP * 2));
         const __amdgpu_buffer_rsrc_t sr = RS16 ? rsrc(reinterpret_cast<const bf16_t*>(r_src) + nb * (2 * CP), rem * (2 * CP * 2))
                                                : rsrc(r_src + nb * (2 * CP), rem * (2 * CP * 4));
-        const __amdgpu_buffer_rsrc_t xr = rsrc(x + nb * CP, rem * (CP * 2));
+        const __amdgpu_buffer_rsrc_t xr = rsrc((BN ? bn.y : x) + nb * CP, rem * (CP * 2));
 #pragma unroll
         for (int l = 0; l < NTL; ++l) treg[l] = __builtin_amdgcn_raw_buffer_load_b128(tr, to + opaque(l * (TROWS * 2 * CP * 2)), 0, 0);
 #pragma unroll
@@ -103,7 +129,19 @@
         }
 #pragma unroll
         for (int l = 0; l < NXL; ++l) {
+            if constexpr (BN) {
+                const int row = xrow0 + l * XROWS;
+                *reinterpret_cast<u32x4_t*>(yl + row * LX + 8 * xcc) = xreg[l];
+                float sc[8], sh[8];
+                *reinterpret_cast<f32x4*>(sc) = *reinterpret_cast<const f32x4*>(bnp + 8 * xcc);
+                *reinterpret_cast<f32x4*>(sc + 4) = *reinterpret_cast<const f32x4*>(bnp + 8 * xcc + 4);
+                *reinterpret_cast<f32x4*>(sh) = *reinterpret_cast<const f32x4*>(bnp + CP + 8 * xcc);
+                *reinterpret_cast<f32x4*>(sh + 4) = *reinterpret_cast<const f32x4*>(bnp + CP + 8 * xcc + 4);
+                const u32x4_t v = bn_apply_chunk8(xreg[l], sc, sh);
+                *reinterpret_cast<u32x4_t*>(xl + row * LX + 8 * xcc) = (nb + row < nrows) ? v : u32x4_t{0u, 0u, 0u, 0u};
+            } else {
             *reinterpret_cast<u32x4_t*>(xl + (xrow0 + l * XROWS) * LX + 8 * xcc) = xreg[l];
+            }
         }
         __syncthreads();
         const bool dxw = wv < 2 * NT;
@@ -130,8 +168,24 @@
             }
             const __amdgpu_buffer_rsrc_t dr = rsrc(dx + (nb + mt0 * 32) * CP, (remg > 0 ? remg : 0) * (CP * 2));
 #pragma unroll
-            for (int r = 0; r < 16; ++r)
-                __builtin_amdgcn_raw_buffer_store_b16((short)f2bf(bf2f((bf16_t)gv[r]) + acc[r]), dr, go + ((r & 3) + 8 * (r >> 2)) * CP * 2, 0, 0);
+            for (int r = 0; r < 16; ++r) {
+                gv[r] = (short)f2bf(bf2f((bf16_t)gv[r]) + acc[r]);
+                __builtin_amdgcn_raw_buffer_store_b16(gv[r], dr, go + ((r & 3) + 8 * (r >> 2)) * CP * 2, 0, 0);
+            }
+            if constexpr (BN) {
+                const int col = nt0 * 32 + i;
+                const float mu = bnp[2 * CP + col], is = bnp[3 * CP + col];
+                const bf16_t* yc = yl + (mt0 * 32 + 4 * h) * LX + col;
+                const int64_t left = nrows - nb - mt0 * 32 - 4 * h;
+#pragma unroll
+                for (int r = 0; r < 16; ++r) {
+                    const int dr_ = (r & 3) + 8 * (r >> 2);
+                    const bool ok = dr_ < left;
+                    const float d = ok ? bf2f((bf16_t)gv[r]) : 0.0f;
+                    bs0 += d;
+                    bs1 += ok ? d * bn_xhat(bf2f(yc[dr_ * LX]), mu, is) : 0.0f;
+                }
+            }
         }
 #pragma unroll
         for (int j = 0; j < MJ; ++j) {
@@ -147,6 +201,25 @@
                 const bf16x8 bfr = {b0[0], b0[1], b0[2], b0[3], b1[0], b1[1], b1[2], b1[3]};
                 dw[j] = __builtin_amdgcn_mfma_f32_32x32x16_bf16(af, bfr, dw[j], 0, 0, 0);
             }
+        }
+    }
+    if constexpr (BN) {
+        if (wv < 2 * NT) { bred[wv * 64 + lane] = bs0; bred[2 * NT * 64 + wv * 64 + lane] = bs1; }
+        __syncthreads();
+        if (tid < CP) {
+            const int nt = tid >> 5, ii = tid & 31;
+            float t0 = 0.0f, t1 = 0.0f;
+#pragma unroll
+            for (int mt = 0; mt < 2; ++mt)
+#pragma unroll
+                for (int hh = 0; hh < 2; ++hh) {
+                    const int at = (mt * NT + nt) * 64 + hh * 32 + ii;
+                    t0 += bred[at];
+                    t1 += bred[2 * NT * 64 + at];
+                }
+            float* dst = bn.sums + (size_t)(blockIdx.x % MDL_BN_REPLICAS) * 2 * CP;
+            unsafeAtomicAdd(dst + tid, t0);
+            unsafeAtomicAdd(dst + CP + tid, t1);
         }
     }
 #pragma unroll
@@ -379,7 +452,8 @@
 }
 
 static int bwd_node_launch(const void* x, const void* grad_out, const void* r_tgt, float* r_src, const void* wn_t, void* dx,
-                           float* dwn, int64_t N, int C, int dtype, int zero_src, bool rs16, int ld_out, mdlStream_t stream);
+                           float* dwn, int64_t N, int C, int dtype, int zero_src, bool rs16, int ld_out, const mdl::NodeBn& bn,
+                           mdlStream_t stream);
 
 extern "C" int mdl_cgconv_bwd_node_ex(const MdlCgNode* a, mdlStream_t stream) {
     MDL_REQUIRE(a && a->size == sizeof(MdlCgNode), MDL_E_ARG, "mdl_cgconv_bwd_node_ex: argument struct of another layout (size %u, expected %u)",
@@ -397,6 +471,7 @@
                         reinterpret_cast<uintptr_t>(a->grad_out) % 4 == 0 && reinterpret_cast<uintptr_t>(a->dx) % 4 == 0, MDL_E_ARG,
                     "mdl_cgconv_bwd_node_ex: 16-byte alignment required");
         MDL_REQUIRE(a->ld_dwn == 0 || a->ld_dwn >= 2 * a->C, MDL_E_ARG, "mdl_cgconv_bwd_node_ex: ld_dwn (%d) below 2 C", a->ld_dwn);
+        MDL_REQUIRE(!a->bn_y, MDL_E_UNSUPP, "mdl_cgconv_bwd_node_ex: bn_y is a bf16 path (not with MDL_SPLIT_BF16)");
         if (a->N == 0) return MDL_OK;
         constexpr int NWX = 8;
         const int lds = (2 * 64 * (256 + 8) + 2 * 64 * (256 + 8) + 2 * 64 * (64 + 8)) * 2;
@@ -409,12 +484,19 @@
                            (const float*)a->r_tgt, static_cast<float*>(a->r_src), (const float*)a->wn_t, (float*)a->dx, a->dwn, a->N, a->zero_src, a->ld_dwn);
         return check_launch("mdl_cgconv_bwd_node_ex");
     }
-    return bwd_node_launch(a->x, a->grad_out, a->r_tgt, static_cast<float*>(a->r_src), a->wn_t, a->dx, a->dwn, a->N, a->C,
-                           a->dtype | (int)a->flags, a->zero_src, a->r_src_dtype == MDL_BF16, a->ld_dwn, stream);
+    const mdl::NodeBn bn = {static_cast<const mdl::bf16_t*>(a->bn_y), a->bn_save, a->bn_gamma, a->bn_beta, a->bn_sums, a->bn_nrows};
+    if (a->bn_y) {
+        MDL_REQUIRE(a->bn_save && a->bn_sums, MDL_E_ARG, "mdl_cgconv_bwd_node_ex: bn_y needs bn_save and bn_sums");
+        MDL_REQUIRE(reinterpret_cast<uintptr_t>(a->bn_y) % 16 == 0, MDL_E_ARG, "mdl_cgconv_bwd_node_ex: bn_y must be 16-byte aligned");
+        MDL_REQUIRE(a->r_src_dtype == MDL_BF16, MDL_E_UNSUPP, "mdl_cgconv_bwd_node_ex: bn_y needs bf16 by-source sums (r_src_dtype MDL_BF16)");
+    }
+    return bwd_node_launch(a->bn_y ? a->bn_y : a->x, a->grad_out, a->r_tgt, static_cast<float*>(a->r_src), a->wn_t, a->dx, a->dwn, a->N, a->C,
+                           a->dtype | (int)a->flags, a->zero_src, a->r_src_dtype == MDL_BF16, a->ld_dwn, bn, stream);
 }
 
 static int bwd_node_launch(const void* x, const void* grad_out, const void* r_tgt, float* r_src, const void* wn_t, void* dx,
-                           float* dwn, int64_t N, int C, int dtype, int zero_src, bool rs16, int ld_out, mdlStream_t stream) {
+                           float* dwn, int64_t N, int C, int dtype, int zero_src, bool rs16, int ld_out, const mdl::NodeBn& bn,
+                           mdlStream_t stream) {
     using namespace mdl;
     const bool det = (dtype & MDL_DETERMINISTIC) != 0;
     dtype &= MDL_DTYPE_MASK;
@@ -430,17 +512,21 @@
     int64_t sgrid = cdiv(N, 64);
     if (det) sgrid = 1;
     if (sgrid > 256) sgrid = 256;
+    const int bn_lds = bn.y ? 64 * (C + 8) * 2 + 4 * C * 4 + 2 * (C / 16) * 64 * 4 : 0;
     if (C == 64) {
-        const int lds = (64 * (256 + 8) + 64 * (256 + 8) + 64 * (64 + 8)) * 2;
-        auto kf = rs16 ? cgconv_node_stream_kernel<64, true, K3C_NW> : cgconv_node_stream_kernel<64, false, K3C_NW>;
-        set_max_dynamic_lds(reinterpret_cast<const void*>(kf), lds);
+        const int lds = (64 * (256 + 8) + 64 * (256 + 8) + 64 * (64 + 8)) * 2 + bn_lds;
+        auto kf = bn.y ? cgconv_node_stream_kernel<64, true, K3C_NW, true>
+                       : (rs16 ? cgconv_node_stream_kernel<64, true, K3C_NW> : cgconv_node_stream_kernel<64, false, K3C_NW>);
+        hipError_t e = set_max_dynamic_lds(reinterpret_cast<const void*>(kf), lds);
+        if (e != hipSuccess) { set_error("mdl_cgconv_bwd_node: LDS attribute (%d B): %s", lds, hipGetErrorString(e)); return MDL_E_LAUNCH; }
         hipLaunchKernelGGL(kf, dim3((unsigned)sgrid), dim3(64 * K3C_NW), lds, st, (const bf16_t*)x, (const bf16_t*)grad_out,
-                           (const bf16_t*)r_tgt, r_src, (const bf16_t*)wn_t, (bf16_t*)dx, dwn, N, zero_src, ld_out);
+                           (const bf16_t*)r_tgt, r_src, (const bf16_t*)wn_t, (bf16_t*)dx, dwn, N, zero_src, ld_out, bn);
     } else {
-        const int lds = (32 * (128 + 8) + 64 * (128 + 8) + 64 * (32 + 8)) * 2;
-        auto kf = rs16 ? cgconv_node_stream_kernel<32, true> : cgconv_node_stream_kernel<32, false>;
+        const int lds = (32 * (128 + 8) + 64 * (128 + 8) + 64 * (32 + 8)) * 2 + bn_lds;
+        auto kf = bn.y ? cgconv_node_stream_kernel<32, true, 4, true>
+                       : (rs16 ? cgconv_node_stream_kernel<32, true> : cgconv_node_stream_kernel<32, false>);
         hipLaunchKernelGGL(kf, dim3((unsigned)sgrid), dim3(256), lds, st, (const bf16_t*)x, (const bf16_t*)grad_out,
-                           (const bf16_t*)r_tgt, r_src, (const bf16_t*)wn_t, (bf16_t*)dx, dwn, N, zero_src, ld_out);
+                           (const bf16_t*)r_tgt, r_src, (const bf16_t*)wn_t, (bf16_t*)dx, dwn, N, zero_src, ld_out, bn);
     }
     return check_launch("mdl_cgconv_bwd_node");
 }
diff --git a/matdeeplearn_amd/csrc/readout.hip b/matdeeplearn_amd/csrc/readout.hip
--- /dev/null
+++ b/matdeeplearn_amd/csrc/readout.hip
@@ -0,0 +1,238 @@
+#include "mdl_common.h"
+#include "bn_apply.h"
+
+namespace mdl {
+
+constexpr int RO_W = 8;
+
+__device__ __forceinline__ void ro_accumulate(const bf16_t* __restrict__ y, int C, int cg, int b, int nv, int j, int RL,
+                                              const float* mean, const float* istd, float* ay, float* ax) {
+    typedef VecW<bf16_t, RO_W> V;
+    const bf16_t* base = y + cg * RO_W;
+    for (int k = b + j; k < b + nv; k += 2 * RL) {
+        float v0[RO_W], v1[RO_W];
+        const int k1 = min(k + RL, b + nv - 1);
+        V::ld(base + (int64_t)k * C, v0);
+        V::ld(base + (int64_t)k1 * C, v1);
+        const float two = (k + RL < b + nv) ? 1.0f : 0.0f;
+#pragma unroll
+        for (int q = 0; q < RO_W; ++q) {
+            ay[q] += v0[q] + two * v1[q];
+            ax[q] += bn_xhat(v0[q], mean[q], istd[q]) + two * bn_xhat(v1[q], mean[q], istd[q]);
+        }
+    }
+}
+
+template <bool SMALL>
+__global__ __launch_bounds__(256) void bn_meanpool_fwd_kernel(const bf16_t* __restrict__ y, float* __restrict__ sums,
+                                                              const float* __restrict__ gamma, const float* __restrict__ beta,
+                                                              float* __restrict__ save, float* __restrict__ run_mean,
+                                                              float* __restrict__ run_var, const int32_t* __restrict__ rowptr,
+                                                              bf16_t* __restrict__ pooled, float* __restrict__ mxhat, int64_t Ncap,
+                                                              int C, int64_t G, float eps, float momentum,
+                                                              const int64_t* __restrict__ n_dev, int shift_row) {
+    constexpr int W = RO_W;
+    typedef VecW<bf16_t, W> V;
+    const int64_t N = n_dev ? max((int64_t)1, min(*n_dev, Ncap)) : Ncap;
+    __shared__ float tot[128];
+    __shared__ float red[SMALL ? 2 * 256 * W : 1];
+    const int CG = C / W, t = threadIdx.x;
+    const int RL = SMALL ? 256 / CG : 4;
+    const int rem = SMALL ? t : t % (CG * 4);
+    const int j = rem / CG, cg = rem - j * CG;
+    float sh[W], mean[W], istd[W], scale[W], shiftv[W];
+    V::ld(y + cg * W, sh);
+    if (shift_row) {
+        const float* srow = sums + (size_t)(2 * BN_R + 2) * C;
+#pragma unroll
+        for (int q = 0; q < W; ++q) sh[q] = srow[cg * W + q];
+    }
+    bn_totals(sums, tot, C, sums + (size_t)BN_R * 2 * C);
+    bn_forward_stats<W>(tot, sh, C, cg, N, eps, momentum, gamma, beta, save, run_mean, run_var, blockIdx.x == 0 && t < CG, mean, istd,
+                        scale, shiftv);
+    const int GPB = SMALL ? 1 : 256 / (CG * 4);
+    for (int64_t g0 = (int64_t)blockIdx.x * GPB; g0 < G; g0 += (int64_t)gridDim.x * GPB) {
+        const int64_t gi = SMALL ? g0 : g0 + t / (CG * 4);
+        const int64_t g = min(gi, G - 1);
+        const int b = rowptr[g], e = rowptr[g + 1];
+        const int nv = (int)max((int64_t)0, min((int64_t)e, N) - b);
+        float ay[W], ax[W];
+#pragma unroll
+        for (int q = 0; q < W; ++q) { ay[q] = 0.0f; ax[q] = 0.0f; }
+        if (!SMALL || j < RL) ro_accumulate(y, C, cg, b, nv, j, RL, mean, istd, ay, ax);
+        if constexpr (SMALL) {
+            __syncthreads();
+#pragma unroll
+            for (int q = 0; q < W; ++q) { red[t * W + q] = ay[q]; red[256 * W + t * W + q] = ax[q]; }
+            __syncthreads();
+            if (t < CG) {
+#pragma unroll
+                for (int q = 0; q < W; ++q) { ay[q] = 0.0f; ax[q] = 0.0f; }
+                for (int r = 0; r < RL; ++r)
+#pragma unroll
+                    for (int q = 0; q < W; ++q) { ay[q] += red[(r * CG + t) * W + q]; ax[q] += red[256 * W + (r * CG + t) * W + q]; }
+            }
+        } else {
+#pragma unroll
+            for (int q = 0; q < W; ++q) {
+                ay[q] += __shfl_xor(ay[q], CG);
+                ay[q] += __shfl_xor(ay[q], 2 * CG);
+                ax[q] += __shfl_xor(ax[q], CG);
+                ax[q] += __shfl_xor(ax[q], 2 * CG);
+            }
+        }
+        if (j == 0 && gi < G) {
+            const float cnt = (float)max(e - b, 1), fv = (float)nv / cnt;
+            float o[W], m[W];
+#pragma unroll
+            for (int q = 0; q < W; ++q) {
+                o[q] = bn_apply_elem(ay[q] / cnt, scale[q], shiftv[q] * fv);
+                m[q] = ax[q] / cnt;
+            }
+            V::st(pooled + (g * CG + cg) * W, o);
+            *reinterpret_cast<f32x4*>(mxhat + (g * CG + cg) * W) = f32x4{m[0], m[1], m[2], m[3]};
+            *reinterpret_cast<f32x4*>(mxhat + (g * CG + cg) * W + 4) = f32x4{m[4], m[5], m[6], m[7]};
+        }
+    }
+}
+
+__global__ __launch_bounds__(256) void bn_meanpool_bwd_sums_kernel(const bf16_t* __restrict__ gp, const float* __restrict__ mxhat,
+                                                                   const int32_t* __restrict__ rowptr, float* __restrict__ sums,
+                                                                   int64_t Ncap, int C, int64_t G, const int64_t* __restrict__ n_dev) {
+    const int64_t N = n_dev ? max((int64_t)1, min(*n_dev, Ncap)) : Ncap;
+    __shared__ float red[2][256];
+    const int t = threadIdx.x, c = t % C, r = t / C, RL = 256 / C;
+    float s0 = 0.0f, s1 = 0.0f;
+    for (int64_t g = (int64_t)blockIdx.x * RL + r; g < G; g += (int64_t)gridDim.x * RL) {
+        const int b = rowptr[g], e = rowptr[g + 1];
+        const float fv = (float)max((int64_t)0, min((int64_t)e, N) - b) / (float)max(e - b, 1);
+        const float v = bf2f(gp[g * C + c]);
+        s0 += v * fv;
+        s1 += v * mxhat[g * C + c];
+    }
+    red[0][t] = s0;
+    red[1][t] = s1;
+    __syncthreads();
+    if (t < C) {
+        float t0 = 0.0f, t1 = 0.0f;
+        for (int q = 0; q < RL; ++q) { t0 += red[0][q * C + t]; t1 += red[1][q * C + t]; }
+        float* dst = sums + (size_t)(blockIdx.x % BN_R) * 2 * C;
+        unsafeAtomicAdd(dst + t, t0);
+        unsafeAtomicAdd(dst + C + t, t1);
+    }
+}
+
+__global__ __launch_bounds__(256) void bn_meanpool_bwd_apply_kernel(const bf16_t* __restrict__ gp, const bf16_t* __restrict__ y,
+                                                                    const float* __restrict__ save, float* __restrict__ sums,
+                                                                    const float* __restrict__ gamma, const int32_t* __restrict__ rowptr,
+                                                                    const int32_t* __restrict__ seg, bf16_t* __restrict__ dx,
+                                                                    int64_t Ncap, int C, const int64_t* __restrict__ n_dev) {
+    constexpr int W = RO_W, U = 2;
+    typedef VecW<bf16_t, W> V;
+    const int64_t N = n_dev ? max((int64_t)1, min(*n_dev, Ncap)) : Ncap;
+    __shared__ float tot[128];
+    const int CG = C / W;
+    const int cg = threadIdx.x % CG;
+    const int64_t total = N * CG;
+    const int64_t stride = (int64_t)gridDim.x * blockDim.x;
+    int64_t q0 = (int64_t)blockIdx.x * blockDim.x + threadIdx.x;
+    float vd[U][W], vx[U][W], rc[U];
+    auto load = [&]() {
+#pragma unroll
+        for (int u = 0; u < U; ++u) {
+            const int64_t n = min(q0 + u * stride, total - 1) / CG;
+            const int g = seg[n];
+            rc[u] = 1.0f / (float)max(rowptr[g + 1] - rowptr[g], 1);
+            V::ld(gp + ((int64_t)g * CG + cg) * W, vd[u]);
+            V::ld(y + n * C + cg * W, vx[u]);
+        }
+    };
+    load();
+    bn_totals(sums, tot, C, sums + (size_t)BN_R * 2 * C);
+    const float invn = 1.0f / (float)N;
+    float mean[W], istd[W], k0[W], k1[W], gs[W];
+#pragma unroll
+    for (int j = 0; j < W; ++j) {
+        const int c = cg * W + j;
+        mean[j] = save[c];
+        istd[j] = save[C + c];
+        gs[j] = (gamma ? gamma[c] : 1.0f) * istd[j];
+        k0[j] = tot[c] * invn;
+        k1[j] = tot[C + c] * invn;
+    }
+    while (true) {
+#pragma unroll
+        for (int u = 0; u < U; ++u) {
+            const int64_t q = q0 + u * stride;
+#pragma unroll
+            for (int j = 0; j < W; ++j) vd[u][j] = gs[j] * (vd[u][j] * rc[u] - k0[j] - bn_xhat(vx[u][j], mean[j], istd[j]) * k1[j]);
+            if (q < total) V::st(dx + (q / CG) * C + cg * W, vd[u]);
+        }
+        q0 += U * stride;
+        if (q0 >= total) break;
+        load();
+    }
+    if (N < Ncap) {
+        float z[W];
+#pragma unroll
+        for (int j = 0; j < W; ++j) z[j] = 0.0f;
+        for (int64_t q = total + (int64_t)blockIdx.x * blockDim.x + threadIdx.x; q < Ncap * CG; q += stride)
+            V::st(dx + (q / CG) * C + cg * W, z);
+    }
+}
+
+static int ro_check(const char* name, int64_t N, int C, int64_t G, int dtype, const void* a, const void* b, const void* c) {
+    MDL_REQUIRE(dtype == MDL_BF16 && (C == 32 || C == 64), MDL_E_UNSUPP, "%s: bf16 with C in {32, 64} only (dtype %d, C=%d)", name, dtype, C);
+    MDL_REQUIRE(N >= 1 && G >= 1 && N < (1ll << 31) && G < (1ll << 31), MDL_E_ARG, "%s: bad N=%lld G=%lld", name, (long long)N, (long long)G);
+    MDL_REQUIRE(a && b && c && (reinterpret_cast<uintptr_t>(a) | reinterpret_cast<uintptr_t>(b) | reinterpret_cast<uintptr_t>(c)) % 16 == 0,
+                MDL_E_ARG, "%s: null or misaligned tensor", name);
+    return MDL_OK;
+}
+
+}
+
+extern "C" int mdl_bn_meanpool_fwd(const void* y, float* sums, const float* gamma, const float* beta, float* save, float* running_mean,
+                                   float* running_var, const int32_t* rowptr, void* pooled, float* mean_xhat, int64_t N, int C,
+                                   int64_t G, float eps, float momentum, const int64_t* n_rows_dev, int dtype, mdlStream_t stream) {
+    using namespace mdl;
+    const int shift_row = (dtype & MDL_BN_SHIFT_ROW) ? 1 : 0;
+    dtype &= MDL_DTYPE_MASK;
+    int rc = ro_check("mdl_bn_meanpool_fwd", N, C, G, dtype, y, pooled, mean_xhat);
+    if (rc) return rc;
+    MDL_REQUIRE(sums && save && rowptr, MDL_E_ARG, "mdl_bn_meanpool_fwd: null pointer");
+    hipStream_t st = (hipStream_t)stream;
+    const int CG = C / RO_W;
+    if (G * CG < 65536 && G <= 65535) {
+        hipLaunchKernelGGL(bn_meanpool_fwd_kernel<true>, dim3((unsigned)G), dim3(256), 0, st, (const bf16_t*)y, sums, gamma, beta, save,
+                           running_mean, running_var, rowptr, (bf16_t*)pooled, mean_xhat, N, C, G, eps, momentum, n_rows_dev, shift_row);
+    } else {
+        int64_t g = cdiv(G * CG * 4, 256);
+        if (g > 1024) g = 1024;
+        hipLaunchKernelGGL(bn_meanpool_fwd_kernel<false>, dim3((unsigned)g), dim3(256), 0, st, (const bf16_t*)y, sums, gamma, beta, save,
+                           running_mean, running_var, rowptr, (bf16_t*)pooled, mean_xhat, N, C, G, eps, momentum, n_rows_dev, shift_row);
+    }
+    return check_launch("mdl_bn_meanpool_fwd");
+}
+
+extern "C" int mdl_bn_meanpool_bwd(const void* grad_pooled, const void* y, const float* save, float* sums, const float* gamma,
+                                   const int32_t* rowptr, const int32_t* seg, const float* mean_xhat, void* dx, int64_t N, int C,
+                                   int64_t G, const int64_t* n_rows_dev, int dtype, mdlStream_t stream) {
+    using namespace mdl;
+    const bool det = (dtype & MDL_DETERMINISTIC) != 0;
+    dtype &= MDL_DTYPE_MASK;
+    int rc = ro_check("mdl_bn_meanpool_bwd", N, C, G, dtype, y, grad_pooled, dx);
+    if (rc) return rc;
+    MDL_REQUIRE(sums && save && rowptr && seg && mean_xhat, MDL_E_ARG, "mdl_bn_meanpool_bwd: null pointer");
+    hipStream_t st = (hipStream_t)stream;
+    int64_t gs = det ? 1 : cdiv(G, (int64_t)(256 / C) * 8);
+    if (gs > 256) gs = 256;
+    hipLaunchKernelGGL(bn_meanpool_bwd_sums_kernel, dim3((unsigned)gs), dim3(256), 0, st, (const bf16_t*)grad_pooled, mean_xhat, rowptr,
+                       sums, N, C, G, n_rows_dev);
+    rc = check_launch("mdl_bn_meanpool_bwd");
+    if (rc) return rc;
+    int64_t g = cdiv(N * (C / RO_W), 256 * 4);
+    if (g > 768) g = 768;
+    hipLaunchKernelGGL(bn_meanpool_bwd_apply_kernel, dim3((unsigned)g), dim3(256), 0, st, (const bf16_t*)grad_pooled, (const bf16_t*)y, save,
+                       sums, gamma, rowptr, seg, (bf16_t*)dx, N, C, n_rows_dev);
+    return check_launch("mdl_bn_meanpool_bwd");
+}
diff --git a/matdeeplearn_amd/models/_base.py b/matdeeplearn_amd/models/_base.py
--- a/matdeeplearn_amd/models/_base.py
+++ b/matdeeplearn_amd/models/_base.py
@@ -129,9 +129,14 @@
             return self.set2set(out, data.batch, num_graphs)
         return ops.POOLS[self.pool](out, data.batch, num_graphs, seg_index=getattr(data, "pool_index", None))
 
-    def _head(self, out, data):
+    def _bn_pool(self, bn, out, data):
+        if not (self.pool == "global_mean_pool" and self.pool_order == "early" and (self.dropout_rate == 0.0 or not self.training)):
+            return None
+        return bn.mean_pool(out, data.batch, getattr(data, "num_graphs", None), seg_index=getattr(data, "pool_index", None))
+
+    def _head(self, out, data, pooled=None):
         if self.pool_order == "early":
-            out = self._post(self._pool(out, data).to(out.dtype), final=True)
+            out = self._post((self._pool(out, data) if pooled is None else pooled).to(out.dtype), final=True)
         else:
             out = self._post(out)
             if self.pool == "set2set":
diff --git a/matdeeplearn_amd/models/cgcnn.py b/matdeeplearn_amd/models/cgcnn.py
--- a/matdeeplearn_amd/models/cgcnn.py
+++ b/matdeeplearn_amd/models/cgcnn.py
@@ -26,7 +26,14 @@
         bn_on = self.batch_norm == "True"
         packs = ops.cgconv_prepack(list(self.conv_list), out.dtype, out.device, want_node=torch.is_grad_enabled()) if out.is_cuda else None
         dist = getattr(data, "dist", None)
+        last = len(self.conv_list) - 1
         for i, conv in enumerate(self.conv_list):
+            if bn_on and i == last and not ops._CG_BN_STATS:
+                y = conv(out, None, edge_attr, csr=csr, packed=None if packs is None else packs[i], split=self.split_products, dist=dist)
+                pooled = self._bn_pool(self.bn_list[i], y, data)
+                if pooled is not None:
+                    return self._head(y, data, pooled=pooled)
+                return self._head(self._drop(self.bn_list[i](y)), data)
             prev = self.bn_list[i - 1].bias if (bn_on and i > 0) else None
             out = self._drop(conv(out, None, edge_attr, csr=csr, bn=self.bn_list[i] if bn_on else None, bn_shift=prev,
                                   packed=None if packs is None else packs[i], split=self.split_products, dist=dist))
diff --git a/matdeeplearn_amd/nn.py b/matdeeplearn_amd/nn.py
--- a/matdeeplearn_amd/nn.py
+++ b/matdeeplearn_amd/nn.py
@@ -371,6 +371,18 @@
         return ops.cgconv_bn(x, edge_index, edge_attr, conv.lin_f.weight, conv.lin_f.bias, conv.lin_s.weight, conv.lin_s.bias,
                              conv.aggr, csr, self.weight, self.bias, rm, rv, self.eps, self.momentum, shift, packed)
 
+    def mean_pool(self, x, batch, size=None, seg_index=None):
+        if not (self.training and self.momentum is not None and self.num_features == x.shape[1]):
+            return None
+        si = ops.bn_mean_pool_ok(x, batch, size, seg_index)
+        if si is None:
+            return None
+        rm = rv = None
+        if self.track_running_stats:
+            rm, rv = self.running_mean, self.running_var
+            self._nbt_pending = getattr(self, "_nbt_pending", 0) + 1
+        return ops.bn_mean_pool(x, si, self.weight, self.bias, rm, rv, self.eps, self.momentum)
+
     def after_linear_relu(self, h, weight, bias, lowp=None, gathered=None):
         use_batch_stats = self.training or not self.track_running_stats
         if not (use_batch_stats and self.momentum is not None and ops.linear_relu_bn_ok(h, weight, bias is not None, gathered)):
diff --git a/matdeeplearn_amd/ops.py b/matdeeplearn_amd/ops.py
--- a/matdeeplearn_amd/ops.py
+++ b/matdeeplearn_amd/ops.py
@@ -538,6 +538,8 @@
     "dense_bwd_wide": ("_DENSE_BWD_WIDE", "... also when both widths exceed 128"),
     "mlp_head": ("_MLP_HEAD", "post-FC head as one launch per direction"),
     "linear_wide": ("_LINEAR_WIDE", "NNConv's Y = x W2r on the streaming kernel"),
+    "node_bn_sums": ("_NODE_BN_SUMS", "BatchNorm backward sums of the layer below a CGConv from that CGConv's node kernel (no mdl_bn_bwd_stats launch)"),
+    "bn_readout": ("_BN_READOUT", "last BatchNorm folded through the mean pool (no [N, C] BatchNorm output, backward sums from graph rows)"),
     "tn_scratch": ("_TN_SCRATCH", "weight-gradient blocks of the TN products as plain stores + a reduce launch (off: atomics from every workgroup)"),
 }
 
@@ -577,6 +579,7 @@
 _BALANCE = True
 _PAD128 = True
 _RSRC16 = True
+_NODE_BN_SUMS = True
 
 
 _RSRC = {}
@@ -610,6 +613,7 @@
         require_hip(x, edge_attr, w_f, w_s)
         if edge_attr.dtype != x.dtype:
             raise MdlError("cgconv: x (%s) and edge_attr (%s) must share a dtype" % (x.dtype, edge_attr.dtype))
+        ctx.bn_rec = getattr(x, "_mdl_bn", None) if _NODE_BN_SUMS else None
         x, edge_attr = x.contiguous(), edge_attr.contiguous()
         N, C = x.shape
         E, G = edge_attr.shape
@@ -717,10 +721,19 @@
         if node_hip:
             wn_t = _node_weights(ctx, C, Cp, torch.float32 if node_x3 else torch.bfloat16, x.device, wf32, ws32)
             dx = torch.empty_like(x)
+            rec = ctx.bn_rec
+            bn_kw = {}
+            if (rec is not None and rs16 and not node_x3 and Ck == C and rec.y.shape == x.shape and rec.y.dtype == x.dtype
+                    and rec.y.data_ptr() % 16 == 0 and ctx.needs_input_grad[0]):
+                R = lib().mdl_bn_sums_rows()
+                bsums = _zeros_grad(R * C, x.device).view(R, C)
+                bn_kw = dict(bn_y=rec.y, bn_save=rec.save, bn_gamma=rec.gamma, bn_beta=rec.beta, bn_sums=bsums, bn_nrows=rec.n_dev)
             nargs = _lib.cg_node_args(dtype=dt, flags=fl | (sp if node_x3 else 0), zero_src=1 if keep is not None else 0, N=N, C=C,
                                       r_src_dtype=_lib.MDL_BF16 if rs16 else _lib.MDL_F32, ld_dwn=ldw if direct else 0, x=x, grad_out=g,
-                                      r_tgt=r_tgt, r_src=r_src, wn_t=wn_t, dx=dx, dwn=dwn)
+                                      r_tgt=r_tgt, r_src=r_src, wn_t=wn_t, dx=dx, dwn=dwn, **bn_kw)
             check(_launch_timed("bwd_node", lambda: lib().mdl_cgconv_bwd_node_ex(nargs, stream())), "mdl_cgconv_bwd_node_ex")
+            if bn_kw:
+                rec.offer(dx, bsums)
             if keep is not None:
                 keep[1] = False
             if direct:
@@ -919,7 +932,7 @@
     R = lib().mdl_bn_sums_rows()
     buf = _zeros_step((R + 3, C), x.device)
     y = cgconv(x, edge_index, edge_attr, w_f, b_f, w_s, b_s, aggr, csr=csr, bn_stats=(buf, _f32c(shift)), packed=packed)
-    return _BatchNormTrain.apply(y, bn_weight, bn_bias, running_mean, running_var, eps, momentum, buf)
+    return _bn_train(y, bn_weight, bn_bias, running_mean, running_var, eps, momentum, buf)
 
 
 class _Gather(torch.autograd.Function):
@@ -1949,9 +1962,34 @@
     return int(lib().mdl_bn_sums_rows())
 
 
+class _BnRecord:
+    __slots__ = ("y", "save", "gamma", "beta", "n_dev", "dx", "dx_version", "sums")
+
+    def __init__(self):
+        self.y = self.dx = self.sums = None
+
+    def offer(self, dx, sums):
+        self.dx, self.dx_version, self.sums = dx, dx._version, sums
+
+    def take(self, dy):
+        dx, sums, self.dx, self.sums = self.dx, self.sums, None, None
+        if (dx is not None and dy.data_ptr() == dx.data_ptr() and dy._version == self.dx_version and dy.shape == dx.shape
+                and dy.dtype == dx.dtype and dy.stride() == dx.stride()):
+            return sums
+        return None
+
+
+def _bn_train(x, weight, bias, running_mean, running_var, eps, momentum, pre=None):
+    rec = _BnRecord() if (_NODE_BN_SUMS and x.dtype == torch.bfloat16 and x.shape[1] in (32, 64)) else None
+    out = _BatchNormTrain.apply(x, weight, bias, running_mean, running_var, eps, momentum, pre, rec)
+    if rec is not None and rec.y is not None:
+        out._mdl_bn = rec
+    return out
+
+
 class _BatchNormTrain(torch.autograd.Function):
     @staticmethod
-    def forward(ctx, x, weight, bias, running_mean, running_var, eps, momentum, pre=None):
+    def forward(ctx, x, weight, bias, running_mean, running_var, eps, momentum, pre=None, rec=None):
         N, C = x.shape
         dt = dtype_code(x)
         R = lib().mdl_bn_sums_rows()
@@ -1969,24 +2007,30 @@
         ctx.save_for_backward(x, save, gw)
         ctx.has = (weight is not None, bias is not None)
         ctx.wdt = None if weight is None else weight.dtype
+        ctx.rec = rec
+        if rec is not None:
+            rec.y, rec.save, rec.gamma, rec.beta, rec.n_dev = x, save, gw, gb, nd
         return y
 
     @staticmethod
     def backward(ctx, dy):
         x, save, gw = ctx.saved_tensors
         N, C = x.shape
+        sums = ctx.rec.take(dy) if ctx.rec is not None else None
         dy = dy.contiguous()
         dt = dtype_code(x)
         R = lib().mdl_bn_sums_rows()
-        sums = _zeros_grad(R * C, x.device).view(R, C)
         dx = torch.empty_like(x)
         nd = ctx.n_dev
-        check(lib().mdl_bn_bwd_stats_n(ptr(dy), ptr(x), ptr(save), ptr(sums), N, C, ptr(nd), dt | _dflag(), stream()), "mdl_bn_bwd_stats")
+        if sums is None:
+            sums = _zeros_grad(R * C, x.device).view(R, C)
+            check(lib().mdl_bn_bwd_stats_n(ptr(dy), ptr(x), ptr(save), ptr(sums), N, C, ptr(nd), dt | _dflag(), stream()),
+                  "mdl_bn_bwd_stats")
         check(lib().mdl_bn_bwd_apply_n(ptr(dy), ptr(x), ptr(save), ptr(sums), ptr(gw), ptr(dx), N, C, ptr(nd), dt, stream()),
               "mdl_bn_bwd_apply")
         dgamma = sums[R - 1].to(ctx.wdt) if ctx.has[0] else None
         dbeta = sums[R - 2].to(ctx.wdt) if ctx.has[1] else None
-        return dx, dgamma, dbeta, None, None, None, None, None
+        return dx, dgamma, dbeta, None, None, None, None, None, None
 
 
 class _LinearReluBN(torch.autograd.Function):
@@ -2079,8 +2123,63 @@
                                *[t.to(x.dtype) for t, _ in gathered])
 
 
+_BN_READOUT = True
+
+
+class _BnMeanPool(torch.autograd.Function):
+    @staticmethod
+    def forward(ctx, x, weight, bias, running_mean, running_var, eps, momentum, si):
+        N, C = x.shape
+        dt = dtype_code(x)
+        R = lib().mdl_bn_sums_rows()
+        buf = _zeros_step((R + 2, C), x.device)
+        sums, save = buf[:R], buf[-2:]
+        gw, gb = _f32c(weight), _f32c(bias)
+        pooled = torch.empty((si.N, C), dtype=x.dtype, device=x.device)
+        mxhat = torch.empty((si.N, C), dtype=torch.float32, device=x.device)
+        nd = _true_rows_for(N)
+        check(lib().mdl_bn_stats_n(ptr(x), ptr(sums), N, C, ptr(nd), dt | _dflag(), stream()), "mdl_bn_stats")
+        check(lib().mdl_bn_meanpool_fwd(ptr(x), ptr(sums), ptr(gw), ptr(gb), ptr(save), ptr(running_mean), ptr(running_var),
+                                        ptr(si.rowptr), ptr(pooled), ptr(mxhat), N, C, si.N, float(eps), float(momentum), ptr(nd), dt,
+                                        stream()), "mdl_bn_meanpool_fwd")
+        ctx.n_dev, ctx.si = nd, si
+        ctx.save_for_backward(x, save, gw, mxhat)
+        ctx.has = (weight is not None, bias is not None)
+        ctx.wdt = None if weight is None else weight.dtype
+        return pooled
+
+    @staticmethod
+    def backward(ctx, gp):
+        x, save, gw, mxhat = ctx.saved_tensors
+        N, C = x.shape
+        si = ctx.si
+        gp = gp.contiguous()
+        R = lib().mdl_bn_sums_rows()
+        sums = _zeros_grad(R * C, x.device).view(R, C)
+        dx = torch.empty_like(x)
+        check(lib().mdl_bn_meanpool_bwd(ptr(gp), ptr(x), ptr(save), ptr(sums), ptr(gw), ptr(si.rowptr), ptr(si.seg), ptr(mxhat),
+                                        ptr(dx), N, C, si.N, ptr(ctx.n_dev), dtype_code(x) | _dflag(), stream()), "mdl_bn_meanpool_bwd")
+        dgamma = sums[R - 1].to(ctx.wdt) if ctx.has[0] else None
+        dbeta = sums[R - 2].to(ctx.wdt) if ctx.has[1] else None
+        return dx, dgamma, dbeta, None, None, None, None, None
+
+
+def bn_mean_pool_ok(x, batch, size, seg_index=None):
+    if not (_BN_READOUT and x.is_cuda and x.dim() == 2 and x.dtype == torch.bfloat16 and x.shape[1] in (32, 64)
+            and x.is_contiguous() and x.shape[0] >= 2 and x.data_ptr() % 16 == 0 and (seg_index is not None or size is not None)):
+        return None
+    si = seg_index if seg_index is not None else _seg_index(batch, size, True)
+    if si.perm is not None or si.E != x.shape[0] or si.N < 1:
+        return None
+    return si
+
+
+def bn_mean_pool(x, si, weight, bias, running_mean, running_var, eps=1e-5, momentum=0.1):
+    return _BnMeanPool.apply(x, weight, bias, running_mean, running_var, eps, momentum, si)
+
+
 def batch_norm_train(x, weight, bias, running_mean, running_var, eps=1e-5, momentum=0.1):
-    return _BatchNormTrain.apply(x, weight, bias, running_mean, running_var, eps, momentum)
+    return _bn_train(x, weight, bias, running_mean, running_var, eps, momentum)
 
 
 GRAPH_MAX_NEIGHBORS = 64
```
